# haberdashPI/SignalOperators.jl

Hardware: AMD Instinct MI355X
Metric: frames/sec sink() 44.1kHz 8ch Mix+Filt+Resample; achieved HBM GB/s (higher is better)
Workload: dtype f64

## Files before the change

### include/sigops.h

```cpp
#ifndef SIGOPS_H
#define SIGOPS_H

#include <stdint.h>

#ifdef __cplusplus
extern "C" {
#endif
#if defined(__GNUC__)
#pragma GCC visibility push(default)
#endif

#define SO_ABI_VERSION 1

typedef enum so_status {
    SO_OK = 0,
    SO_ERR_INVALID = -1,
    SO_ERR_LENGTH = -2,
    SO_ERR_UNSUPPORTED = -3,
    SO_ERR_RUNTIME = -4,
    SO_ERR_CHANNELS = -5,
    SO_ERR_NODEVICE = -6
} so_status_t;

typedef enum so_dtype {
// ... 30 lines not shown
    SO_FN_IDENTITY = 2,
    SO_FN_RANDN = 3
} so_fn_t;

typedef enum so_rampfn {
    SO_RAMP_SINRAMP = 0,
    SO_RAMP_IDENTITY = 1,
    SO_RAMP_EXPR = 2
} so_rampfn_t;

typedef enum so_mapfn {
    SO_MAP_ADD = 0,
    SO_MAP_MUL = 1,
    SO_MAP_SUB = 2,
    SO_MAP_DIV = 3,
    SO_MAP_TUPLECAT = 4,
    SO_MAP_GETCHAN = 5,
    SO_MAP_AS1CHANNEL = 6,
    SO_MAP_ASNCHANNELS = 7,
    SO_MAP_TOELTYPE = 8,
    SO_MAP_REVERSECH = 9,
    SO_MAP_EXPR = 10
} so_mapfn_t;

typedef struct so_eop {
    int32_t code;
    int32_t arg;
} so_eop_t;

typedef enum so_eop_code {
    SO_EOP_ARG = 0,
    SO_EOP_CONST = 1,
    SO_EOP_UN = 2,
    SO_EOP_BIN = 3,
    SO_EOP_CMP = 4,
    SO_EOP_SELECT = 5,
    SO_EOP_ROUND32 = 6,
    SO_EOP_INTERP = 7
} so_eop_code_t;

typedef enum so_un {
    SO_UN_NEG = 0, SO_UN_ABS = 1, SO_UN_SQRT = 2, SO_UN_CBRT = 3, SO_UN_SQUARE = 4,
    SO_UN_RECIPROCAL = 5, SO_UN_EXP = 6, SO_UN_EXP2 = 7, SO_UN_EXPM1 = 8, SO_UN_LOG = 9,
    SO_UN_LOG2 = 10, SO_UN_LOG10 = 11, SO_UN_LOG1P = 12, SO_UN_SIN = 13, SO_UN_COS = 14,
    SO_UN_TAN = 15, SO_UN_ARCSIN = 16, SO_UN_ARCCOS = 17, SO_UN_ARCTAN = 18, SO_UN_SINH = 19,
    SO_UN_COSH = 20, SO_UN_TANH = 21, SO_UN_ARCSINH = 22, SO_UN_ARCCOSH = 23,
    SO_UN_ARCTANH = 24, SO_UN_FLOOR = 25, SO_UN_CEIL = 26, SO_UN_TRUNC = 27, SO_UN_RINT = 28,
    SO_UN_SIGN = 29,
    SO_UN_COUNT = 30
} so_un_t;

typedef enum so_bin {
    SO_BIN_ADD = 0, SO_BIN_SUB = 1, SO_BIN_MUL = 2, SO_BIN_DIV = 3, SO_BIN_POW = 4,
    SO_BIN_REMAINDER = 5, SO_BIN_FMOD = 6, SO_BIN_MINIMUM = 7, SO_BIN_MAXIMUM = 8,
    SO_BIN_FMIN = 9, SO_BIN_FMAX = 10, SO_BIN_ARCTAN2 = 11, SO_BIN_HYPOT = 12,
    SO_BIN_COPYSIGN = 13,
    SO_BIN_COUNT = 14
} so_bin_t;

typedef enum so_cmp {
    SO_CMP_LT = 0, SO_CMP_LE = 1, SO_CMP_GT = 2, SO_CMP_GE = 3, SO_CMP_EQ = 4, SO_CMP_NE = 5,
    SO_CMP_COUNT = 6
} so_cmp_t;

typedef enum so_padkind {
    SO_PAD_VALUE = 0,
    SO_PAD_VECTOR = 1,
    SO_PAD_ZERO = 2,
    SO_PAD_ONE = 3,
    SO_PAD_LASTFRAME = 4,
    SO_PAD_CYCLE = 5,
    SO_PAD_MIRROR = 6
} so_padkind_t;

typedef enum so_rskind {
    SO_RS_RATIONAL = 0,
    SO_RS_ARBITRARY = 1,
    SO_RS_FIR = 2
} so_rskind_t;

typedef struct so_node {
    int32_t kind;
    int32_t dtype;
    int32_t nch;
    int32_t n_children;
    const int32_t* children;
    int64_t nframes;
    double fs;
    int32_t i0, i1, i2, i3;
    int64_t l0, l1;
    double d0, d1, d2, d3;
    const void* p0;
    const void* p1;
    int64_t s0, s1;
} so_node_t;

typedef struct so_out_desc {
    int32_t dtype;
    int32_t nch;
    int64_t nframes;
    int64_t frame_stride;
    int64_t chan_stride;
    int32_t is_device;
    int32_t reserved;
} so_out_desc_t;

typedef struct so_stats {
    int32_t n_stages;
    int32_t n_launches;
    int64_t algorithmic_bytes;
    int64_t scratch_bytes;
    int64_t h2d_bytes;
    int64_t d2h_bytes;
    double last_exec_ms;
    double dominant_kernel_ms;
    int64_t dominant_kernel_bytes;
    char dominant_kernel[64];
} so_stats_t;

typedef struct so_plan so_plan_t;

int32_t so_abi_version(void);

const char* so_last_error(void);

int32_t so_device_count(void);

int32_t so_plan_create(const so_node_t* nodes, int32_t n_nodes, int32_t root,
                       const so_out_desc_t* out, int32_t device, so_plan_t** plan);

int64_t so_plan_nframes(const so_plan_t* plan);

int32_t so_plan_execute(so_plan_t* plan, void* out, void* hip_stream);

int32_t so_plan_check(so_plan_t* plan, void* hip_stream);

int32_t so_plan_set_array(so_plan_t* plan, int32_t node_index, const void* data);

int32_t so_plan_stats(const so_plan_t* plan, so_stats_t* stats);

typedef struct so_step_info {
    char name[64];
    int64_t algorithmic_bytes;
    double ms;
    int32_t launches;
    int32_t pad;
} so_step_info_t;
int32_t so_plan_step_info(const so_plan_t* plan, int32_t index, so_step_info_t* info);

typedef enum so_counter {
    SO_COUNTER_GRAPH_REPLAYS = 0,
    SO_COUNTER_GRAPH_CAPTURES = 1,
    SO_COUNTER_DIRECT_EXECUTES = 2,
    SO_COUNTER_FUSED_MFMAS_PER_BLOCK = 3
} so_counter_t;
int64_t so_plan_counter(const so_plan_t* plan, int32_t which);

int32_t so_rtc_compile_check(const char* body, char* log, int32_t log_capacity);

int32_t so_rtc_wait_idle(void);
int32_t so_rtc_shutdown(void);

int32_t so_plan_set_profiling(so_plan_t* plan, int32_t enable);

void so_plan_destroy(so_plan_t* plan);

typedef struct so_comm so_comm_t;
typedef struct so_slab {
    int64_t rows, row_elems;
    int64_t dst_offset;
    int64_t dst_row_stride;
} so_slab_t;
int32_t so_comm_unique_id(void* id128);
int32_t so_comm_create(const void* id128, int32_t world, int32_t rank, int32_t device, so_comm_t** comm);
int32_t so_comm_allgather(so_comm_t* comm, const void* mine, int64_t src_row_stride, void* full,
                          const so_slab_t* slabs, int32_t dtype, void* stream);
int32_t so_comm_reduce_sum(so_comm_t* comm, void* buf, int64_t rows, int64_t row_elems, int64_t row_stride,
                           int32_t dtype, int32_t root, void* stream);
const char* so_comm_last_error(void);
void so_comm_destroy(so_comm_t* comm);

typedef enum so_filt_type {
    SO_FILT_LOWPASS = 0,
    SO_FILT_HIGHPASS = 1,
    SO_FILT_BANDPASS = 2,
    SO_FILT_BANDSTOP = 3
} so_filt_type_t;

typedef enum so_filt_method {
    SO_METHOD_BUTTERWORTH = 0,
    SO_METHOD_CHEBYSHEV1 = 1
} so_filt_method_t;

int32_t so_design_iir(int32_t type, double f1, double f2, double fs, int32_t method,
                      int32_t order, double ripple_db, double* sos, int32_t sos_capacity,
                      int32_t* nsections, double* gain);

int32_t so_design_iir_zpk(int32_t type, double f1, double f2, double fs, int32_t method, int32_t order,
                          double ripple_db, double* z, int32_t* nz, double* p, int32_t* np, int32_t capacity,
                          double* k);
int32_t so_zpk_to_sos(const double* z, int32_t nz, const double* p, int32_t np, double k, double* sos,
                      int32_t sos_capacity, int32_t* nsections, double* gain);

int32_t so_tf_to_sos(const double* b, int32_t nb, const double* a, int32_t na, double* sos, int32_t sos_capacity,
                     int32_t* nsections, double* gain, double* residual);
int32_t so_tf_zero_input(const double* b, int32_t nb, const double* a, int32_t na, const double* si, int32_t nsi,
                         double* out, int64_t capacity, int64_t* nframes);

int32_t so_design_resample_rational(int64_t num, int64_t den, double* h, int32_t capacity,
                                    int32_t* hlen);
int32_t so_design_resample_arbitrary(double rate, int32_t nphi, double* h, int32_t capacity,
                                     int32_t* hlen);

int32_t so_resample_positions(double fs_in, double fs_out, double rate, int32_t nphi, const double* h,
                              int32_t hlen, int64_t n_out, int64_t* j, int32_t* p, double* alpha,
                              int64_t* nfix, int64_t* nbaked);

#if defined(__GNUC__)
#pragma GCC visibility pop
#endif
#ifdef __cplusplus
}
#endif
#endif
```

### signaloperators.jl_amd/_capi.py

```python
import ctypes as C
import os

_HERE = os.path.dirname(os.path.abspath(__file__))
LIB_PATH = os.environ.get("SIGOPS_LIB") or os.path.join(_HERE, "csrc", "libsigops.so")

SO_F32, SO_F64, SO_I64 = 0, 1, 2
SO_LEN_INF, SO_LEN_MISSING, SO_LEN_UNCHECKED = -1, -2, -3
(NODE_ARRAY, NODE_CONST, NODE_FUNC, NODE_UNTIL, NODE_AFTER, NODE_PAD, NODE_APPEND, NODE_RAMP,
 NODE_MAP, NODE_FILT_SOS, NODE_RESAMPLE, NODE_NORMPOWER, NODE_SAMPLEAT, NODE_COMB, NODE_CUMSUM) = range(15)
FN = {"sin": 0, "cos": 1, "identity": 2, "randn": 3}
SO_FN_RANDN = FN["randn"]
RAMPFN = {"sinramp": 0, "identity": 1, "expr": 2}
MAPFN = {"add": 0, "mul": 1, "sub": 2, "div": 3, "tuplecat": 4, "getchan": 5, "as1channel": 6,
         "asnchannels": 7, "toeltype": 8, "reversech": 9, "expr": 10}
EOP = {"arg": 0, "const": 1, "un": 2, "bin": 3, "cmp": 4, "select": 5, "round32": 6, "interp": 7}
INTERP_MAX_KNOTS = 1 << 20
UN = {name: i for i, name in enumerate((
    "neg", "abs", "sqrt", "cbrt", "square", "reciprocal", "exp", "exp2", "expm1", "log", "log2", "log10", "log1p",
    "sin", "cos", "tan", "arcsin", "arccos", "arctan", "sinh", "cosh", "tanh", "arcsinh", "arccosh", "arctanh",
    "floor", "ceil", "trunc", "rint", "sign"))}
BIN = {name: i for i, name in enumerate((
    "add", "sub", "mul", "div", "pow", "remainder", "fmod", "minimum", "maximum", "fmin", "fmax", "arctan2", "hypot",
    "copysign"))}
CMP = {"lt": 0, "le": 1, "gt": 2, "ge": 3, "eq": 4, "ne": 5}
PAD = {"value": 0, "vector": 1, "zero": 2, "one": 3, "lastframe": 4, "cycle": 5, "mirror": 6}
RS_RATIONAL, RS_ARBITRARY, RS_FIR = 0, 1, 2
FILT = {"lowpass": 0, "highpass": 1, "bandpass": 2, "bandstop": 3}
METHOD = {"butterworth": 0, "chebyshev1": 1}


class so_node_t(C.Structure):
    _fields_ = [("kind", C.c_int32), ("dtype", C.c_int32), ("nch", C.c_int32),
                ("n_children", C.c_int32), ("children", C.POINTER(C.c_int32)),
                ("nframes", C.c_int64), ("fs", C.c_double),
                ("i0", C.c_int32), ("i1", C.c_int32), ("i2", C.c_int32), ("i3", C.c_int32),
                ("l0", C.c_int64), ("l1", C.c_int64),
                ("d0", C.c_double), ("d1", C.c_double), ("d2", C.c_double), ("d3", C.c_double),
                ("p0", C.c_void_p), ("p1", C.c_void_p), ("s0", C.c_int64), ("s1", C.c_int64)]


class so_out_desc_t(C.Structure):
    _fields_ = [("dtype", C.c_int32), ("nch", C.c_int32), ("nframes", C.c_int64),
                ("frame_stride", C.c_int64), ("chan_stride", C.c_int64),
                ("is_device", C.c_int32), ("reserved", C.c_int32)]


class so_stats_t(C.Structure):
    _fields_ = [("n_stages", C.c_int32), ("n_launches", C.c_int32),
                ("algorithmic_bytes", C.c_int64), ("scratch_bytes", C.c_int64),
                ("h2d_bytes", C.c_int64), ("d2h_bytes", C.c_int64),
                ("last_exec_ms", C.c_double), ("dominant_kernel_ms", C.c_double),
                ("dominant_kernel_bytes", C.c_int64), ("dominant_kernel", C.c_char * 64)]


class so_slab_t(C.Structure):
    _fields_ = [("rows", C.c_int64), ("row_elems", C.c_int64), ("dst_offset", C.c_int64), ("dst_row_stride", C.c_int64)]


class so_step_info_t(C.Structure):
    _fields_ = [("name", C.c_char * 64), ("algorithmic_bytes", C.c_int64), ("ms", C.c_double),
                ("launches", C.c_int32), ("pad", C.c_int32)]


EXPORTS = ["so_abi_version", "so_last_error", "so_device_count", "so_plan_create",
           "so_plan_nframes", "so_plan_execute", "so_plan_check", "so_plan_set_array", "so_plan_stats",
           "so_plan_set_profiling", "so_plan_destroy", "so_design_iir",
           "so_design_resample_rational", "so_design_resample_arbitrary",
           "so_resample_positions", "so_plan_step_info", "so_design_iir_zpk", "so_zpk_to_sos", "so_tf_to_sos", "so_tf_zero_input", "so_plan_counter",
           "so_rtc_compile_check", "so_rtc_wait_idle", "so_rtc_shutdown", "so_comm_unique_id", "so_comm_create", "so_comm_allgather", "so_comm_reduce_sum", "so_comm_last_error", "so_comm_destroy"]

_lib = None


class EngineMissing(RuntimeError):
    pass


def lib():
    global _lib
    if _lib is not None:
        return _lib
    if not os.path.exists(LIB_PATH):
        raise EngineMissing(
            f"{LIB_PATH} not built: run `python __graft_entry__.py build` "
            "(hipcc --offload-arch=gfx950). The HIP engine has no CPU fallback.")
    try:
        import importlib.util as _ilu

        if _ilu.find_spec("torch") is not None:
            import torch
    except Exception:
        pass
    L = C.CDLL(LIB_PATH)
    L.so_abi_version.restype = C.c_int32
    L.so_last_error.restype = C.c_char_p
    L.so_device_count.restype = C.c_int32
    L.so_plan_create.restype = C.c_int32
    L.so_plan_create.argtypes = [C.POINTER(so_node_t), C.c_int32, C.c_int32,
                                 C.POINTER(so_out_desc_t), C.c_int32, C.POINTER(C.c_void_p)]
    L.so_plan_nframes.restype = C.c_int64
    L.so_plan_nframes.argtypes = [C.c_void_p]
    L.so_plan_execute.restype = C.c_int32
    L.so_plan_execute.argtypes = [C.c_void_p, C.c_void_p, C.c_void_p]
    L.so_plan_check.restype = C.c_int32
    L.so_plan_check.argtypes = [C.c_void_p, C.c_void_p]
    L.so_plan_set_array.restype = C.c_int32
    L.so_plan_set_array.argtypes = [C.c_void_p, C.c_int32, C.c_void_p]
    L.so_plan_stats.restype = C.c_int32
    L.so_plan_stats.argtypes = [C.c_void_p, C.POINTER(so_stats_t)]
    L.so_plan_set_profiling.restype = C.c_int32
    L.so_plan_set_profiling.argtypes = [C.c_void_p, C.c_int32]
    L.so_plan_destroy.restype = None
    L.so_plan_destroy.argtypes = [C.c_void_p]
    L.so_design_iir.restype = C.c_int32
    L.so_design_iir.argtypes = [C.c_int32, C.c_double, C.c_double, C.c_double, C.c_int32,
                                C.c_int32, C.c_double, C.POINTER(C.c_double), C.c_int32,
                                C.POINTER(C.c_int32), C.POINTER(C.c_double)]
    L.so_design_resample_rational.restype = C.c_int32
    L.so_design_resample_rational.argtypes = [C.c_int64, C.c_int64, C.POINTER(C.c_double),
                                              C.c_int32, C.POINTER(C.c_int32)]
    L.so_design_resample_arbitrary.restype = C.c_int32
    L.so_design_resample_arbitrary.argtypes = [C.c_double, C.c_int32, C.POINTER(C.c_double),
                                               C.c_int32, C.POINTER(C.c_int32)]
    L.so_design_iir_zpk.restype = C.c_int32
    L.so_design_iir_zpk.argtypes = [C.c_int32, C.c_double, C.c_double, C.c_double, C.c_int32, C.c_int32, C.c_double,
                                    C.POINTER(C.c_double), C.POINTER(C.c_int32), C.POINTER(C.c_double),
                                    C.POINTER(C.c_int32), C.c_int32, C.POINTER(C.c_double)]
    L.so_zpk_to_sos.restype = C.c_int32
    L.so_zpk_to_sos.argtypes = [C.POINTER(C.c_double), C.c_int32, C.POINTER(C.c_double), C.c_int32, C.c_double,
                                C.POINTER(C.c_double), C.c_int32, C.POINTER(C.c_int32), C.POINTER(C.c_double)]
    L.so_tf_to_sos.restype = C.c_int32
    L.so_tf_to_sos.argtypes = [C.POINTER(C.c_double), C.c_int32, C.POINTER(C.c_double), C.c_int32, C.POINTER(C.c_double),
                               C.c_int32, C.POINTER(C.c_int32), C.POINTER(C.c_double), C.POINTER(C.c_double)]
    L.so_tf_zero_input.restype = C.c_int32
    L.so_tf_zero_input.argtypes = [C.POINTER(C.c_double), C.c_int32, C.POINTER(C.c_double), C.c_int32,
                                   C.POINTER(C.c_double), C.c_int32, C.POINTER(C.c_double), C.c_int64,
                                   C.POINTER(C.c_int64)]
    L.so_rtc_compile_check.restype = C.c_int32
    L.so_rtc_compile_check.argtypes = [C.c_char_p, C.c_char_p, C.c_int32]
    L.so_rtc_wait_idle.restype = C.c_int32
    L.so_rtc_wait_idle.argtypes = []
    L.so_rtc_shutdown.restype = C.c_int32
    L.so_rtc_shutdown.argtypes = []
    import atexit

    atexit.register(L.so_rtc_shutdown)
    L.so_comm_unique_id.restype = C.c_int32
    L.so_comm_unique_id.argtypes = [C.c_void_p]
    L.so_comm_create.restype = C.c_int32
    L.so_comm_create.argtypes = [C.c_void_p, C.c_int32, C.c_int32, C.c_int32, C.POINTER(C.c_void_p)]
    L.so_comm_allgather.restype = C.c_int32
    L.so_comm_allgather.argtypes = [C.c_void_p, C.c_void_p, C.c_int64, C.c_void_p, C.POINTER(so_slab_t), C.c_int32, C.c_void_p]
    L.so_comm_reduce_sum.restype = C.c_int32
    L.so_comm_reduce_sum.argtypes = [C.c_void_p, C.c_void_p, C.c_int64, C.c_int64, C.c_int64, C.c_int32, C.c_int32, C.c_void_p]
    L.so_comm_last_error.restype = C.c_char_p
    L.so_comm_destroy.restype = None
    L.so_comm_destroy.argtypes = [C.c_void_p]
    L.so_plan_counter.restype = C.c_int64
    L.so_plan_counter.argtypes = [C.c_void_p, C.c_int32]
    L.so_plan_step_info.restype = C.c_int32
    L.so_plan_step_info.argtypes = [C.c_void_p, C.c_int32, C.POINTER(so_step_info_t)]
    L.so_resample_positions.restype = C.c_int32
    L.so_resample_positions.argtypes = [C.c_double, C.c_double, C.c_double, C.c_int32, C.POINTER(C.c_double),
                                        C.c_int32, C.c_int64, C.POINTER(C.c_int64), C.POINTER(C.c_int32),
                                        C.POINTER(C.c_double), C.POINTER(C.c_int64), C.POINTER(C.c_int64)]
    if L.so_abi_version() != 1:
        raise EngineMissing("libsigops ABI version mismatch")
    _lib = L
    return L


def last_error():
    return lib().so_last_error().decode("utf-8", "replace")
```

### signaloperators.jl_amd/csrc/capi.cpp

```cpp
#include <hip/hip_runtime_api.h>

#include <cstring>
#include <string>
#include <vector>

#include "../../include/sigops.h"
#include "plan.h"

namespace {
thread_local std::string g_err;
int set_err(int status, const std::string& msg) {
    g_err = msg;
    return status;
}
}

struct so_plan {
    so::Plan* p;
};

extern "C" {

int32_t so_abi_version(void) { return SO_ABI_VERSION; }

// ... 53 lines not shown

int32_t so_plan_set_profiling(so_plan_t* plan, int32_t enable) {
    if (!plan) return set_err(SO_ERR_INVALID, "so_plan_set_profiling: null plan");
    so::plan_set_profiling(plan->p, enable);
    return SO_OK;
}

int32_t so_rtc_compile_check(const char* body, char* log, int32_t log_capacity) {
    if (!body) return set_err(SO_ERR_INVALID, "so_rtc_compile_check: null source");
    std::string err;
    const int st = so::rtc_compile_check(body, err);
    if (log && log_capacity > 0) std::snprintf(log, (size_t)log_capacity, "%s", err.c_str());
    return st == 0 ? SO_OK : set_err(SO_ERR_UNSUPPORTED, err);
}

int32_t so_rtc_wait_idle(void) {
    so::rtc_wait_idle();
    return SO_OK;
}

int32_t so_rtc_shutdown(void) {
    so::rtc_shutdown();
    return SO_OK;
}

int64_t so_plan_counter(const so_plan_t* plan, int32_t which) {
    if (!plan) return -1;
    return so::plan_counter(plan->p, which);
}

int32_t so_plan_step_info(const so_plan_t* plan, int32_t index, so_step_info_t* info) {
    if (!plan) return set_err(SO_ERR_INVALID, "so_plan_step_info: null plan");
    return so::plan_step_info(plan->p, index, info);
}

void so_plan_destroy(so_plan_t* plan) {
    if (!plan) return;
    so::plan_destroy(plan->p);
    delete plan;
}

int32_t so_design_iir(int32_t type, double f1, double f2, double fs, int32_t method,
                      int32_t order, double ripple_db, double* sos, int32_t sos_capacity,
                      int32_t* nsections, double* gain) {
    std::vector<double> s;
    double g = 1.0;
    std::string err;
    int st = so::design_iir(type, f1, f2, fs, method, order, ripple_db, s, g, err);
    if (st != SO_OK) return set_err(st, err);
    if (!sos || !nsections || !gain || (int)s.size() > sos_capacity)
        return set_err(SO_ERR_INVALID, "so_design_iir: output buffer too small");
    std::memcpy(sos, s.data(), s.size() * sizeof(double));
    *nsections = (int32_t)(s.size() / 6);
    *gain = g;
    return SO_OK;
}

int32_t so_design_iir_zpk(int32_t type, double f1, double f2, double fs, int32_t method, int32_t order,
                          double ripple_db, double* z, int32_t* nz, double* p, int32_t* np, int32_t capacity,
                          double* k) {
    std::vector<double> zz, pp;
    double kk = 1.0;
    std::string err;
    int st = so::design_iir_zpk(type, f1, f2, fs, method, order, ripple_db, zz, pp, kk, err);
    if (st != SO_OK) return set_err(st, err);
    if (!z || !p || !nz || !np || !k || (int)zz.size() > 2 * capacity || (int)pp.size() > 2 * capacity)
        return set_err(SO_ERR_INVALID, "so_design_iir_zpk: output buffer too small");
    std::memcpy(z, zz.data(), zz.size() * sizeof(double));
    std::memcpy(p, pp.data(), pp.size() * sizeof(double));
    *nz = (int32_t)(zz.size() / 2);
    *np = (int32_t)(pp.size() / 2);
    *k = kk;
    return SO_OK;
}

int32_t so_zpk_to_sos(const double* z, int32_t nz, const double* p, int32_t np, double k, double* sos,
                      int32_t sos_capacity, int32_t* nsections, double* gain) {
    std::vector<double> s;
    double g = 1.0;
    std::string err;
    if ((nz > 0 && !z) || (np > 0 && !p)) return set_err(SO_ERR_INVALID, "so_zpk_to_sos: null roots");
    int st = so::zpk_to_sos(z, nz, p, np, k, s, g, err);
    if (st != SO_OK) return set_err(st, err);
    if (!sos || !nsections || !gain || (int)s.size() > sos_capacity)
        return set_err(SO_ERR_INVALID, "so_zpk_to_sos: output buffer too small");
    std::memcpy(sos, s.data(), s.size() * sizeof(double));
    *nsections = (int32_t)(s.size() / 6);
    *gain = g;
    return SO_OK;
}

int32_t so_tf_to_sos(const double* b, int32_t nb, const double* a, int32_t na, double* sos, int32_t sos_capacity,
                     int32_t* nsections, double* gain, double* residual) {
    std::vector<double> s;
    double g = 1.0, r = 0.0;
    std::string err;
    int st = so::tf_to_sos(b, nb, a, na, s, g, r, err);
    if (st != SO_OK) return set_err(st, err);
    if (!sos || !nsections || !gain || (int)s.size() > sos_capacity)
        return set_err(SO_ERR_INVALID, "so_tf_to_sos: output buffer too small");
    std::memcpy(sos, s.data(), s.size() * sizeof(double));
    *nsections = (int32_t)(s.size() / 6);
    *gain = g;
    if (residual) *residual = r;
    return SO_OK;
}

int32_t so_tf_zero_input(const double* b, int32_t nb, const double* a, int32_t na, const double* si, int32_t nsi,
                         double* out, int64_t capacity, int64_t* nframes) {
    std::string err;
    int64_t used = 0;
    if (!out || !nframes || capacity < 0) return set_err(SO_ERR_INVALID, "so_tf_zero_input: null output");
    int st = so::tf_zero_input(b, nb, a, na, si, nsi, out, capacity, used, err);
    if (st != SO_OK) return set_err(st, err);
    *nframes = used;
    return SO_OK;
}

static int32_t copy_taps(const std::vector<double>& h, double* out, int32_t capacity, int32_t* hlen) {
    if (!hlen) return set_err(SO_ERR_INVALID, "null hlen");
    *hlen = (int32_t)h.size();
    if (!out) return SO_OK;
    if ((int)h.size() > capacity) return set_err(SO_ERR_INVALID, "tap buffer too small");
    std::memcpy(out, h.data(), h.size() * sizeof(double));
    return SO_OK;
}

int32_t so_design_resample_rational(int64_t num, int64_t den, double* h, int32_t capacity,
                                    int32_t* hlen) {
    std::vector<double> t;
    std::string err;
    int st = so::design_resample_rational(num, den, t, err);
    if (st != SO_OK) return set_err(st, err);
    return copy_taps(t, h, capacity, hlen);
}

int32_t so_design_resample_arbitrary(double rate, int32_t nphi, double* h, int32_t capacity,
                                     int32_t* hlen) {
    std::vector<double> t;
    std::string err;
    int st = so::design_resample_arbitrary(rate, nphi, t, err);
    if (st != SO_OK) return set_err(st, err);
    return copy_taps(t, h, capacity, hlen);
}

int32_t so_resample_positions(double fs_in, double fs_out, double rate, int32_t nphi, const double* h,
                              int32_t hlen, int64_t n_out, int64_t* j, int32_t* p, double* alpha,
                              int64_t* nfix, int64_t* nbaked) {
    if (!h || hlen < 1 || nphi < 1 || !(rate > 0) || n_out < 0 || !j || !p || !alpha)
        return set_err(SO_ERR_INVALID, "so_resample_positions: bad arguments");
    return so::resample_positions(fs_in, fs_out, rate, nphi, h, hlen, n_out, j, p, alpha, nfix, nbaked);
}

}
```

### signaloperators.jl_amd/csrc/executor.cpp

```cpp
#include "plan_impl.h"

namespace so {

static inline int carrier_vec_ok(const DCarrier& c, int64_t V) {
    if (!std::getenv("SIGOPS_STRICT_ALIGN")) return (uintptr_t)c.base % (c.dtype == SO_F64 ? 8 : 4) == 0;
    return ((uintptr_t)c.base % 16 == 0) && (c.cstride % V == 0);
}

static hipError_t h2d_small(void* dst, const void* src, size_t bytes) {
    constexpr size_t kPiece = 16 * 1024;
    if (bytes < 2 * kPiece || bytes > (1u << 20)) return hipMemcpy(dst, src, bytes, hipMemcpyHostToDevice);
    for (size_t off = 0; off < bytes; off += kPiece) {
        const hipError_t e = hipMemcpy((char*)dst + off, (const char*)src + off, std::min(kPiece, bytes - off), hipMemcpyHostToDevice);
        if (e != hipSuccess) return e;
    }
    return hipSuccess;
}

void Plan::finalize() {
    for (size_t si = 0; si < stages.size(); ++si) {
        Stage& S = stages[si];
        if (S.out_buf >= 0 && ((int)si == alias_stage || S.win_off >= 0)) {
            bufs[S.out_buf].external = true;
            bufs[S.out_buf].bytes = 0;
// ... 1101 lines not shown
                P->steps[si].ms = ms;
                total += ms;
                if (ms > best) {
                    best = ms;
                    P->stats.dominant_kernel_ms = ms;
                    P->stats.dominant_kernel_bytes = P->steps[si].bytes;
                    std::snprintf(P->stats.dominant_kernel, sizeof P->stats.dominant_kernel, "%s", P->steps[si].name.c_str());
                }
            }
            P->stats.last_exec_ms = total;
        }
    } catch (const PlanError& e) {
        err = e.msg;
        return e.status;
    }
    return SO_OK;
}

int plan_execute(Plan* P, void* outp, void* stream, std::string& err) {
    DeviceGuard guard(P->device);
    if (kernel_gave_up(P, err)) return SO_ERR_RUNTIME;
    const bool eligible = P->steps.size() >= 4 && P->out.is_device && P->host_leaves.empty() && !P->profiling &&
                          !std::getenv("SIGOPS_NO_GRAPH") && !std::getenv("SIGOPS_RS_TRACE");
    if (!eligible) {
        P->n_direct++;
        return plan_execute_direct(P, outp, stream, err);
    }
    hipStream_t st = (hipStream_t)stream;
    const bool leaves_match = P->out_alias_buf < 0 || P->bufs[P->out_alias_buf].d == outp;
    if (P->graph_exec && P->graph_out == outp && P->graph_epoch == P->array_epoch && leaves_match) {
        if (hipSetDevice(P->device) == hipSuccess && hipGraphLaunch(P->graph_exec, st) == hipSuccess) {
            P->n_replays++;
            return SO_OK;
        }
        (void)hipGetLastError();
        (void)hipGraphExecDestroy(P->graph_exec);
        P->graph_exec = nullptr;
        P->graph_failed = true;
    }
    if (P->graph_failed || P->last_out != outp || P->last_epoch != P->array_epoch) {
        P->last_out = outp;
        P->last_epoch = P->array_epoch;
        P->n_direct++;
        return plan_execute_direct(P, outp, stream, err);
    }
    if (P->graph_exec && P->graph_out == outp && P->graph_epoch == P->array_epoch) {
        P->n_direct++;
        return plan_execute_direct(P, outp, stream, err);
    }
    if (P->graph_exec) {
        (void)hipGraphExecDestroy(P->graph_exec);
        P->graph_exec = nullptr;
    }
    hipGraph_t graph = nullptr;
    if (!P->capture_stream && hipStreamCreateWithFlags(&P->capture_stream, hipStreamNonBlocking) != hipSuccess)
        P->capture_stream = nullptr;
    if (!P->capture_stream || hipSetDevice(P->device) != hipSuccess ||
        hipStreamBeginCapture(P->capture_stream, hipStreamCaptureModeRelaxed) != hipSuccess) {
        (void)hipGetLastError();
        P->graph_failed = true;
        return plan_execute_direct(P, outp, stream, err);
    }
    const int rc = plan_execute_direct(P, outp, (void*)P->capture_stream, err);
    const hipError_t ec = hipStreamEndCapture(P->capture_stream, &graph);
    if (std::getenv("SIGOPS_DEBUG_PLAN"))
        std::fprintf(stderr, "[sigops] graph capture: rc=%d end=%d (%s) graph=%p err=%s\n", rc, (int)ec, hipGetErrorString(ec), (void*)graph, err.c_str());
    if (rc != SO_OK || ec != hipSuccess || !graph ||
        hipGraphInstantiate(&P->graph_exec, graph, nullptr, nullptr, 0) != hipSuccess) {
        (void)hipGetLastError();
        if (graph) (void)hipGraphDestroy(graph);
        P->graph_exec = nullptr;
        P->graph_failed = true;
        return rc != SO_OK ? rc : plan_execute_direct(P, outp, stream, err);
    }
    (void)hipGraphDestroy(graph);
    P->graph_out = outp;
    P->graph_epoch = P->array_epoch;
    P->n_captures++;
    if (hipGraphLaunch(P->graph_exec, st) != hipSuccess) {
        (void)hipGetLastError();
        P->graph_failed = true;
        return plan_execute_direct(P, outp, stream, err);
    }
    return SO_OK;
}

int plan_set_array(Plan* P, int32_t node_index, const void* data, std::string& err) {
    if (node_index < 0 || node_index >= (int)P->nodes.size() || P->nodes[node_index].nd.kind != SO_NODE_ARRAY) {
        err = "so_plan_set_array: not an ARRAY node";
        return SO_ERR_INVALID;
    }
    DeviceGuard guard(P->device);
    P->array_ptr[node_index] = data;
    P->array_epoch++;
    if (P->nodes[node_index].nd.i0) {
        bool changed = false;
        for (size_t i = 0; i < P->leaves.size(); ++i)
            if (P->leaf_array_node[i] == node_index) {
                P->leaves[i].base = data;
                changed = true;
            }
        if (changed && P->d_leaves)
            if (hipMemcpy(P->d_leaves, P->leaves.data(), P->leaves.size() * sizeof(DLeaf), hipMemcpyHostToDevice) != hipSuccess) {
                err = "so_plan_set_array: leaf upload failed";
                return SO_ERR_RUNTIME;
            }
        for (auto& S : P->stages) {
            bool touched = false;
            for (auto& c : S.carriers) {
                if (c.array_node == node_index) {
                    c.base = data;
                    const int64_t V = 16 / (int64_t)dsize(c.dtype);
                    c.vec_ok = carrier_vec_ok(c, V);
                    touched = true;
                }
                if (car_has_arr2(c) && c.array_node2 == node_index) {
                    c.base2 = data;
                    c.vec_ok2 = (uintptr_t)c.base2 % (c.dtype2 == SO_F64 ? 8 : 4) == 0;
                    touched = true;
                }
            }
            if (touched) {
                const RsCtl ctl = P->make_ctl(S);
                if (hipMemcpy(P->bufs[S.car_buf].d, S.carriers.data(), S.carriers.size() * sizeof(DCarrier), hipMemcpyHostToDevice) != hipSuccess ||
                    hipMemcpy(P->bufs[S.ctl_buf].d, &ctl, sizeof(RsCtl), hipMemcpyHostToDevice) != hipSuccess) {
                    err = "so_plan_set_array: carrier upload failed";
                    return SO_ERR_RUNTIME;
                }
            }
        }
    }
    return SO_OK;
}

int64_t plan_nframes(const Plan* P) {
    const Node& R = P->nodes[P->root];
    return isinf_(R.len) ? SO_LEN_INF : R.len.n;
}
void plan_stats(const Plan* P, so_stats_t* st) { *st = P->stats; }
void plan_set_profiling(Plan* P, int mode) {
    P->profiling = mode < 0 || mode > 2 ? 1 : mode;
    P->prof_execs = 0;
}
int64_t plan_counter(const Plan* P, int which) {
    switch (which) {
    case SO_COUNTER_GRAPH_REPLAYS: return P->n_replays;
    case SO_COUNTER_GRAPH_CAPTURES: return P->n_captures;
    case SO_COUNTER_DIRECT_EXECUTES: return P->n_direct;
    case SO_COUNTER_FUSED_MFMAS_PER_BLOCK: {
        for (const Stage& S : P->stages)
            if (S.kind == ST_SOS && S.rsos_src >= 0 && S.need > 0) return S.rs.ks + 14;
        return 0;
    }
    default: return -1;
    }
}
int plan_step_info(const Plan* P, int index, so_step_info_t* info) {
    if (info && index >= 0 && index < (int)P->steps.size()) {
        const Step& s = P->steps[index];
        std::memset(info, 0, sizeof *info);
        std::snprintf(info->name, sizeof info->name, "%s", s.name.c_str());
        info->algorithmic_bytes = s.bytes;
        info->ms = s.ms;
        if (P->profiling == 2 && P->prof_execs > 0) {
            const size_t evset = 2 * P->steps.size();
            const int64_t n = std::min<int64_t>(P->prof_execs, (int64_t)prof_cap(P));
            double sum = 0;
            int64_t got = 0;
            for (int64_t e = 0; e < n; ++e) {
                float ms = 0;
                if (hipEventElapsedTime(&ms, P->events[evset * e + 2 * index], P->events[evset * e + 2 * index + 1]) == hipSuccess) {
                    sum += ms;
                    ++got;
                } else (void)hipGetLastError();
            }
            info->ms = got ? sum / (double)got : 0.0;
        }
        info->launches = s.launches;
    }
    return (int)P->steps.size();
}
int plan_check(Plan* P, void* stream, std::string& err) {
    DeviceGuard guard(P->device);
    try {
        if (P->nlanes > 1 || P->graph_exec) HIPCHECK(hipDeviceSynchronize());
        else HIPCHECK(hipStreamSynchronize((hipStream_t)stream));
    } catch (const PlanError& e) {
        err = e.msg;
        return e.status;
    }
    if (kernel_gave_up(P, err)) return SO_ERR_RUNTIME;
    return SO_OK;
}

void plan_destroy(Plan* P) {
    if (!P) return;
    {
        DeviceGuard guard(P->device);
        P->release();
    }
    delete P;
}


}
```

### signaloperators.jl_amd/csrc/k_rsos.hip

```cpp
#include "kcommon.h"
#include "kstage.h"

#ifndef SO_RSOS_ONLY_KS
#define SO_RSOS_ONLY_KS -1
#endif
#ifndef SO_RSOS_ONLY_F32
#define SO_RSOS_ONLY_F32 0
#endif
#ifndef SO_RSOS_ONLY_NW
#define SO_RSOS_ONLY_NW 0
#endif

namespace so {

typedef double v4d __attribute__((ext_vector_type(4)));
typedef float v4f __attribute__((ext_vector_type(4)));

#define SO_LDS __attribute__((address_space(3)))
__device__ __forceinline__ int flag_ld(uint32_t a) { return *(const volatile SO_LDS int*)(uintptr_t)a; }
__device__ __forceinline__ void flag_st(uint32_t a, int v) { *(volatile SO_LDS int*)(uintptr_t)a = v; }
#define SO_SPIN_PAUSE(spins, sleep, limit)                         \
    do {                                                           \
        if (++(spins) > (limit)) rsos_wait_failed(sh);             \
        if ((sleep) == 1) __builtin_amdgcn_s_sleep(1);             \
// ... 39 lines not shown
    return double2{sb, cb};
}

template <int RU>
__device__ __attribute__((noinline)) void rsos_stage_slow(int64_t n_in, int rpitch, const DCarrier* gcar, int ncar, const DOp* gops,
                                                          const DLeaf* gleaves, int64_t n0, int lanes, int ch0, double* buf) {
    const int lane = threadIdx.x & 63;
    if (lane < lanes) stage_generic_impl<double, RU, true>(n_in, rpitch, gcar, ncar, gops, gleaves, n0 + 2 * lane, lane, 0, ch0, buf);
}
template <int RU>
__device__ __attribute__((noinline)) void rsos_stage_slow32(int64_t n_in, int rpitch, const DCarrier* gcar, int ncar, const DOp* gops,
                                                            const DLeaf* gleaves, int64_t n0, int lanes, int ch0, float* buf) {
    const int lane = threadIdx.x & 63;
    if (lane < lanes) stage_generic_impl<float, RU>(n_in, 2 * rpitch, gcar, ncar, gops, gleaves, n0 + 4 * lane, lane, 0, ch0, buf);
}

template <int RU, int OP>
__device__ __forceinline__ void rsos_rmw(uint32_t la, uint32_t row_bytes, v2d gn) {
    if constexpr (RU > 4) {
        rsos_rmw<4, OP>(la, row_bytes, gn);
        rsos_rmw<RU - 4, OP>(la + 4 * row_bytes, row_bytes, gn);
        return;
    } else {
        v2d raw[RU];
#pragma unroll
        for (int c = 0; c < RU; ++c) raw[c] = lds_ld16(la + (uint32_t)c * row_bytes);
        lds_wait(raw);
#pragma unroll
        for (int c = 0; c < RU; ++c) raw[c] = OP == 0 ? raw[c] * gn : OP == 1 ? raw[c] + gn : OP == 2 ? raw[c] - gn : gn - raw[c];
        lds_pin(raw);
#pragma unroll
        for (int c = 0; c < RU; ++c) lds_st16(la + (uint32_t)c * row_bytes, raw[c]);
    }
}

template <int RU>
__device__ __forceinline__ void rsos_add(uint32_t la, uint32_t row_bytes, v2d gn) {
    const double g0 = gn[0], g1 = gn[1];
#pragma unroll
    for (int c = 0; c < RU; ++c) {
        const uint32_t a = la + (uint32_t)c * row_bytes;
        asm volatile("ds_add_f64 %0, %1\n\tds_add_f64 %0, %2 offset:8" ::"v"(a), "v"(g0), "v"(g1) : "memory");
    }
}

template <int RB, int C, int RU>
__device__ __forceinline__ void rsos_add_imm(uint32_t la, double g0, double g1) {
    if constexpr (C < RU) {
        asm volatile("ds_add_f64 %0, %1 offset:%3\n\tds_add_f64 %0, %2 offset:%4" ::"v"(la), "v"(g0), "v"(g1), "n"(C * RB), "n"(C * RB + 8) : "memory");
        rsos_add_imm<RB, C + 1, RU>(la, g0, g1);
    }
}

template <int RB, int R, int N>
__device__ __forceinline__ void rsos_add_rows(uint32_t la0, uint32_t la8, double g0, double g1) {
    if constexpr (N > 0) {
        asm volatile("ds_add_f64 %0, %1 offset:%3\n\tds_add_f64 %0, %2 offset:%4" ::"v"(R < 8 ? la0 : la8), "v"(g0), "v"(g1), "n"((R & 7) * RB), "n"((R & 7) * RB + 8) : "memory");
        rsos_add_rows<RB, R + 1, N - 1>(la0, la8, g0, g1);
    }
}
template <int RB, int RU, int NL, int J, int MUC>
__device__ __forceinline__ void rsos_add_units(uint32_t la0, uint32_t la8, const double2 (&bs)[MUC], double2 d0, double2 d1, bool sine, double gc, bool neg) {
    if constexpr (J < MUC) {
        double g0 = gc, g1 = gc;
        if (sine) {
            g0 = fma(bs[J].x, d0.y, bs[J].y * d0.x);
            g1 = fma(bs[J].x, d1.y, bs[J].y * d1.x);
        }
        if (neg) {
            g0 = -g0;
            g1 = -g1;
        }
        rsos_add_rows<RB, J * NL * RU, RU>(la0, la8, g0, g1);
        rsos_add_units<RB, RU, NL, J + 1, MUC>(la0, la8, bs, d0, d1, sine, gc, neg);
    }
}

template <int RU, int OP>
__device__ __forceinline__ void rsos_step32(uint32_t la, uint32_t row_bytes, float g0, float g1) {
    if constexpr (RU > 4) {
        rsos_step32<4, OP>(la, row_bytes, g0, g1);
        rsos_step32<RU - 4, OP>(la + 4 * row_bytes, row_bytes, g0, g1);
    } else {
        float2 raw[RU];
#pragma unroll
        for (int c = 0; c < RU; ++c) asm volatile("ds_read_b64 %0, %1" : "=v"(raw[c]) : "v"(la + (uint32_t)c * row_bytes) : "memory");
        if constexpr (RU == 4) asm volatile("s_waitcnt lgkmcnt(0)" : "+v"(raw[0]), "+v"(raw[1]), "+v"(raw[2]), "+v"(raw[3])::"memory");
        else if constexpr (RU == 2) asm volatile("s_waitcnt lgkmcnt(0)" : "+v"(raw[0]), "+v"(raw[1])::"memory");
        else asm volatile("s_waitcnt lgkmcnt(0)" : "+v"(raw[0])::"memory");
#pragma unroll
        for (int c = 0; c < RU; ++c) {
            raw[c].x = OP == 0 ? raw[c].x * g0 : OP == 1 ? raw[c].x + g0 : g0 - raw[c].x;
            raw[c].y = OP == 0 ? raw[c].y * g1 : OP == 1 ? raw[c].y + g1 : g1 - raw[c].y;
        }
#pragma unroll
        for (int c = 0; c < RU; ++c) asm volatile("ds_write_b64 %0, %1" ::"v"(la + (uint32_t)c * row_bytes), "v"(raw[c]) : "memory");
    }
}

template <int RB, int RU, int OP>
__device__ __forceinline__ void rsos_step32_imm(uint32_t la, float g0, float g1) {
    float2 raw[RU];
#define SO_RD(C) if constexpr (C < RU) asm volatile("ds_read_b64 %0, %1 offset:%2" : "=v"(raw[C < RU ? C : 0]) : "v"(la), "n"((C < RU ? C : 0) * RB) : "memory");
    SO_RD(0) SO_RD(1) SO_RD(2) SO_RD(3) SO_RD(4) SO_RD(5) SO_RD(6) SO_RD(7)
#undef SO_RD
    if constexpr (RU == 8) asm volatile("s_waitcnt lgkmcnt(0)" : "+v"(raw[0]), "+v"(raw[1]), "+v"(raw[2]), "+v"(raw[3]), "+v"(raw[4]), "+v"(raw[5]), "+v"(raw[6]), "+v"(raw[7])::"memory");
    else if constexpr (RU == 4) asm volatile("s_waitcnt lgkmcnt(0)" : "+v"(raw[0]), "+v"(raw[1]), "+v"(raw[2]), "+v"(raw[3])::"memory");
    else if constexpr (RU == 2) asm volatile("s_waitcnt lgkmcnt(0)" : "+v"(raw[0]), "+v"(raw[1])::"memory");
    else asm volatile("s_waitcnt lgkmcnt(0)" : "+v"(raw[0])::"memory");
#pragma unroll
    for (int c = 0; c < RU; ++c) {
        raw[c].x = OP == 0 ? raw[c].x * g0 : OP == 1 ? raw[c].x + g0 : g0 - raw[c].x;
        raw[c].y = OP == 0 ? raw[c].y * g1 : OP == 1 ? raw[c].y + g1 : g1 - raw[c].y;
    }
#define SO_WR(C) if constexpr (C < RU) asm volatile("ds_write_b64 %0, %1 offset:%2" ::"v"(la), "v"(raw[C < RU ? C : 0]), "n"((C < RU ? C : 0) * RB) : "memory");
    SO_WR(0) SO_WR(1) SO_WR(2) SO_WR(3) SO_WR(4) SO_WR(5) SO_WR(6) SO_WR(7)
#undef SO_WR
}

template <int RU, int OP>
__device__ __forceinline__ void rsos_widen(uint32_t slot, uint32_t row_bytes, int lane, double g0, double g1) {
    if constexpr (RU > 4) {
        rsos_widen<4, OP>(slot, row_bytes, lane, g0, g1);
        rsos_widen<RU - 4, OP>(slot + 4 * row_bytes, row_bytes, lane, g0, g1);
        return;
    } else {
        float a[RU], b[RU];
        const uint32_t ra = slot + 512u + (uint32_t)lane * 4u;
#pragma unroll
        for (int c = 0; c < RU; ++c) {
            asm volatile("ds_read_b32 %0, %1" : "=v"(a[c]) : "v"(ra + (uint32_t)c * row_bytes) : "memory");
            asm volatile("ds_read_b32 %0, %1 offset:256" : "=v"(b[c]) : "v"(ra + (uint32_t)c * row_bytes) : "memory");
        }
        if constexpr (RU == 4) asm volatile("s_waitcnt lgkmcnt(0)" : "+v"(a[0]), "+v"(a[1]), "+v"(a[2]), "+v"(a[3]), "+v"(b[0]), "+v"(b[1]), "+v"(b[2]), "+v"(b[3])::"memory");
        else if constexpr (RU == 2) asm volatile("s_waitcnt lgkmcnt(0)" : "+v"(a[0]), "+v"(a[1]), "+v"(b[0]), "+v"(b[1])::"memory");
        else asm volatile("s_waitcnt lgkmcnt(0)" : "+v"(a[0]), "+v"(b[0])::"memory");
        double v0[RU], v1[RU];
#pragma unroll
        for (int c = 0; c < RU; ++c) {
            const double x0 = (double)a[c], x1 = (double)b[c];
            v0[c] = OP == 0 ? x0 * g0 : OP == 1 ? x0 + g0 : OP == 2 ? x0 - g0 : OP == 3 ? g0 - x0 : x0;
            v1[c] = OP == 0 ? x1 * g1 : OP == 1 ? x1 + g1 : OP == 2 ? x1 - g1 : OP == 3 ? g1 - x1 : x1;
        }
        const uint32_t wa = slot + (uint32_t)lane * 8u;
#pragma unroll
        for (int c = 0; c < RU; ++c) {
            asm volatile("ds_write_b64 %0, %1" ::"v"(wa + (uint32_t)c * row_bytes), "v"(v0[c]) : "memory");
            asm volatile("ds_write_b64 %0, %1 offset:512" ::"v"(wa + (uint32_t)c * row_bytes), "v"(v1[c]) : "memory");
        }
    }
}

constexpr int kRsosFlagLdp = 0, kRsosFlagYrd = 4, kRsosFlagXseq = 16, kRsosFlagSseq = 48, kRsosFlagXh = 49, kRsosFlagLnd = 52, kRsosFlags = 56;
constexpr int kRsosHres0 = 1, kRsosHres1 = 5, kRsosHres2 = 7, kRsosHelper = 6, kRsosHslots = 3;
constexpr int kRsosMaxGroups = 256;

struct RsosShared {
    RsSos g;
    const DCarrier* gcar;
    const DOp* gops;
    const DLeaf* gleaves;
    void* y;
    const double* tab;
    int flags[kRsosFlags];
    int jend[kRsosMaxGroups];
    RsCtl ctl;
};

__device__ __forceinline__ int uni(int v) { return __builtin_amdgcn_readfirstlane(v); }


#define SO_GLB __attribute__((address_space(1)))

__device__ __forceinline__ void rsos_wait_failed(SO_LDS RsosShared* sh) {
    uint32_t SO_GLB* const e = (uint32_t SO_GLB*)rfl64((int64_t)(uintptr_t)sh->g.err);
    if (e == nullptr) __builtin_trap();
    if ((threadIdx.x & 63) == 0) __hip_atomic_store((uint32_t*)e, 1u, __ATOMIC_RELAXED, __HIP_MEMORY_SCOPE_SYSTEM);
    __threadfence_system();
    asm volatile("s_waitcnt vmcnt(0) lgkmcnt(0)" ::: "memory");
    __builtin_amdgcn_endpgm();
}

#ifndef SO_RSOS_TRACE
#define SO_RSOS_TRACE 0
#endif
__device__ __forceinline__ void rsos_stamp(long long* trace, int wave, int it, int k, int it0 = 400) {
    if constexpr (!SO_RSOS_TRACE) return;
    if (trace != nullptr && blockIdx.x == 0 && (threadIdx.x & 63) == 0 && it >= it0 && it < it0 + kRsosTraceIters)
        ((long long SO_GLB*)trace)[(wave * kRsosTraceIters + (it - it0)) * 8 + k] = clock64();
}

#ifndef SO_RSOS_COUNT
#define SO_RSOS_COUNT 0
#endif
__device__ __forceinline__ void rsos_count_out(long long* trace, int wave, int row, int k, long long v) {
    if constexpr (!SO_RSOS_COUNT) return;
    if (trace != nullptr && blockIdx.x == 0) ((long long SO_GLB*)trace)[((wave * kRsosTraceIters) + row) * 8 + k] = v + 1;
}

struct RsosLds {
    SO_LDS double *taps, *ring, *gtab;
    volatile SO_LDS double *xs, *ss;
    volatile SO_LDS double* xh;
};
__device__ __forceinline__ SO_LDS double* rsos_lds_ptr(const void* p) {
    return (SO_LDS double*)(uintptr_t)__builtin_amdgcn_readfirstlane((uint32_t)(uintptr_t)(const SO_LDS void*)p);
}
#ifndef SO_NSS_EXTRA
#define SO_NSS_EXTRA (ny + 1)
#endif
__host__ __device__ constexpr int rsos_nss(int ny) { return ny + SO_NSS_EXTRA; }
__device__ __forceinline__ RsosLds rsos_carve(double* dyn_, int tapd, int rpitch, int nx, int ns) {
    RsosLds l;
    SO_LDS double* dyn = rsos_lds_ptr(dyn_);
    l.taps = dyn;
    l.ring = l.taps + tapd;
    l.xs = l.ring + (size_t)16 * rpitch;
    l.ss = l.xs + (size_t)nx * 192;
    l.gtab = (SO_LDS double*)l.ss + (size_t)ns * 192;
    l.xh = l.gtab + 16 * 16 * 2;
    return l;
}

struct RsosGroup {
    int cg;
    int64_t pb0;
    int64_t ob0;
    int64_t prM, prL;
    int64_t r0;
    int e0m, prMm;
};
__device__ __forceinline__ RsosGroup rsos_group(const SO_LDS RsosShared* sh, int64_t G, bool single, int64_t base0_8, int64_t cs0, int64_t df0) {
    const SO_LDS RsSos& g = sh->g;
    const int ct = uni(g.ct), rgs = uni(g.rgs);
    const int64_t ncg = uni(g.nch) / ct;
    const int64_t pr = rfl64(g.pr), M = rfl64(g.M), L = rfl64(g.L);
    const int wp = uni(g.wp), ulo = uni(g.ulo);
    RsosGroup q;
    q.cg = (int)(G % ncg);
    const int64_t r0 = (G / ncg) * rgs;
    q.r0 = r0;
    q.pb0 = (r0 * pr - wp) * M;
    q.ob0 = (r0 * pr - wp) * L;
    q.prM = pr * M;
    q.prL = pr * L;
    if (single) {
        const int64_t e = base0_8 + (int64_t)(q.cg * ct) * cs0 + df0 + q.pb0 + ulo;
        q.e0m = (int)(((e % 16) + 16) % 16);
        q.prMm = (int)(q.prM % 16);
    } else
        q.e0m = q.prMm = 0;
    return q;
}

template <int NY, int NK>
__device__ __attribute__((noinline)) void rsos_chain(RsosShared* sh_, double* dyn, int64_t G_) {
    constexpr int NX = 2 * NY + 1;
    const int lane = threadIdx.x & 63;
    SO_LDS RsosShared* const sh = (SO_LDS RsosShared*)rsos_lds_ptr(sh_);
    const SO_LDS RsSos& g = sh->g;
    const int ngroups = uni(g.ngroups);
    const RsosLds l = rsos_carve(dyn, uni(g.cyc) > 0 ? 0 : ngroups * uni(g.ks) * 64, uni(g.rpitch), NX, rsos_nss(NY));
    const int NB = (uni(g.wp) + (int)rfl64(g.pr)) * ngroups;
    const double SO_GLB* mats = (const double SO_GLB*)rfl64((int64_t)(uintptr_t)g.mats);
    long long* trace = (long long*)rfl64((int64_t)(uintptr_t)g.trace);
    const uint32_t fl_base = (uint32_t)(uintptr_t)sh->flags;
    const int debug = uni(g.debug);
    double Ak[3];
#pragma unroll
    for (int v = 0; v < 3; ++v) Ak[v] = mats[(4 + v) * 64 + lane];
    __builtin_amdgcn_s_setprio(3);
    int spins = 0;
    [[maybe_unused]] int cnt_wait = 0, cnt_blocks = 0;
    [[maybe_unused]] const long long cyc0 = SO_RSOS_COUNT ? clock64() : 0;
    while (uni(flag_ld(fl_base + 4 * (kRsosFlagXseq + 0))) < 1 && !(debug & 4)) SO_SPIN_PAUSE(spins, 1, 1 << 22);
    v4d sA = v4d{0.0, 0.0, 0.0, 0.0}, sB = v4d{0.0, 0.0, 0.0, 0.0};
    v4d dA = v4d{0.0, 0.0, 0.0, 0.0}, dB = v4d{0.0, 0.0, 0.0, 0.0};
#pragma unroll
    for (int v = 0; v < NK; ++v) dA[v] = l.xs[v * 64 + lane];
    if (NB > 1) {
        spins = 0;
        while (uni(flag_ld(fl_base + 4 * (kRsosFlagXseq + 1))) < 2 && !(debug & 4)) SO_SPIN_PAUSE(spins, 1, 1 << 22);
#pragma unroll
        for (int v = 0; v < NK; ++v) dB[v] = l.xs[192 + v * 64 + lane];
    }
    const uint32_t xs0 = (uint32_t)(uintptr_t)l.xs + (uint32_t)lane * 8u, ss0 = (uint32_t)(uintptr_t)l.ss + (uint32_t)lane * 8u;
    int fA = NB > 2 ? flag_ld(fl_base + 4 * (kRsosFlagXseq + 2 % NX)) : 0x7fffffff;
    int fB = NB > 3 ? flag_ld(fl_base + 4 * (kRsosFlagXseq + 3 % NX)) : 0x7fffffff;
    int slot = 0;
    int sslot = 0;
    constexpr int NS = rsos_nss(NY);
    auto step = [&](int b, v4d& sin, v4d& sout, v4d& din, int& fpend) __attribute__((always_inline)) {
        int f = uni(fpend);
        const int s2 = slot + 2 >= NX ? slot + 2 - NX : slot + 2, s4 = s2 + 2 >= NX ? s2 + 2 - NX : s2 + 2;
        uint32_t ax = xs0 + (uint32_t)s2 * 1536u, as = ss0 + (uint32_t)sslot * 1536u;
        uint32_t af = fl_base + 4u * (uint32_t)(kRsosFlagXseq + s4), ag = fl_base + 4u * (uint32_t)kRsosFlagSseq;
        int bv = b;
        asm volatile("" : "+v"(ax), "+v"(as), "+v"(af), "+v"(ag), "+v"(bv));
        __builtin_amdgcn_sched_barrier(0);
        v4d acc = __builtin_amdgcn_mfma_f64_16x16x4f64(Ak[0], sin[0], din, 0, 0, 0);
        __builtin_amdgcn_sched_barrier(0);
#ifndef SO_CHAIN_ORDER
#define SO_CHAIN_ORDER 1
#endif
        auto put_state = [&]() __attribute__((always_inline)) {
            if (!(debug & 1024)) {
#pragma unroll
                for (int v = 0; v < NK; ++v) *(volatile SO_LDS double*)(uintptr_t)(as + (uint32_t)v * 512u) = sin[v];
                *(volatile SO_LDS int*)(uintptr_t)ag = bv;
            }
        };
        const bool more = b + 2 < NB && !(debug & 512);
        auto wait_dx = [&]() __attribute__((always_inline)) {
            if (more && f < b + 3 && !(debug & 4)) {
                spins = 0;
                if constexpr (SO_RSOS_COUNT) cnt_blocks += lane == (b + 2) % NY ? 1 : 0;
                do {
                    SO_SPIN_PAUSE(spins, 1, 1 << 22);
                    if constexpr (SO_RSOS_COUNT) cnt_wait += lane == (b + 2) % NY ? 1 : 0;
                    f = uni(flag_ld(fl_base + 4 * (kRsosFlagXseq + s2)));
                } while (f < b + 3);
            }
        };
        auto get_dx = [&]() __attribute__((always_inline)) {
            if (more) {
#pragma unroll
                for (int v = 0; v < NK; ++v) din[v] = *(volatile SO_LDS double*)(uintptr_t)(ax + (uint32_t)v * 512u);
            }
        };
        auto get_flag = [&]() __attribute__((always_inline)) {
            if (more && b + 4 < NB) fpend = *(volatile SO_LDS int*)(uintptr_t)af;
        };
        if constexpr (NK == 1) {
            put_state();
            wait_dx();
            get_dx();
            get_flag();
        } else if constexpr (NK == 2) {
            put_state();
            wait_dx();
            get_dx();
            get_flag();
            __builtin_amdgcn_sched_barrier(0);
            acc = __builtin_amdgcn_mfma_f64_16x16x4f64(Ak[1], sin[1], acc, 0, 0, 0);
        } else if constexpr (SO_CHAIN_ORDER == 0) {
            wait_dx();
            get_dx();
            get_flag();
            put_state();
            __builtin_amdgcn_sched_barrier(0);
            acc = __builtin_amdgcn_mfma_f64_16x16x4f64(Ak[1], sin[1], acc, 0, 0, 0);
            acc = __builtin_amdgcn_mfma_f64_16x16x4f64(Ak[2], sin[2], acc, 0, 0, 0);
        } else {
            put_state();
            __builtin_amdgcn_sched_barrier(0);
            acc = __builtin_amdgcn_mfma_f64_16x16x4f64(Ak[1], sin[1], acc, 0, 0, 0);
            __builtin_amdgcn_sched_barrier(0);
            wait_dx();
            get_dx();
            get_flag();
            __builtin_amdgcn_sched_barrier(0);
            acc = __builtin_amdgcn_mfma_f64_16x16x4f64(Ak[2], sin[2], acc, 0, 0, 0);
        }
        __builtin_amdgcn_sched_barrier(0);
        sout = acc;
        slot = slot + 1 == NX ? 0 : slot + 1;
        sslot = sslot + 1 == NS ? 0 : sslot + 1;
    };
    for (int b = 0; b < NB; b += 2) {
        rsos_stamp(trace, 0, b >> 1, 0, 200);
        step(b, sA, sB, dA, fA);
        if (b + 1 < NB) step(b + 1, sB, sA, dB, fB);
        rsos_stamp(trace, 0, b >> 1, 3, 200);
    }
    __builtin_amdgcn_s_setprio(0);
    if constexpr (SO_RSOS_COUNT) {
        if (lane < 8) rsos_count_out(trace, 0, 0, lane, cnt_wait);
        else if (lane < 16) rsos_count_out(trace, 0, 1, lane - 8, cnt_wait);
        if (lane < 8) rsos_count_out(trace, 0, 2, lane, cnt_blocks);
        else if (lane < 16) rsos_count_out(trace, 0, 3, lane - 8, cnt_blocks);
        if (lane == 0) rsos_count_out(trace, 0, 4, 0, clock64() - cyc0);
    }
    int32_t* bad = (int32_t*)rfl64((int64_t)(uintptr_t)g.bad);
    if (bad != nullptr) {
        const v4d sE = (NB & 1) ? sB : sA;
        const bool nf = !(isfinite(sE[0]) && (NK < 2 || isfinite(sE[1])) && (NK < 3 || isfinite(sE[2])));
        const uint64_t m = __ballot(nf);
        const uint32_t rows = (uint32_t)((m | (m >> 16) | (m >> 32) | (m >> 48)) & 0xffffu);
        if (rows != 0 && lane < 16 && ((rows >> lane) & 1u)) {
            const int ct = uni(g.ct), rgs = uni(g.rgs);
            const int64_t G = rfl64(G_);
            const int64_t ncg = uni(g.nch) / ct;
            const int64_t r = (G / ncg) * rgs + lane / ct;
            if (r < uni(g.nranges)) atomicMin(bad + ((int)(G % ncg) * ct + lane % ct), (int32_t)r);
        }
    }
}

__device__ __forceinline__ bool rsos_two_ok(const SO_LDS DCarrier& C0, int chunk) {
    const uint64_t b0 = (uint64_t)rfl64((int64_t)(uintptr_t)C0.base), b2 = (uint64_t)rfl64((int64_t)(uintptr_t)C0.base2);
    const int64_t df0 = rfl64(C0.df), df2 = rfl64(C0.df2), cs0 = rfl64(C0.cstride), cs2 = rfl64(C0.cstride2);
    return uni((int)(C0.base2 != nullptr && C0.vec_ok2 && C0.dtype2 == SO_F64)) && chunk == 128 && !((((b2 >> 3) + (uint64_t)df2) ^ ((b0 >> 3) + (uint64_t)df0)) & 1) &&
           !((cs2 ^ cs0) & 1);
}

__device__ __forceinline__ int vmcnt_now() {
    const uint32_t v = __builtin_amdgcn_s_getreg(7 | (0 << 6) | (31 << 11));
    return (int)((v & 0xfu) | ((v >> 18) & 0x30u));
}

template <int NY, int NL, int RU, bool SRC32, int RB = 0, int MODE = 0, bool A2 = false>
__device__ __attribute__((noinline)) void rsos_loader(RsosShared* sh_, double* dyn, int64_t G_, int q_) {
    static_assert(!A2 || ((RU == 8 || RU == 4 || RU == 2) && !SRC32 && MODE == 2 && NL == 2), "the second array's waves: groups of two, four or eight channels, sixteen waves");
    constexpr int NX = 2 * NY + 1;
    const int lane = threadIdx.x & 63;
    const int wave = uni(threadIdx.x >> 6);
    SO_LDS RsosShared* const sh = (SO_LDS RsosShared*)rsos_lds_ptr(sh_);
    const int64_t G = rfl64(G_);
    const int q = uni(q_);
    const SO_LDS RsSos& g = sh->g;
    const int ngroups = uni(g.ngroups), rpitch = uni(g.rpitch), RING = uni(g.ring), CH = uni(g.chunk);
    const RsosLds l = rsos_carve(dyn, uni(g.cyc) > 0 ? 0 : ngroups * uni(g.ks) * 64, rpitch, NX, rsos_nss(NY));
    const int ct = uni(g.ct);
    const int M = (int)rfl64(g.M);
    const int NP = uni(g.wp) + (int)rfl64(g.pr);
    const int ulo = uni(g.ulo);
    const int64_t n_in = rfl64(g.n_in);
    long long* trace = (long long*)rfl64((int64_t)(uintptr_t)g.trace);
    const uint32_t fl_base = (uint32_t)(uintptr_t)sh->flags;
    constexpr int nunits = 16 / RU;
    const int lanes = CH >> 1;
    const uint64_t dmask = lanes >= 64 ? ~0ull : ((1ull << lanes) - 1ull);
    const int total_rho = (NP - 1) * M + uni(sh->jend[ngroups - 1]) - ulo + 1 + 16;
    const int NK = (total_rho + CH - 1) / CH;
    const uint32_t ring_b = (uint32_t)(uintptr_t)l.ring;
    const uint32_t row_bytes = (uint32_t)rpitch * 8u;
    const uint32_t lane16 = (uint32_t)lane * 16u;
    __builtin_amdgcn_s_setprio(2);
    const SO_LDS DCarrier& C0 = sh->ctl.car[0];
    const int64_t a0 = rfl64(C0.a), b0 = rfl64(C0.b), cs0 = rfl64(C0.cstride), df0 = rfl64(C0.df);
    const char* const base0 = (const char*)rfl64((int64_t)(uintptr_t)C0.base);
    const int fuse = uni(g.fuse), fuse_sine = uni(g.fuse_sine), debug = uni(g.debug);
    const bool ring32 = SRC32 && uni(g.ring32) != 0;
    const bool sring = ring32 && uni(g.sring) != 0;
    const uint32_t half_bytes = (uint32_t)uni(g.rpitch) * 4u;
    constexpr bool src32 = SRC32;
    constexpr int esh = src32 ? 2 : 3;
    const bool single = uni((int)(C0.base != nullptr && C0.vec_ok && C0.dtype == (src32 ? SO_F32 : SO_F64))) && !(df0 & 1) && fuse >= -1 &&
                        (!src32 || CH == 128) && (!uni(g.arr2) || rsos_two_ok(C0, CH));
    const int64_t lo_ok = a0 > 0 ? a0 : 0, hi_ok = b0 < n_in ? b0 : n_in;
    const RsosGroup grp = rsos_group(sh, G, single, (int64_t)((uintptr_t)base0 >> esh), cs0, df0);
    const int kind0 = uni(C0.slot_kind[0]);
    const DLeaf leaf0 = leaf_uniform(sh_->ctl.leaves[min(kCtlLeaves - 1, max(0, uni(C0.slot_leaf[0])))]);
    double2 d0 = double2{0.0, 1.0}, d1 = double2{0.0, 1.0};
    double2 d16 = double2{0.0, 1.0};
    double gconst = 0.0;
    if (fuse >= 0) {
        if (fuse_sine) {
            d0 = rsos_sine_at(src32 && !ring32 ? lane : 2 * lane, leaf0.v0, 0.0, leaf0.v2, leaf0.flag);
            d1 = rsos_sine_at(src32 && !ring32 ? 64 + lane : 2 * lane + 1, leaf0.v0, 0.0, leaf0.v2, leaf0.flag);
            d16 = rsos_sine_at(16 * CH, leaf0.v0, 0.0, leaf0.v2, leaf0.flag);
        } else
            gconst = slot_eval(kind0, leaf0, 0);
    }
    double2 rbase[4] = {double2{0.0, 1.0}, double2{0.0, 1.0}, double2{0.0, 1.0}, double2{0.0, 1.0}};
    const int shift = CH == 128 ? 7 : 6;
    int64_t Au_l = 0, rowb_l = 0;
    int klo_l = 1, khi_l = 0, ch0_l = 0;
    int kzl_l = 0, kzh_l = 0x3fffffff;
    uint32_t lds_l = 0;
    {
        const int u = q + lane * NL;
        if (u < nunits) {
            const int ri = (u * RU) / ct, c0u = (u * RU) % ct;
            ch0_l = grp.cg * ct + c0u;
            Au_l = grp.pb0 + ri * grp.prM + ulo - ((grp.e0m + ri * grp.prMm) & 15);
            rowb_l = (int64_t)(uintptr_t)base0 + (((int64_t)ch0_l * cs0 + df0 + Au_l) << esh);
            lds_l = ring_b + (uint32_t)(u * RU) * row_bytes;
            {
                const int64_t zl = (-Au_l) >> shift, zh = (n_in - Au_l + CH - 1) >> shift;
                kzl_l = (int)(zl < 0 ? 0 : (zl > 0x3fffffff ? 0x3fffffff : zl));
                kzh_l = (int)(zh < 0 ? 0 : (zh > 0x3fffffff ? 0x3fffffff : zh));
            }
            if (single) {
                const int64_t lo = (lo_ok - Au_l + CH - 1) >> shift, hi = (hi_ok - Au_l) >> shift;
                klo_l = (int)(lo < 0 ? 0 : (lo > 0x3fffffff ? 0x3fffffff : lo));
                khi_l = (int)(hi < 0 ? 0 : (hi > 0x3fffffff ? 0x3fffffff : hi));
            }
        }
    }
    auto lane64 = [&](int64_t v, int j) __attribute__((always_inline)) {
        const uint32_t lo = __builtin_amdgcn_readlane((uint32_t)v, j), hi = __builtin_amdgcn_readlane((uint32_t)((uint64_t)v >> 32), j);
        return (int64_t)(((uint64_t)hi << 32) | lo);
    };
    const int MU = (nunits - q + NL - 1) / NL;
    const int64_t rowb_s0 = lane64(rowb_l, 0), rowb_s1 = lane64(rowb_l, 1), Au_s0 = lane64(Au_l, 0), Au_s1 = lane64(Au_l, 1);
    const int klo_s0 = __builtin_amdgcn_readlane(klo_l, 0), khi_s0 = __builtin_amdgcn_readlane(khi_l, 0);
    const int klo_s1 = __builtin_amdgcn_readlane(klo_l, 1), khi_s1 = __builtin_amdgcn_readlane(khi_l, 1);
    const int ch0_s0 = __builtin_amdgcn_readlane(ch0_l, 0), ch0_s1 = __builtin_amdgcn_readlane(ch0_l, 1);
    const uint32_t lds_s0 = (uint32_t)__builtin_amdgcn_readlane((int)lds_l, 0), lds_s1 = (uint32_t)__builtin_amdgcn_readlane((int)lds_l, 1);
    auto u_klo = [&](int j) __attribute__((always_inline)) { return j == 0 ? klo_s0 : j == 1 ? klo_s1 : __builtin_amdgcn_readlane(klo_l, j); };
    auto u_khi = [&](int j) __attribute__((always_inline)) { return j == 0 ? khi_s0 : j == 1 ? khi_s1 : __builtin_amdgcn_readlane(khi_l, j); };
    auto u_rowb = [&](int j) __attribute__((always_inline)) { return j == 0 ? rowb_s0 : j == 1 ? rowb_s1 : lane64(rowb_l, j); };
    auto u_Au = [&](int j) __attribute__((always_inline)) { return j == 0 ? Au_s0 : j == 1 ? Au_s1 : lane64(Au_l, j); };
    auto u_ch0 = [&](int j) __attribute__((always_inline)) { return j == 0 ? ch0_s0 : j == 1 ? ch0_s1 : __builtin_amdgcn_readlane(ch0_l, j); };
    auto u_lds = [&](int j) __attribute__((always_inline)) { return j == 0 ? lds_s0 : j == 1 ? lds_s1 : (uint32_t)__builtin_amdgcn_readlane((int)lds_l, j); };
    auto issue = [&](int k, int rho0) __attribute__((always_inline)) -> int {
        int n = 0;
        if constexpr (RU < 8) {
            const bool mine = lane < MU;
            const bool fast_l = mine && k >= klo_l && k < khi_l && !(debug & 8192);
            const bool zero_l = mine && !(k >= klo_l && k < khi_l) && (k < kzl_l || k >= kzh_l);
            const bool slow_l = mine && !(k >= klo_l && k < khi_l) && !zero_l && !(debug & 4096);
            const uint64_t fast_m = __ballot(fast_l), zero_m = __ballot(zero_l), slow_m = __ballot(slow_l);
            const int64_t row_l = rowb_l + ((int64_t)k << (shift + esh));
            for (uint64_t m = fast_m; m; m &= m - 1) {
                const int j = __builtin_ctzll(m);
                const char* row = (const char*)(uintptr_t)lane64(row_l, j);
                const uint32_t ld = (uint32_t)__builtin_amdgcn_readlane((int)lds_l, j);
                if constexpr (src32) dma_rows<RU>(0xffffffffull, lane16, row, cs0 * 4, ld + (ring32 ? (uint32_t)rho0 * 4u : (uint32_t)rho0 * 8u + 512u), row_bytes);
                else dma_rows<RU>(dmask, lane16, row, cs0 * 8, ld + (uint32_t)rho0 * 8u, row_bytes);
                n += RU;
            }
            for (uint64_t m = zero_m; m; m &= m - 1) {
                const int j = __builtin_ctzll(m);
                if (lane < (ring32 ? lanes >> 1 : lanes)) {
                    const uint32_t la = (uint32_t)__builtin_amdgcn_readlane((int)lds_l, j) + (uint32_t)rho0 * (ring32 ? 4u : 8u) + lane16;
                    const v2d z = v2d{0.0, 0.0};
#pragma unroll
                    for (int c = 0; c < RU; ++c) lds_st16(la + (uint32_t)c * row_bytes, z);
                }
            }
            for (uint64_t m = slow_m; m; m &= m - 1) {
                const int j = __builtin_ctzll(m);
                const int u = q + j * NL;
                if (ring32) {
                    if constexpr (src32)
                        rsos_stage_slow32<RU>(n_in, rpitch, (const DCarrier*)rfl64((int64_t)(uintptr_t)sh->gcar), uni(sh->ctl.ncar),
                                              (const DOp*)rfl64((int64_t)(uintptr_t)sh->gops), (const DLeaf*)rfl64((int64_t)(uintptr_t)sh->gleaves),
                                              lane64(Au_l, j) + ((int64_t)k << shift), lanes >> 1, __builtin_amdgcn_readlane(ch0_l, j),
                                              (float*)(l.ring + (size_t)(u * RU) * rpitch) + rho0);
                } else
                    rsos_stage_slow<RU>(n_in, rpitch, (const DCarrier*)rfl64((int64_t)(uintptr_t)sh->gcar), uni(sh->ctl.ncar),
                                        (const DOp*)rfl64((int64_t)(uintptr_t)sh->gops), (const DLeaf*)rfl64((int64_t)(uintptr_t)sh->gleaves),
                                        lane64(Au_l, j) + ((int64_t)k << shift), lanes, __builtin_amdgcn_readlane(ch0_l, j),
                                        (double*)(l.ring + (size_t)(u * RU) * rpitch + rho0));
            }
            return n;
        }
        for (int j = 0; j < MU; ++j) {
            const bool fast = k >= u_klo(j) && k < u_khi(j);
            if (fast && (debug & 8192)) continue;
            if (fast) {
                const char* row = (const char*)(uintptr_t)(u_rowb(j) + ((int64_t)k << (shift + esh)));
                if constexpr (src32) dma_rows<RU>(0xffffffffull, lane16, row, cs0 * 4, u_lds(j) + (ring32 ? (uint32_t)rho0 * 4u : (uint32_t)rho0 * 8u + 512u), row_bytes);
                else dma_rows<RU>(dmask, lane16, row, cs0 * 8, u_lds(j) + (uint32_t)rho0 * 8u, row_bytes);
                n += RU;
            } else if (k < __builtin_amdgcn_readlane(kzl_l, j) || k >= __builtin_amdgcn_readlane(kzh_l, j)) {
                if (lane < (ring32 ? lanes >> 1 : lanes)) {
                    const uint32_t la = u_lds(j) + (uint32_t)rho0 * (ring32 ? 4u : 8u) + lane16;
                    const v2d z = v2d{0.0, 0.0};
#pragma unroll
                    for (int c = 0; c < RU; ++c) lds_st16(la + (uint32_t)c * row_bytes, z);
                }
            } else if (!(debug & 4096) && ring32) {
                if constexpr (src32) {
                    const int u = q + j * NL;
                    rsos_stage_slow32<RU>(n_in, rpitch, (const DCarrier*)rfl64((int64_t)(uintptr_t)sh->gcar), uni(sh->ctl.ncar),
                                          (const DOp*)rfl64((int64_t)(uintptr_t)sh->gops), (const DLeaf*)rfl64((int64_t)(uintptr_t)sh->gleaves),
                                          u_Au(j) + ((int64_t)k << shift), lanes >> 1, u_ch0(j),
                                          (float*)(l.ring + (size_t)(u * RU) * rpitch) + rho0);
                }
            } else if (!(debug & 4096)) {
                const int u = q + j * NL;
                rsos_stage_slow<RU>(n_in, rpitch, (const DCarrier*)rfl64((int64_t)(uintptr_t)sh->gcar), uni(sh->ctl.ncar),
                                    (const DOp*)rfl64((int64_t)(uintptr_t)sh->gops), (const DLeaf*)rfl64((int64_t)(uintptr_t)sh->gleaves),
                                    u_Au(j) + ((int64_t)k << shift), lanes, u_ch0(j),
                                    (double*)(l.ring + (size_t)(u * RU) * rpitch + rho0));
// ... 166 lines not shown
        }
        flag_st(fl_base + 4 * (kRsosFlagLdp + q), (k + 1) * CH);
        rsos_stamp(trace, wave, k, 4, 40);
    };
    if constexpr (MODE == 2 && A2) {
        constexpr int MUA = (16 / RU) / NL;
        const char* const base2 = (const char*)rfl64((int64_t)(uintptr_t)C0.base2);
        const int64_t cs2 = rfl64(C0.cstride2), df2 = rfl64(C0.df2);
        v2d b0[8], b1[8], b2[8];
        auto ld = [&](int k, v2d (&b)[8]) __attribute__((always_inline)) -> int {
            int n = 0;
            if (k >= NK) return 0;
#pragma unroll
            for (int j = 0; j < MUA; ++j) {
                if (!(k >= u_klo(j) && k < u_khi(j))) continue;
                const char* row = base2 + ((((int64_t)u_ch0(j) * cs2 + df2 + u_Au(j)) << 3) + ((int64_t)k << 10));
#pragma unroll
                for (int c = 0; c < RU; ++c) {
                    uint64_t rc = (uint64_t)(uintptr_t)(row + (int64_t)c * cs2 * 8);
                    asm volatile("" : "+s"(rc));
                    asm volatile("global_load_dwordx4 %0, %1, %2" SO_LD_NT : "=v"(b[j * RU + c]) : "v"(lane16), "s"(rc) : "memory");
                }
                n += RU;
            }
            return n;
        };
        auto ap = [&](int k, int rho0, v2d (&b)[8], int nself, int younger) __attribute__((always_inline)) {
            int sp = 0;
            while (uni(flag_ld(fl_base + 4 * (kRsosFlagLnd + q))) < k + 1 && !(debug & 32)) SO_SPIN_PAUSE(sp, 2, 1 << 22);
            if (nself && !(debug & 2)) {
                wait_vmcnt_le60(younger);
#pragma unroll
                for (int j = 0; j < MUA; ++j) {
                    if (!(k >= u_klo(j) && k < u_khi(j))) continue;
                    const uint32_t la = u_lds(j) + (uint32_t)rho0 * 8u + lane16;
                    if (fuse == 1) {
#pragma unroll
                        for (int c = 0; c < RU; ++c)
                            asm volatile("ds_add_f64 %0, %1\n\tds_add_f64 %0, %2 offset:8" ::"v"(la + (uint32_t)c * row_bytes), "v"(b[j * RU + c][0]), "v"(b[j * RU + c][1]) : "memory");
                    } else if (fuse == 2) {
#pragma unroll
                        for (int c = 0; c < RU; ++c)
                            asm volatile("ds_add_f64 %0, %1\n\tds_add_f64 %0, %2 offset:8" ::"v"(la + (uint32_t)c * row_bytes), "v"(-b[j * RU + c][0]), "v"(-b[j * RU + c][1]) : "memory");
                    } else {
#pragma unroll
                        for (int c = 0; c < RU; ++c) {
                            const uint32_t a = la + (uint32_t)c * row_bytes;
                            v2d vv[1] = {lds_ld16(a)};
                            lds_wait(vv);
                            vv[0] = fuse == 0 ? vv[0] * b[j * RU + c] : b[j * RU + c] - vv[0];
                            lds_pin(vv);
                            lds_st16(a, vv[0]);
                        }
                    }
                }
            }
            flag_st(fl_base + 4 * (kRsosFlagLdp + q), (k + 1) * CH);
        };
        int n0 = ld(0, b0), n1 = ld(1, b1), n2 = ld(2, b2);
        int rho = 0;
        for (int k = 0; k < NK; k += 3) {
            ap(k, rho, b0, n0, n1 + n2);
            n0 = ld(k + 3, b0);
            rho = rho + CH == RING ? 0 : rho + CH;
            if (k + 1 < NK) {
                ap(k + 1, rho, b1, n1, n2 + n0);
                n1 = ld(k + 4, b1);
                rho = rho + CH == RING ? 0 : rho + CH;
            }
            if (k + 2 < NK) {
                ap(k + 2, rho, b2, n2, n0 + n1);
                n2 = ld(k + 5, b2);
                rho = rho + CH == RING ? 0 : rho + CH;
            }
        }
        asm volatile("s_waitcnt vmcnt(0)" ::: "memory");
        __builtin_amdgcn_s_setprio(0);
        return;
    }
    if constexpr (MODE == 2) {
        int rho = 0, spins2 = 0;
        for (int k = 0; k < NK; ++k) {
            spins2 = 0;
            while (uni(flag_ld(fl_base + 4 * (kRsosFlagLnd + q))) < k + 1 && !(debug & 32)) SO_SPIN_PAUSE(spins2, 2, 1 << 22);
            retire(k, rho, 0);
            rho = rho + CH == RING ? 0 : rho + CH;
        }
        __builtin_amdgcn_s_setprio(0);
        return;
    }
    int issued = 0, retired = 0;
    int rho_i = 0, rho_r = 0;
    int c0n = 0, c1n = 0, c2n = 0;
    const int depth = uni(g.depth);
    int minrd = 0;
    int spins = 0;
    [[maybe_unused]] int cnt_idle = 0;
    [[maybe_unused]] const long long cyc0 = SO_RSOS_COUNT ? clock64() : 0;
    for (;;) {
        if (retired < issued && !(debug & 16384)) {
            const int inflight = issued - retired;
            const int allowed = (inflight > 1 ? c0n : 0) + (inflight > 2 ? c1n : 0) + (inflight > 3 ? c2n : 0);
            if (vmcnt_now() <= allowed) {
                retire(retired, rho_r, allowed);
                rho_r = rho_r + CH == RING ? 0 : rho_r + CH;
                ++retired;
                spins = 0;
                continue;
            }
        }
        bool can = issued < NK && issued - retired < depth;
        if (can && (issued + 1) * CH > RING) {
            const int needrd = (issued + 1) * CH - RING;
            if (minrd < needrd) {
                const int v = lane < NY ? flag_ld(fl_base + 4 * (kRsosFlagYrd + lane)) : 0x7fffffff;
                minrd = wave_min(v, NY);
            }
            can = minrd >= needrd || (debug & 32);
        }
        if (can) {
            spins = 0;
            rsos_stamp(trace, wave, issued, 0, 40);
            const int n = issue(issued, rho_i);
            rsos_stamp(trace, wave, issued, 1, 40);
            rho_i = rho_i + CH == RING ? 0 : rho_i + CH;
            c2n = c1n;
            c1n = c0n;
            c0n = n;
            ++issued;
            continue;
        }
        if (retired < issued) {
            const int inflight = issued - retired;
            const int allowed = (inflight > 1 ? c0n : 0) + (inflight > 2 ? c1n : 0) + (inflight > 3 ? c2n : 0);
            retire(retired, rho_r, allowed);
            rho_r = rho_r + CH == RING ? 0 : rho_r + CH;
            ++retired;
            spins = 0;
            continue;
        }
        if (issued >= NK) break;
        SO_SPIN_PAUSE(spins, 2, 1 << 22);
        if constexpr (SO_RSOS_COUNT) ++cnt_idle;
    }
    __builtin_amdgcn_s_setprio(0);
    if constexpr (SO_RSOS_COUNT) {
        if (lane == 0) {
            rsos_count_out(trace, wave, 0, 0, cnt_idle);
            rsos_count_out(trace, wave, 0, 4, clock64() - cyc0);
        }
    }
}

template <int NY>
__device__ __attribute__((noinline)) void rsos_helper(RsosShared* sh_, double* dyn) {
    constexpr int NX = 2 * NY + 1;
    const int lane = threadIdx.x & 63;
    SO_LDS RsosShared* const sh = (SO_LDS RsosShared*)rsos_lds_ptr(sh_);
    const SO_LDS RsSos& g = sh->g;
    const RsosLds l = rsos_carve(dyn, 0, uni(g.rpitch), NX, rsos_nss(NY));
    const int NB = (uni(g.wp) + (int)rfl64(g.pr)) * uni(g.ngroups);
    const double SO_GLB* mats = (const double SO_GLB*)rfl64((int64_t)(uintptr_t)g.mats);
    const uint32_t fl_base = (uint32_t)(uintptr_t)sh->flags;
    const int debug = uni(g.debug);
    const bool f32m = uni(g.f32m) != 0 && uni(g.out_f32) != 0;
    double Dk[4];
#pragma unroll
    for (int v = 0; v < 4; ++v) Dk[v] = f32m ? mats[(lane >> 4) * 64 + v * 16 + (lane & 15)] : mats[v * 64 + lane];
    __builtin_amdgcn_s_setprio(1);
    constexpr int res[3] = {kRsosHres0, kRsosHres1, kRsosHres2};
    int hslot[3] = {kRsosHres0 % NX, kRsosHres1 % NX, kRsosHres2 % NX}, hring = 0;
    for (int b0 = 0; b0 < NB; b0 += NY) {
#pragma unroll
        for (int j = 0; j < 3; ++j) {
            const int bh = b0 + res[j];
            if (bh < NB) {
                int spins = 0;
                while (uni(flag_ld(fl_base + 4 * (kRsosFlagXh + j))) < bh + 1 && !(debug & 16)) SO_SPIN_PAUSE(spins, 2, 1 << 22);
                double xr[4];
#pragma unroll
                for (int v = 0; v < 3; ++v) xr[v] = l.xs[hslot[j] * 192 + v * 64 + lane];
                xr[3] = l.xh[(j * kRsosHslots + hring) * 64 + lane];
                v4d dh = v4d{0.0, 0.0, 0.0, 0.0};
#pragma unroll
                for (int v = 0; v < 4; ++v) dh = __builtin_amdgcn_mfma_f64_16x16x4f64(Dk[v], xr[v], dh, 0, 0, 0);
#pragma unroll
                for (int v = 0; v < 3; ++v) l.xs[hslot[j] * 192 + v * 64 + lane] = dh[v];
                flag_st(fl_base + 4 * (kRsosFlagXseq + hslot[j]), bh + 1);
            }
            hslot[j] += NY;
            if (hslot[j] >= NX) hslot[j] -= NX;
        }
        hring = hring + 1 == kRsosHslots ? 0 : hring + 1;
    }
    __builtin_amdgcn_s_setprio(0);
}

template <int KS, int NY, int NL, typename TO, int CYC, bool F32M = false, bool HW = false>
__device__ __attribute__((noinline)) void rsos_ywave(RsosShared* sh_, double* dyn, int64_t G_, int yi_) {
    static_assert(!F32M || (sizeof(TO) == 4 && CYC > 0), "the Float32 MFMA form: Float32 results, taps in registers");
    constexpr int NX = 2 * NY + 1;
    const int lane = threadIdx.x & 63;
    const int wave = uni(threadIdx.x >> 6);
    SO_LDS RsosShared* const sh = (SO_LDS RsosShared*)rsos_lds_ptr(sh_);
    const int64_t G = rfl64(G_);
    const int yi = uni(yi_);
    const SO_LDS RsSos& g = sh->g;
    const int ngroups = uni(g.ngroups), rpitch = uni(g.rpitch), RING = uni(g.ring);
    const RsosLds l = rsos_carve(dyn, CYC > 0 ? 0 : ngroups * KS * 64, rpitch, NX, rsos_nss(NY));
    const int ct = uni(g.ct), wp = uni(g.wp), debug = uni(g.debug);
    const int M = (int)rfl64(g.M);
    const int NB = (wp + (int)rfl64(g.pr)) * ngroups;
    constexpr int kw = 4 * KS;
    const int ulo_kw = uni(g.ulo) + (kw - 1);
    const int64_t n_out = rfl64(g.n_out), out_pitch = rfl64(g.out_pitch);
    const double SO_GLB* mats = (const double SO_GLB*)rfl64((int64_t)(uintptr_t)g.mats);
    long long* trace = (long long*)rfl64((int64_t)(uintptr_t)g.trace);
    TO SO_GLB* const y = (TO SO_GLB*)rfl64((int64_t)(uintptr_t)sh->y);
    const uint32_t fl_base = (uint32_t)(uintptr_t)sh->flags;
    const SO_LDS DCarrier& C0 = sh->ctl.car[0];
    const int64_t cs0 = rfl64(C0.cstride), df0 = rfl64(C0.df);
    const bool src32 = uni(g.src32) != 0;
    const bool x32 = sizeof(TO) == 4 && uni(g.x32) != 0;
    [[maybe_unused]] const bool ring32 = sizeof(TO) == 4 && uni(g.ring32) != 0;
    [[maybe_unused]] const bool sring = F32M && uni(g.sring) != 0;
    [[maybe_unused]] const int srow = ((lane & 15) / (ct < 8 ? ct : 8)) * (ct < 8 ? ct : 8);
    const bool single = uni((int)(C0.base != nullptr && C0.vec_ok && C0.dtype == (src32 ? SO_F32 : SO_F64))) && !(df0 & 1) && uni(g.fuse) >= -1 &&
                        (!src32 || uni(g.chunk) == 128) && (!uni(g.arr2) || rsos_two_ok(C0, uni(g.chunk)));
    const RsosGroup grp = rsos_group(sh, G, single, (int64_t)(rfl64((int64_t)(uintptr_t)C0.base) >> (src32 ? 2 : 3)), cs0, df0);
    const int gq = lane >> 4, n16 = lane & 15;
    double Dk[4], Tk[4], Ck[3];
    const int nkc = (uni(g.debug) & 131072) ? 3 : (2 * uni(g.nsec) + 3) / 4;
#pragma unroll
    for (int v = 0; v < 4; ++v) Dk[v] = F32M ? mats[(lane >> 4) * 64 + v * 16 + (lane & 15)] : mats[v * 64 + lane];
#pragma unroll
    for (int v = 0; v < 4; ++v) Tk[v] = F32M ? mats[(7 + (lane >> 4)) * 64 + v * 16 + (lane & 15)] : mats[(7 + v) * 64 + lane];
#pragma unroll
    for (int v = 0; v < 3; ++v) Ck[v] = mats[(11 + v) * 64 + lane];
    int cl;
    int nb0;
    {
        const int ri = n16 / ct;
        cl = ((grp.e0m + ri * grp.prMm) & 15) + gq;
        const int64_t ob = grp.ob0 + ri * grp.prL;
        nb0 = ob < 0 ? (int)((-ob) / 16) : 0;
    }
    const SO_LDS char* const ringc = (const SO_LDS char*)l.ring + (uint32_t)n16 * (uint32_t)rpitch * 8u;
    uint32_t yo0;
    int64_t ystep[4];
    const int64_t ybase_e = (int64_t)(grp.cg * ct) * out_pitch + grp.ob0;
#ifndef SO_Y_EARLY
#define SO_Y_EARLY 0
#endif
#ifndef SO_Y_SADDR
#define SO_Y_SADDR 1
#endif
#ifndef SO_ST_NT
#define SO_ST_NT ""
#endif
    const bool yfits = SO_Y_SADDR && uni((int)((((int64_t)(ct - 1) * out_pitch + (int64_t)(16 / ct) * grp.prL + 16) * (int64_t)sizeof(TO)) < ((int64_t)1 << 32)));
    int nbs_all;
    {
        int m = 0x7fffffff;
        int64_t off0 = 0;
#pragma unroll
        for (int v = 0; v < 4; ++v) {
            const int row = gq + 4 * v;
            const int ri = row / ct, cv = row % ct;
            const int64_t ob = grp.ob0 + ri * grp.prL;
            const int64_t off = ((int64_t)cv * out_pitch + (int64_t)ri * grp.prL + n16) * (int64_t)sizeof(TO);
            if (v == 0) off0 = off;
            ystep[v] = rfl64(off - off0);
            const int64_t tl = n_out - ob - n16;
            const int64_t nb = tl <= 0 ? 0 : (tl + 15) / 16;
            m = min(m, (int)(nb > 0x3fffffff ? 0x3fffffff : nb));
        }
        yo0 = (uint32_t)off0;
#pragma unroll
        for (int off = 32; off > 0; off >>= 1) m = min(m, __shfl_xor(m, off, 64));
        nbs_all = uni(m);
    }
    const int64_t slo = rfl64(g.store_lo);
    int nbl_max = 0;
    if (slo > grp.ob0) {
        const int64_t nb = (slo - grp.ob0 + 15) / 16;
        nbl_max = (int)(nb > 0x3fffffff ? 0x3fffffff : nb);
    }
    int nb0_any;
    {
        int m = nb0;
#pragma unroll
        for (int off = 32; off > 0; off >>= 1) m = max(m, __shfl_xor(m, off, 64));
        nb0_any = uni(m);
    }
    constexpr bool HELPABLE = HW && NY == 10 && CYC == 1;
    const bool help_on = HELPABLE && uni(g.help) != 0;
    const int hj = !help_on ? -1 : yi == kRsosHres0 ? 0 : yi == kRsosHres1 ? 1 : yi == kRsosHres2 ? 2 : -1;
    int hr = 0;
    int pi = 0, gi = yi;
    while (gi >= ngroups) {
        gi -= ngroups;
        ++pi;
    }
    int slot = yi % NX;
    int avail = 0;
    int wbm = -1;
    if (yi >= NB) flag_st(fl_base + 4 * (kRsosFlagYrd + yi), 0x7fffffff);
    uint32_t f_sseq = fl_base + 4 * kRsosFlagSseq, f_yrd = fl_base + 4 * (kRsosFlagYrd + yi);
    asm volatile("" : "+v"(f_sseq), "+v"(f_yrd));
    constexpr int NS = rsos_nss(NY);
    int sslot = yi % NS;
    int pb_ = -1, ppi_ = 0, pslot_ = 0;
    uint64_t ycur = (uint64_t)rfl64((int64_t)(uintptr_t)(y + (ybase_e + (int64_t)16 * yi))), ypend = 0;
    [[maybe_unused]] int cnt_in = 0, cnt_in_b = 0, cnt_st = 0, cnt_st_b = 0;
    [[maybe_unused]] const long long cyc0 = SO_RSOS_COUNT ? clock64() : 0;
    v4d payA = v4d{0.0, 0.0, 0.0, 0.0}, payB = v4d{0.0, 0.0, 0.0, 0.0};
    auto back_wait = [&](int sq, double (&sv)[3]) __attribute__((always_inline)) {
        int spins = 0;
        sq = uni(sq);
        if (sq < pb_ && !(debug & 8)) {
            if constexpr (SO_RSOS_COUNT) ++cnt_st_b;
            do {
                SO_SPIN_PAUSE(spins, 1, (debug & 32768) ? 4096 : (1 << 22));
                if constexpr (SO_RSOS_COUNT) ++cnt_st;
                sq = uni(flag_ld(f_sseq));
            } while (sq < pb_);
#pragma unroll
            for (int v = 0; v < 3; ++v) sv[v] = l.ss[pslot_ * 192 + v * 64 + lane];
        }
    };
    auto back_mfma = [&](const double (&sv)[3], v4d ay) __attribute__((always_inline)) {
        ay = __builtin_amdgcn_mfma_f64_16x16x4f64(sv[0], Ck[0], ay, 0, 0, 0);
        if (nkc > 1) ay = __builtin_amdgcn_mfma_f64_16x16x4f64(sv[1], Ck[1], ay, 0, 0, 0);
        if (nkc > 2) ay = __builtin_amdgcn_mfma_f64_16x16x4f64(sv[2], Ck[2], ay, 0, 0, 0);
        return ay;
    };
    auto back_store = [&](v4d ay, bool fresh) __attribute__((always_inline)) {
        if (debug & 1) return;
        const int64_t t0 = (int64_t)16 * pb_;
        const uint64_t yb = (uint64_t)rfl64((int64_t)ypend);
        if (fresh && yfits && sizeof(TO) == 8) asm volatile("s_nop 15\n\ts_nop 1" : "+v"(ay[0]), "+v"(ay[1]), "+v"(ay[2]), "+v"(ay[3])::"memory");
        auto out_index = [&](int v) __attribute__((always_inline)) { return grp.ob0 + (int64_t)((gq + 4 * v) / ct) * grp.prL + t0 + n16; };
        auto put = [&](int v, TO val) __attribute__((always_inline)) {
            if (yfits) {
                const uint64_t ybv = yb + (uint64_t)ystep[v];
                if constexpr (sizeof(TO) == 8) asm volatile("global_store_dwordx2 %0, %1, %2" SO_ST_NT ::"v"(yo0), "v"(val), "s"(ybv) : "memory");
                else asm volatile("global_store_dword %0, %1, %2" ::"v"(yo0), "v"(val), "s"(ybv) : "memory");
            } else {
                int row = gq + 4 * v;
                asm volatile("" : "+v"(row));
                y[(int64_t)(grp.cg * ct + row % ct) * out_pitch + grp.ob0 + (int64_t)(row / ct) * grp.prL + n16 + t0] = val;
            }
        };
        if (pb_ >= nbl_max && pb_ < nbs_all) {
#pragma unroll
            for (int v = 0; v < 4; ++v) put(v, (TO)ay[v]);
        } else {
#pragma unroll
            for (int v = 0; v < 4; ++v) {
                const int64_t m = out_index(v);
                if (m >= slo && m < n_out) put(v, (TO)ay[v]);
            }
        }
// ... 118 lines not shown
        bool early = false;
        v4d ay_early = pin;
        if (SO_Y_EARLY && pb_ >= 0 && ppi_ >= wp && (uni(sq) >= pb_ || (debug & 8))) {
            ay_early = back_mfma(sv, pin);
            early = true;
        }
        int pi2 = pi, gi2 = gi + NY;
        while (gi2 >= ngroups) {
            gi2 -= ngroups;
            ++pi2;
        }
        const int wb2 = b + NY < NB ? pi2 * M + jn - ulo_kw : 0x7fffffff;
        flag_st(f_yrd, wb2);
        if (b + NY < NB) {
            wbm += wb2 - wb;
            while (wbm >= RING) wbm -= RING;
        }
        if (b < nb0_any) {
            asm volatile("" ::: "memory");
            if (b < nb0) ax = v4d{0.0, 0.0, 0.0, 0.0};
            asm volatile("" : "+v"(ax));
        }
        rsos_stamp(trace, wave, b / NY, 2, 40);
        v4d dx = v4d{0.0, 0.0, 0.0, 0.0};
        if (!HELPABLE || hj < 0) {
#pragma unroll
            for (int v = 0; v < 4; ++v) dx = __builtin_amdgcn_mfma_f64_16x16x4f64(Dk[v], ax[v], dx, 0, 0, 0);
        }
        pout = __builtin_amdgcn_mfma_f64_16x16x4f64(ax[0], Tk[0], v4d{0.0, 0.0, 0.0, 0.0}, 0, 0, 0);
#pragma unroll
        for (int v = 1; v < 4; ++v) pout = __builtin_amdgcn_mfma_f64_16x16x4f64(ax[v], Tk[v], pout, 0, 0, 0);
        if (!HELPABLE || hj < 0) {
#pragma unroll
            for (int v = 0; v < 3; ++v) l.xs[slot * 192 + v * 64 + lane] = dx[v];
            flag_st(fl_base + 4 * (kRsosFlagXseq + slot), b + 1);
        } else {
#pragma unroll
            for (int v = 0; v < 3; ++v) l.xs[slot * 192 + v * 64 + lane] = ax[v];
            l.xh[(hj * kRsosHslots + hr) * 64 + lane] = ax[3];
            flag_st(fl_base + 4 * (kRsosFlagXh + hj), b + 1);
            hr = hr + 1 == kRsosHslots ? 0 : hr + 1;
        }
        if (early) back_store(ay_early, false);
        else if (pb_ >= 0) back(sq, sv, pin);
        rsos_stamp(trace, wave, b / NY, 3, 40);
        pb_ = b;
        ppi_ = pi;
        pslot_ = sslot;
        ypend = ycur;
        ycur += (uint64_t)(16 * NY) * sizeof(TO);
        sslot += NY % NS;
        if (sslot >= NS) sslot -= NS;
        pi = pi2;
        gi = gi2;
        slot += NY;
        if (slot >= NX) slot -= NX;
    };
    int cur = 0;
    auto last_back = [&]() __attribute__((always_inline)) {
        if (pb_ < 0) return;
        double sv[3];
        const int sq = flag_ld(f_sseq);
#pragma unroll
        for (int v = 0; v < 3; ++v) sv[v] = l.ss[pslot_ * 192 + v * 64 + lane];
        if (cur) back(sq, sv, payB);
        else back(sq, sv, payA);
    };
    if constexpr (CYC > 0) {
        const double SO_GLB* tab = (const double SO_GLB*)rfl64((int64_t)(uintptr_t)sh->tab);
        TapT treg[CYC][KS];
        int jec[CYC];
#pragma unroll
        for (int c = 0; c < CYC; ++c) {
            const int gc = (yi + c * NY) % ngroups;
            jec[c] = uni(sh->jend[gc]);
#pragma unroll
            for (int s = 0; s < KS; ++s) treg[c][s] = (TapT)tab[((size_t)gc * KS + s) * 64 + lane];
        }
        for (int b = yi; b < NB;) {
#pragma unroll
            for (int k = 0; k < 2 * CYC; ++k) {
                if (b < NB) {
                    if ((k & 1) == 0) block(b, treg[k % CYC], payA, payB, jec[k % CYC], jec[(k + 1) % CYC]);
                    else block(b, treg[k % CYC], payB, payA, jec[k % CYC], jec[(k + 1) % CYC]);
                    cur = (k & 1) ^ 1;
                }
                b += NY;
            }
        }
        last_back();
        if constexpr (SO_RSOS_COUNT) {
            if (lane == 0) {
                rsos_count_out(trace, wave, 0, 0, cnt_in);
                rsos_count_out(trace, wave, 0, 1, cnt_in_b);
                rsos_count_out(trace, wave, 0, 2, cnt_st);
                rsos_count_out(trace, wave, 0, 3, cnt_st_b);
                rsos_count_out(trace, wave, 0, 4, clock64() - cyc0);
            }
        }
    } else if constexpr (!F32M) {
        for (int b = yi; b < NB; b += NY) {
            double at[KS];
            const SO_LDS double* tp = l.taps + gi * KS * 64 + lane;
#pragma unroll
            for (int s = 0; s < KS; ++s) at[s] = tp[s * 64];
            int gn = gi + NY;
            while (gn >= ngroups) gn -= ngroups;
            const int je = uni(sh->jend[gi]), jn = uni(sh->jend[gn]);
            if (cur == 0) block(b, at, payA, payB, je, jn);
            else block(b, at, payB, payA, je, jn);
            cur ^= 1;
        }
        last_back();
    }
}


constexpr int rsos_nthreads(int nw) { return (nw == 17 ? 16 : nw) * 64; }
template <int KS, int NW, typename TO, int CYC>
__device__ __forceinline__ void rsos_body(const double* __restrict__ tab, const int* __restrict__ jend_g, const RsSos& g, TO* __restrict__ y,
                                          const RsGlobalTables& gsrc, int64_t G0, int64_t Gstep) {
    constexpr bool HW = NW == 17;
    constexpr int NT = rsos_nthreads(NW);
    constexpr int NY = NW >= 16 ? 10 : NW - 2, NL = NW == 16 ? 2 : 1, NX = 2 * NY + 1;
    extern __shared__ double lds_raw[];
    __shared__ RsosShared sh;
    const int wave = uni(threadIdx.x >> 6);
    {
        if (threadIdx.x == 0) {
            sh.g = g;
            sh.gcar = gsrc.car;
            sh.gops = gsrc.ops;
            sh.gleaves = gsrc.leaves;
            sh.y = (void*)y;
            sh.tab = tab;
        }
    }
    if constexpr (CYC == 0)
        for (int i = threadIdx.x; i < g.ngroups * KS * 64; i += NT) lds_raw[i] = tab[i];
    for (int i = threadIdx.x; i < g.ngroups; i += NT) sh.jend[i] = jend_g[i];
    {
        const int* src = reinterpret_cast<const int*>(gsrc.ctl);
        int* dst = reinterpret_cast<int*>(&sh.ctl);
        for (int i = threadIdx.x; i < (int)(sizeof(RsCtl) / 4); i += NT) dst[i] = src[i];
    }
    const int64_t ncg = g.nch / g.ct;
    const int64_t ngrp = ncg * ((g.nranges + g.rgs - 1) / g.rgs);
    double* const ss = lds_raw + (CYC > 0 ? 0 : (size_t)g.ngroups * KS * 64) + (size_t)16 * g.rpitch + (size_t)NX * 192;
    const int ru = g.ct < 8 ? g.ct : 8;
    for (int64_t G = G0; G < ngrp; G += Gstep) {
        __syncthreads();
        if (threadIdx.x < kRsosFlags) sh.flags[threadIdx.x] = 0;
        if (threadIdx.x < 192) ss[threadIdx.x] = 0.0;
        __syncthreads();
        if (wave == 0) {
            if (!(g.debug & 64)) {
                const int nk = (g.debug & 131072) ? 3 : (2 * g.nsec + 3) / 4;
                if (nk <= 1) rsos_chain<NY, 1>(&sh, lds_raw, G);
                else if (nk == 2) rsos_chain<NY, 2>(&sh, lds_raw, G);
                else rsos_chain<NY, 3>(&sh, lds_raw, G);
            }
        } else if (NW == 16 && (wave == 13 || wave == 14)) {
            if (!g.gsplit || (g.debug & 256) || g.src32) continue;
            const int q = wave - 13;
            if (g.arr2) {
                if constexpr (NL == 2) {
                    if (ru == 8) rsos_loader<NY, NL, 8, false, 0, 2, true>(&sh, lds_raw, G, q);
                    else if (ru == 4) rsos_loader<NY, NL, 4, false, 0, 2, true>(&sh, lds_raw, G, q);
                    else if (ru == 2) rsos_loader<NY, NL, 2, false, 0, 2, true>(&sh, lds_raw, G, q);
                }
            } else if (ru == 2) {
                if (g.rpitch == 770) rsos_loader<NY, NL, 2, false, 770 * 8, 2>(&sh, lds_raw, G, q);
                else if (g.rpitch == 642) rsos_loader<NY, NL, 2, false, 642 * 8, 2>(&sh, lds_raw, G, q);
                else rsos_loader<NY, NL, 2, false, 0, 2>(&sh, lds_raw, G, q);
            } else if (ru == 4) {
                if (g.rpitch == 770) rsos_loader<NY, NL, 4, false, 770 * 8, 2>(&sh, lds_raw, G, q);
                else if (g.rpitch == 642) rsos_loader<NY, NL, 4, false, 642 * 8, 2>(&sh, lds_raw, G, q);
                else rsos_loader<NY, NL, 4, false, 0, 2>(&sh, lds_raw, G, q);
            }
        } else if (wave == 4 || (NW == 16 && wave == 8)) {
            const int q = wave == 4 ? 0 : 1;
            if (g.debug & 256) continue;
            if (NW == 16 && g.gsplit && !g.src32 && ru == 8 && g.arr2) {
                rsos_loader<NY, NL, 8, false, 0, 1>(&sh, lds_raw, G, q);
                continue;
            }
            if (NW == 16 && g.gsplit && !g.src32 && (ru == 2 || ru == 4)) {
                if (ru == 2) {
                    if (g.rpitch == 770) rsos_loader<NY, NL, 2, false, 770 * 8, 1>(&sh, lds_raw, G, q);
                    else if (g.rpitch == 642) rsos_loader<NY, NL, 2, false, 642 * 8, 1>(&sh, lds_raw, G, q);
                    else rsos_loader<NY, NL, 2, false, 0, 1>(&sh, lds_raw, G, q);
                } else {
                    if (g.rpitch == 770) rsos_loader<NY, NL, 4, false, 770 * 8, 1>(&sh, lds_raw, G, q);
                    else if (g.rpitch == 642) rsos_loader<NY, NL, 4, false, 642 * 8, 1>(&sh, lds_raw, G, q);
                    else rsos_loader<NY, NL, 4, false, 0, 1>(&sh, lds_raw, G, q);
                }
                continue;
            }
            switch (ru) {
            case 8:
                if (g.src32 && g.rpitch == 770) rsos_loader<NY, NL, 8, true, 770 * 8>(&sh, lds_raw, G, q);
                else if (g.src32 && g.rpitch == 642) rsos_loader<NY, NL, 8, true, 642 * 8>(&sh, lds_raw, G, q);
                else if (g.src32) rsos_loader<NY, NL, 8, true>(&sh, lds_raw, G, q);
                else if (g.rpitch == 770) rsos_loader<NY, NL, 8, false, 770 * 8>(&sh, lds_raw, G, q);
                else if (g.rpitch == 642) rsos_loader<NY, NL, 8, false, 642 * 8>(&sh, lds_raw, G, q);
                else rsos_loader<NY, NL, 8, false>(&sh, lds_raw, G, q);
                break;
            case 4:
                if (g.src32) rsos_loader<NY, NL, 4, true>(&sh, lds_raw, G, q);
                else if (g.rpitch == 770) rsos_loader<NY, NL, 4, false, 770 * 8>(&sh, lds_raw, G, q);
                else if (g.rpitch == 642) rsos_loader<NY, NL, 4, false, 642 * 8>(&sh, lds_raw, G, q);
                else rsos_loader<NY, NL, 4, false>(&sh, lds_raw, G, q);
                break;
            case 2:
                if (g.src32) rsos_loader<NY, NL, 2, true>(&sh, lds_raw, G, q);
                else if (g.rpitch == 770) rsos_loader<NY, NL, 2, false, 770 * 8>(&sh, lds_raw, G, q);
                else if (g.rpitch == 642) rsos_loader<NY, NL, 2, false, 642 * 8>(&sh, lds_raw, G, q);
                else rsos_loader<NY, NL, 2, false>(&sh, lds_raw, G, q);
                break;
            default:
                if (g.src32) rsos_loader<NY, NL, 1, true>(&sh, lds_raw, G, q);
                else rsos_loader<NY, NL, 1, false>(&sh, lds_raw, G, q);
                break;
            }
        } else if (HW && wave == 12) {
            if (g.help && !(g.debug & 128)) rsos_helper<NY>(&sh, lds_raw);
        } else if (!(g.debug & 128))
            {
            if (NW >= 16 && wave > 12) continue;
            const int yi = NW == 16 ? (wave < 4 ? wave - 1 : wave < 8 ? wave - 2 : wave < 12 ? wave - 3 : 9) : wave - (wave > 4 ? 2 : 1);
            if constexpr (sizeof(TO) == 4 && CYC > 0) {
                if (g.f32m) {
                    rsos_ywave<KS, NY, NL, TO, CYC, true, HW>(&sh, lds_raw, G, yi);
                    continue;
                }
            }
            rsos_ywave<KS, NY, NL, TO, CYC, false, HW>(&sh, lds_raw, G, yi);
        }
    }
}

template <int KS, int NW, typename TO, int CYC>
__global__ __launch_bounds__(rsos_nthreads(NW)) void k_rsos(const double* __restrict__ tab, const int* __restrict__ jend_g, RsSos g,
                                                  TO* __restrict__ y, RsGlobalTables gsrc) {
    rsos_body<KS, NW, TO, CYC>(tab, jend_g, g, y, gsrc, (int64_t)blockIdx.x, (int64_t)gridDim.x);
}

template <int KS, int NW, typename TO, int CYC>
__global__ __launch_bounds__(rsos_nthreads(NW)) void k_rsos_batch(const RsosItem* __restrict__ items, int gpm) {
    const int it = (int)(blockIdx.x / (unsigned)gpm);
    const RsosItem I = items[it];
    rsos_body<KS, NW, TO, CYC>(I.tab, I.jend, I.g, (TO*)I.y, I.gsrc, (int64_t)(blockIdx.x % (unsigned)gpm), (int64_t)gpm);
}

constexpr size_t kRsosStaticLds = sizeof(RsosShared) + 64;

#if SO_RSOS_ONLY_KS != 0
template <int KS, int NW, typename TO, int CYC>
static void launch_rsos_k(const double* tab, const int* jend, const RsSos& g, void* y, const RsGlobalTables& gsrc, int grid, hipStream_t st) {
    const size_t lds = rsos_lds_bytes(g.ngroups, KS, g.rpitch, NW, CYC);
    static bool seen[64];
    if (first_use_on_device(seen))
        (void)hipFuncSetAttribute((const void*)k_rsos<KS, NW, TO, CYC>, hipFuncAttributeMaxDynamicSharedMemorySize, (int)rsos_lds_budget());
    hipLaunchKernelGGL((k_rsos<KS, NW, TO, CYC>), dim3((unsigned)grid), dim3(rsos_nthreads(NW)), lds, st, tab, jend, g, (TO*)y, gsrc);
}

template <int KS, int NW, typename TO>
static void launch_rsos_batch_k(const RsosItem* items, int nitems, int gpm, const RsSos& g0, hipStream_t st) {
    const size_t lds = rsos_lds_bytes(g0.ngroups, KS, g0.rpitch, NW, 1);
    static bool seen[64];
    if (first_use_on_device(seen))
        (void)hipFuncSetAttribute((const void*)k_rsos_batch<KS, NW, TO, 1>, hipFuncAttributeMaxDynamicSharedMemorySize, (int)rsos_lds_budget());
    hipLaunchKernelGGL((k_rsos_batch<KS, NW, TO, 1>), dim3((unsigned)(nitems * gpm)), dim3(rsos_nthreads(NW)), lds, st, items, gpm);
}

template <int KS, typename TO>
static int launch_rsos_t(const double* tab, const int* jend, const RsSos& g, void* y, const RsGlobalTables& gsrc, int grid, hipStream_t st) {
    if constexpr (SO_RSOS_ONLY_NW == 0 || SO_RSOS_ONLY_NW == 12) if (g.nwaves == 12) {
        switch (g.cyc) {
        case 0: launch_rsos_k<KS, 12, TO, 0>(tab, jend, g, y, gsrc, grid, st); return 0;
        case 1: launch_rsos_k<KS, 12, TO, 1>(tab, jend, g, y, gsrc, grid, st); return 0;
        case 2:
            if constexpr (KS <= 16) {
                launch_rsos_k<KS, 12, TO, 2>(tab, jend, g, y, gsrc, grid, st);
                return 0;
            }
            return -1;
        default: return -1;
        }
    }
    if constexpr (SO_RSOS_ONLY_NW == 0 || SO_RSOS_ONLY_NW == 16) if (g.nwaves == 16) {
        if (g.cyc != 1) return -1;
        launch_rsos_k<KS, 16, TO, 1>(tab, jend, g, y, gsrc, grid, st);
        return 0;
    }
    if constexpr (SO_RSOS_ONLY_NW == 0 || SO_RSOS_ONLY_NW == 17) if (g.nwaves == 17) {
        if (g.cyc != 1) return -1;
        launch_rsos_k<KS, 17, TO, 1>(tab, jend, g, y, gsrc, grid, st);
        return 0;
    }
    if constexpr (SO_RSOS_ONLY_NW == 0 || SO_RSOS_ONLY_NW == 8) if (g.nwaves == 8) {
        switch (g.cyc) {
        case 0: launch_rsos_k<KS, 8, TO, 0>(tab, jend, g, y, gsrc, grid, st); return 0;
        case 1: launch_rsos_k<KS, 8, TO, 1>(tab, jend, g, y, gsrc, grid, st); return 0;
        case 2: launch_rsos_k<KS, 8, TO, 2>(tab, jend, g, y, gsrc, grid, st); return 0;
        case 3:
            if constexpr (KS <= 20) {
                launch_rsos_k<KS, 8, TO, 3>(tab, jend, g, y, gsrc, grid, st);
                return 0;
            }
            return -1;
        case 5:
            if constexpr (KS <= 16) {
                launch_rsos_k<KS, 8, TO, 5>(tab, jend, g, y, gsrc, grid, st);
                return 0;
            }
            return -1;
        default: return -1;
        }
    }
    return -1;
}
#endif

#define SO_RSOS_ARGS const double *tab, const int *jend, const RsSos &g, void *y, const RsGlobalTables &gsrc, int grid, hipStream_t st
#if SO_RSOS_ONLY_KS > 0
#define SO_RSOS_CAT2(a, b) a##b
#define SO_RSOS_CAT(a, b) SO_RSOS_CAT2(a, b)
#if SO_RSOS_ONLY_F32
#define SO_RSOS_TAG f
#define SO_RSOS_TO float
#else
#define SO_RSOS_TAG d
#define SO_RSOS_TO double
#endif
int SO_RSOS_CAT(SO_RSOS_CAT(SO_RSOS_CAT(launch_rsos_ks, SO_RSOS_ONLY_KS), SO_RSOS_TAG), SO_RSOS_ONLY_NW)(SO_RSOS_ARGS) {
    return launch_rsos_t<SO_RSOS_ONLY_KS, SO_RSOS_TO>(tab, jend, g, y, gsrc, grid, st);
}
#if SO_RSOS_ONLY_KS == 4 && (SO_RSOS_ONLY_NW == 12 || SO_RSOS_ONLY_NW == 16)
int SO_RSOS_CAT(SO_RSOS_CAT(launch_rsos_batch4, SO_RSOS_TAG), SO_RSOS_ONLY_NW)(const RsosItem* items, int nitems, int gpm, const RsSos& g0, hipStream_t st) {
    launch_rsos_batch_k<4, SO_RSOS_ONLY_NW, SO_RSOS_TO>(items, nitems, gpm, g0, st);
    return 0;
}
#endif
#else
size_t rsos_lds_bytes(int ngroups, int ks, int rpitch, int nwaves, int cyc) {
    const int ny = nwaves >= 16 ? 10 : nwaves - 2, nx = 2 * ny + 1;
    return ((cyc > 0 ? 0 : (size_t)ngroups * ks * 64) + (size_t)16 * rpitch + (size_t)nx * 192 + (size_t)rsos_nss(ny) * 192 + 16 * 16 * 2 +
            (nwaves == 17 ? 3 * kRsosHslots * 64 : 0)) * 8;
}
size_t rsos_lds_budget() { return 160 * 1024 - kRsosStaticLds; }

#if SO_RSOS_ONLY_KS == 0
#define SO_RS(KS_) \
    int launch_rsos_ks##KS_##d12(SO_RSOS_ARGS); int launch_rsos_ks##KS_##d16(SO_RSOS_ARGS); int launch_rsos_ks##KS_##d8(SO_RSOS_ARGS); \
    int launch_rsos_ks##KS_##f12(SO_RSOS_ARGS); int launch_rsos_ks##KS_##f16(SO_RSOS_ARGS); int launch_rsos_ks##KS_##f8(SO_RSOS_ARGS); \
    int launch_rsos_ks##KS_##d17(SO_RSOS_ARGS); int launch_rsos_ks##KS_##f17(SO_RSOS_ARGS);
SO_RS(4) SO_RS(12) SO_RS(13) SO_RS(14) SO_RS(16) SO_RS(20)
#undef SO_RS
#endif
#if SO_RSOS_ONLY_KS == 0
int launch_rsos_batch4d12(const RsosItem*, int, int, const RsSos&, hipStream_t);
int launch_rsos_batch4f12(const RsosItem*, int, int, const RsSos&, hipStream_t);
int launch_rsos_batch4d16(const RsosItem*, int, int, const RsSos&, hipStream_t);
int launch_rsos_batch4f16(const RsosItem*, int, int, const RsSos&, hipStream_t);
#endif
int launch_rsos_batch(const RsosItem* items, int nitems, int gpm, const RsSos& g0, hipStream_t st) {
    if (nitems <= 0 || gpm <= 0) return 0;
    if (g0.ks != 4 || g0.cyc != 1 || (g0.nwaves != 12 && g0.nwaves != 16)) return -1;
#if SO_RSOS_ONLY_KS == 0
    if (g0.nwaves == 12) return g0.out_f32 ? launch_rsos_batch4f12(items, nitems, gpm, g0, st) : launch_rsos_batch4d12(items, nitems, gpm, g0, st);
    return g0.out_f32 ? launch_rsos_batch4f16(items, nitems, gpm, g0, st) : launch_rsos_batch4d16(items, nitems, gpm, g0, st);
#else
    if (g0.nwaves == 12) {
        if (g0.out_f32) launch_rsos_batch_k<4, 12, float>(items, nitems, gpm, g0, st);
        else launch_rsos_batch_k<4, 12, double>(items, nitems, gpm, g0, st);
    } else {
        if (g0.out_f32) launch_rsos_batch_k<4, 16, float>(items, nitems, gpm, g0, st);
        else launch_rsos_batch_k<4, 16, double>(items, nitems, gpm, g0, st);
    }
    return 0;
#endif
}
// ... 25 lines not shown
```

### signaloperators.jl_amd/csrc/plan.h

```cpp
#pragma once
#include <cstdint>
#include <string>
#include <vector>

#include "../../include/sigops.h"

namespace so {

int design_iir(int type, double f1, double f2, double fs, int method, int order, double ripple,
               std::vector<double>& sos, double& gain, std::string& err);
int design_iir_zpk(int type, double f1, double f2, double fs, int method, int order, double ripple,
                   std::vector<double>& z, std::vector<double>& p, double& k, std::string& err);
int zpk_to_sos(const double* z, int nz, const double* p, int np, double k, std::vector<double>& sos, double& gain,
               std::string& err);
int tf_to_sos(const double* b, int nb, const double* a, int na, std::vector<double>& sos, double& gain, double& resid,
              std::string& err);
int tf_zero_input(const double* b, int nb, const double* a, int na, const double* si0, int nsi, double* out, int64_t cap,
                  int64_t& used, std::string& err);
int design_resample_rational(int64_t num, int64_t den, std::vector<double>& h, std::string& err);
int design_resample_arbitrary(double rate, int nphi, std::vector<double>& h, std::string& err);

int resample_positions(double fs_in, double fs_out, double rate, int nphi, const double* h, int hlen,
                       int64_t n_out, int64_t* j, int32_t* p, double* alpha, int64_t* nfix, int64_t* nbaked);

int rtc_compile_check(const std::string& body, std::string& err);
void rtc_wait_idle();
void rtc_shutdown();

struct Plan;
Plan* plan_create(const so_node_t* nodes, int32_t n_nodes, int32_t root, const so_out_desc_t* out,
                  int32_t device, int& status, std::string& err);
int plan_execute(Plan* p, void* out, void* stream, std::string& err);
int plan_check(Plan* p, void* stream, std::string& err);
int plan_set_array(Plan* p, int32_t node_index, const void* data, std::string& err);
int64_t plan_nframes(const Plan* p);
void plan_stats(const Plan* p, so_stats_t* st);
void plan_set_profiling(Plan* p, int mode);
int64_t plan_counter(const Plan* p, int which);
int plan_step_info(const Plan* p, int index, so_step_info_t* info);
void plan_destroy(Plan* p);

}
```

### signaloperators.jl_amd/csrc/sigops_internal.h

```cpp
#pragma once
#include <cstdint>

namespace so {

enum OpCode : int32_t {
    OP_CONST = 0,
    OP_LOAD = 1,
    OP_SCALAR = 2,
    OP_FUNC = 3,
    OP_RAMP = 4,
    OP_ADD = 5,
    OP_SUB = 6,
    OP_MUL = 7,
    OP_DIV = 8,
    OP_NEG = 9,
    OP_ROUND32 = 10,
    OP_STOREF = 11,
    OP_LOADF = 12
};

enum LeafMode : int32_t { LM_PLAIN = 0, LM_CYCLE = 1, LM_MIRROR = 2 };

struct DOp {
    int32_t code;
// ... 132 lines not shown
    int32_t nch;
    int32_t ntiles;
    int32_t nlev;
    int32_t kt;
    int32_t vec_in, vec_out;
    int32_t bt;
    int32_t debug;
};

struct RsGeom {
    int64_t n_in, n_out;
    int64_t m0;
    int64_t j0;
    int64_t L, M;
    double delta, c0;
    int64_t c0i;
    int32_t arbitrary;
    int32_t exact;
    int32_t nphi, taps, nch;
    int32_t in_dtype, out_dtype;
    int64_t in_pitch, out_pitch;
};

struct RsTiled {
    RsGeom g;
    int32_t ct;
    int32_t tile_out;
    int32_t tile_in;
    int32_t pitch;
    int64_t ntiles;
    int32_t pair;
    int32_t pad_;
};

struct RsArb {
    RsGeom g;
    int32_t ct;
    int32_t nc;
    int32_t ringf;
    int32_t zrows;
    int32_t nranges;
    int32_t dma_ok, vec_out, depth, debug;
    int32_t no, pad_;
    int64_t bpr;
    int64_t nbatches;
    uint32_t* err;
};

struct RsFix {
    int64_t m;
    int64_t j;
    int32_t p;
    int32_t pad;
    double alpha;
};
struct RsFixArgs {
    const RsFix* fix;
    int64_t nfix;
    const double* pfb;
    const double* dpfb;
    int64_t n_in;
    int32_t taps, nch;
    int32_t stage_dtype;
    int32_t out_dtype;
    const DCarrier* car;
    const DOp* ops;
    const DLeaf* leaves;
    int32_t ncar, in_dtype;
    const void* x;
    int64_t in_pitch;
    void* y;
    int64_t out_pitch;
};

struct RsPeriodic {
    int64_t n_in, n_out;
    int64_t L, M;
    int64_t nperiods;
    int32_t pt, ct;
    int32_t rows;
    int32_t f32m;
    int32_t ngroups;
    int32_t kw;
    int32_t tile_len;
    int32_t lds_pitch;
    int32_t jlo;
    int32_t nch;
    int32_t vec_ok;
    int32_t nwaves;
    int32_t ptshift;
    int32_t ncompute;
    int32_t grid;
    int32_t pad;
    int32_t nslots;
    int32_t fslots;
    int32_t fpitch;
    int32_t nload;
    int32_t ftwo;
    int32_t out_f32;
    int32_t ga;
    int32_t arr2;
    int32_t nstate, ksw;
    const double* wtab;
    double* vper;
    int64_t in_pitch, out_pitch;
    long long* trace;
    uint32_t* nf;
};
constexpr int kRsTraceIters = 48, kRsTraceStamps = 8;
constexpr uint32_t kRsNfCap = 2047;

struct RsPerFixup {
    RsPeriodic g;
    const double* tab;
    const int* jend;
    const int* jrel;
    int32_t taps, out_f32;
    RsGlobalTables gsrc;
    void* y;
};
constexpr int kRsTwoBases = 128;
constexpr int kRsTwoDoubles = 128 + 2 * 2 * kRsTwoBases;

struct RsSos {
    int64_t n_in, n_out;
    int64_t L, M;
    int64_t pr;
    int32_t wp;
    int32_t nranges;
    int32_t ngroups;
    int32_t ks;
    int32_t ulo;
    int32_t ct, rgs;
    int32_t nch;
    int32_t nwaves;
    int32_t ring;
    int32_t rpitch;
    int32_t chunk;
    int32_t depth;
    int32_t nsec;
    int32_t fuse;
    int32_t fuse_sine;
    int32_t out_f32;
    int32_t src32;
    int32_t ring32;
    int32_t x32;
    int32_t f32m;
    int32_t sring;
    int32_t gsplit;
    int32_t help;
    int32_t debug;
    int32_t cyc;
    int32_t arr2;
    int32_t pad_;
    int64_t out_pitch;
    int64_t store_lo;
    const double* mats;
    int32_t* bad;
    long long* trace;
    uint32_t* err;
};
constexpr int kRsosTraceIters = 96;

struct RsosItem {
    RsSos g;
    const double* tab;
    const int* jend;
    void* y;
    RsGlobalTables gsrc;
};

struct RsFixup {
    RsSos g;
    const double* tab;
    const int* jend;
    const int* jrel;
    int32_t taps;
    int32_t pad;
    SosCoefs cf;
    RsGlobalTables gsrc;
    void* y;
};

struct RsRows {
    int64_t n_in, n_out;
    int64_t L, M;
    int64_t nperiods;
    int32_t taps;
    int32_t ct, pb;
    int32_t jlo;
    int32_t tile_len;
    int32_t pitch;
    int32_t nch;
    int32_t debug;
    int32_t kw, ngroups, pbshift;
    int32_t threads;
    int64_t in_pitch, out_pitch;
};

}
```

### signaloperators.jl_amd/csrc/stages.cpp

```cpp
#include "plan_impl.h"

namespace so {

static int env_int(const char* name, int dflt) {
    const char* ev = std::getenv(name);
    return ev ? std::atoi(ev) : dflt;
}

Mat matmul(const Mat& a, const Mat& b, int D) {
    Mat c((size_t)D * D, 0.0);
    for (int i = 0; i < D; ++i)
        for (int k = 0; k < D; ++k) {
            double v = a[(size_t)i * D + k];
            if (v == 0.0) continue;
            for (int j = 0; j < D; ++j) c[(size_t)i * D + j] += v * b[(size_t)k * D + j];
        }
    return c;
}
double maxabs(const Mat& a) {
    double m = 0;
    for (double v : a) {
        if (!std::isfinite(v)) return INFINITY;
        m = std::max(m, std::fabs(v));
    }
// ... 1286 lines not shown
    const size_t leaves_before = leaves.size();
    for (size_t i = 0; i < cs.size(); ++i) {
        DCarrier& c = cs[i];
        std::vector<DOp>& fcode = fcodes[i];
        int dmax = 2;
        c.nslots = (int)monos_all[i].size();
        for (size_t k = 0; k < monos_all[i].size(); ++k) {
            int ei = monos_all[i][k], r32 = 0;
            for (;;) {
                const Expr& ex = exprs[ei];
                if (ex.op == E_RETYPE) ei = ex.a;
                else if (ex.op == E_ROUND32) { r32 = 0x100; ei = ex.a; }
                else if (ex.op == E_ADD && is_const(ex.a, 0.0)) ei = ex.b;
                else if ((ex.op == E_ADD || ex.op == E_SUB) && is_const(ex.b, 0.0)) ei = ex.a;
                else break;
            }
            const int eop = exprs[ei].op;
            const int kind = eop == E_CONST ? OP_CONST : eop == E_SCALAR ? OP_SCALAR : eop == E_FUNC ? OP_FUNC : eop == E_RAMP ? OP_RAMP : -1;
            if (kind < 0) {
                leaves.resize(leaves_before);
                leaf_array_node.resize(leaves_before);
                { if (std::getenv("SIGOPS_DEBUG_PLAN")) std::fprintf(stderr, "[sigops] carrier fusion rejected (#%d)\n", 5); return false; }
            }
            c.slot_leaf[k] = add_leaf(exprs[ei]);
            c.slot_kind[k] = kind | r32;
            leafset.insert(c.slot_leaf[k]);
            std::map<int, int> none;
            gen(monos_all[i][k], fcode, none, fcode, false);
            fcode.push_back(DOp{OP_STOREF, (int)k});
            dmax = std::max(dmax, depth(monos_all[i][k]));
        }
        c.depth = dmax;
        nops_total += fcode.size();
        for (auto& o : fcode)
            if (o.code <= OP_RAMP) leafset.insert(o.arg);
        if (dmax > 2 || nops_total > (size_t)kCtlOps || leafset.size() > (size_t)kCtlLeaves) {
            leaves.resize(leaves_before);
            leaf_array_node.resize(leaves_before);
            { if (std::getenv("SIGOPS_DEBUG_PLAN")) std::fprintf(stderr, "[sigops] carrier fusion rejected (#%d)\n", 6); return false; }
        }
    }
    for (size_t i = 0; i < cs.size(); ++i) {
        cs[i].frame_pc = (int)ops.size();
        cs[i].frame_len = (int)fcodes[i].size();
        ops.insert(ops.end(), fcodes[i].begin(), fcodes[i].end());
    }
    if (ga) {
        auto same_leaf = [&](int a, int b) {
            const DLeaf &x = leaves[a], &y = leaves[b];
            return x.base == y.base && x.fstride == y.fstride && x.cstride == y.cstride && x.df == y.df && x.dc == y.dc &&
                   x.modn == y.modn && x.v0 == y.v0 && x.v1 == y.v1 && x.v2 == y.v2 && x.sf == y.sf && x.sc == y.sc &&
                   x.dtype == y.dtype && x.mode == y.mode && x.flag == y.flag && x.buf == y.buf;
        };
        for (size_t i = 1; i < cs.size(); ++i)
            if (cs[i].slot_kind[0] != cs[0].slot_kind[0] || !same_leaf(cs[i].slot_leaf[0], cs[0].slot_leaf[0])) ga = false;
        if (!ga) {
            leaves.resize(leaves_before);
            leaf_array_node.resize(leaves_before);
            ops.resize(ops.size() - nops_total);
            if (std::getenv("SIGOPS_DEBUG_PLAN")) std::fprintf(stderr, "[sigops] carrier fusion rejected (#%d)\n", 7);
            return false;
        }
        for (size_t i = 0; i < cs.size(); ++i) {
            cs[i].pad_ = (i == 0 ? 1 : 2) + (ga_add ? 2 : 0);
            cs[i].nsteps = 0;
            cs[i].dtype = SO_F32;
        }
    }
    out = cs;
    return true;
}

RsCtl Plan::make_ctl(const Stage& S) const {
    RsCtl ctl{};
    std::map<int, int> leafmap;
    for (const DCarrier& c0 : S.carriers) {
        if (ctl.ncar >= kCtlCar) throw PlanError{SO_ERR_RUNTIME, "internal: carrier control block overflow"};
        DCarrier c = c0;
        c.frame_pc = ctl.nops;
        for (int k = 0; k < c0.frame_len; ++k) {
            DOp o = ops[c0.frame_pc + k];
            if (o.code <= OP_RAMP) {
                auto it = leafmap.find(o.arg);
                if (it == leafmap.end()) {
                    if (ctl.nleaves >= kCtlLeaves) throw PlanError{SO_ERR_RUNTIME, "internal: leaf control block overflow"};
                    ctl.leaves[ctl.nleaves] = leaves[o.arg];
                    if (o.code == OP_SCALAR) ctl.leaves[ctl.nleaves].flag = 0;
                    it = leafmap.emplace(o.arg, ctl.nleaves++).first;
                }
                o.arg = it->second;
            }
            if (ctl.nops >= kCtlOps) throw PlanError{SO_ERR_RUNTIME, "internal: op control block overflow"};
            ctl.ops[ctl.nops++] = o;
        }
        for (int k = 0; k < c0.nslots; ++k) {
            auto it = leafmap.find(c0.slot_leaf[k]);
            if (it == leafmap.end()) {
                if (ctl.nleaves >= kCtlLeaves) throw PlanError{SO_ERR_RUNTIME, "internal: leaf control block overflow"};
                ctl.leaves[ctl.nleaves] = leaves[c0.slot_leaf[k]];
                if ((c0.slot_kind[k] & 0xff) == OP_SCALAR) ctl.leaves[ctl.nleaves].flag = 0;
                it = leafmap.emplace(c0.slot_leaf[k], ctl.nleaves++).first;
            }
            c.slot_leaf[k] = it->second;
        }
        ctl.car[ctl.ncar++] = c;
    }
    return ctl;
}


void Plan::batch_sos_stages() {
    if (std::getenv("SIGOPS_SOS_NOBATCH")) return;
    std::map<std::pair<int, int>, std::vector<int>> kinds;
    std::vector<int> order;
    for (size_t i = 0; i < stages.size(); ++i)
        if (stages[i].need > 0) order.push_back((int)i);
    std::sort(order.begin(), order.end(), [&](int a, int b) { return stages[a].node < stages[b].node; });
    for (int sid : order) {
        const Stage& S = stages[sid];
        if (S.kind != ST_SOS || S.onepass || S.sg.exact || S.xscan || S.under_norm || S.pre_stage >= 0 || S.groups.size() != 1 ||
            S.in_array_node < 0 || S.pw_step >= 0 || S.sg.nchunks < 1 || S.rsos_src >= 0)
            continue;
        kinds[{S.groups[0].nsec, nodes[S.node].dtype}].push_back(sid);
    }
    for (auto& kv : kinds) {
        if (kv.second.size() < 2) continue;
        SosBatch B;
        B.members = kv.second;
        B.nsec = kv.first.first;
        B.dtype = kv.first.second;
        int64_t chans = 0;
        for (int sid : B.members) chans += stages[sid].sg.nch;
        if (!std::getenv("SIGOPS_SOS_BATCH_KEEPCHUNKS"))
            for (int sid : B.members) {
                Stage& S = stages[sid];
                sos_chunking(sid, S.sg.n, S.sg.nch, nodes[S.node].dtype, S.groups, false, std::max<int64_t>(1, kSosSequences / chans));
            }
        B.desc_buf = raw_buf((B.members.size() + 1) * sizeof(SosDesc));
        {
            int off = 0;
            for (int sid : B.members) {
                B.bad_off.push_back(off);
                off += stages[sid].sg.nch;
            }
            B.bad_buf = raw_buf((size_t)std::max(off, 1) * 4);
        }
        for (int sid : B.members) stages[sid].batch = (int)batches.size();
        if (std::getenv("SIGOPS_DEBUG_PLAN"))
            std::fprintf(stderr, "[sigops] %zu IIR stages of %d sections share their launches\n", B.members.size(), B.nsec);
        batches.push_back(std::move(B));
    }
}

static void rsos_block_matrices(const SosCoefs& cf, std::vector<double>& mats) {
    const int ns = cf.nsec, D = 2 * ns, B = 16;
    std::vector<double> Tm(B * B, 0.0), Cm(B * 12, 0.0), Dm(12 * B, 0.0), Am(12 * 12, 0.0);
    for (int col = 0; col < B + D; ++col) {
        std::vector<double> st(D, 0.0);
        if (col >= B) st[col - B] = 1.0;
        for (int t = 0; t < B; ++t) {
            double v = col == t ? 1.0 : 0.0;
            for (int f = 0; f < ns; ++f) {
                const double xi = v;
                v = st[2 * f] + cf.b0[f] * xi;
                st[2 * f] = st[2 * f + 1] + cf.b1[f] * xi - cf.a1[f] * v;
                st[2 * f + 1] = cf.b2[f] * xi - cf.a2[f] * v;
            }
            v *= cf.gain;
            if (col < B) Tm[t * B + col] = v;
            else Cm[t * 12 + (col - B)] = v;
        }
        for (int d = 0; d < D; ++d) {
            if (col < B) Dm[d * B + col] = st[d];
            else Am[d * 12 + (col - B)] = st[d];
        }
    }
    mats.assign((size_t)14 * 64, 0.0);
    for (int lane = 0; lane < 64; ++lane) {
        const int i = lane & 15, kq = lane >> 4;
        for (int v = 0; v < 4; ++v) {
            const int k = 4 * v + kq;
            mats[(size_t)(0 + v) * 64 + lane] = i < 12 ? Dm[i * B + k] : 0.0;
            mats[(size_t)(7 + v) * 64 + lane] = Tm[i * B + k];
            if (v < 3) {
                mats[(size_t)(4 + v) * 64 + lane] = i < 12 ? Am[i * 12 + k] : 0.0;
                mats[(size_t)(11 + v) * 64 + lane] = Cm[i * 12 + k];
            }
        }
    }
}

void Plan::fuse_resample_sos() {
    if (std::getenv("SIGOPS_NO_RSOS")) return;
    auto env_int = [](const char* name, int dflt) {
        const char* ev = std::getenv(name);
        return ev ? std::atoi(ev) : dflt;
    };
    for (size_t i2 = 0; i2 < stages.size(); ++i2) {
        Stage& S2 = stages[i2];
        if (S2.kind != ST_SOS || S2.onepass || S2.need <= 0 || S2.groups.size() != 1 || S2.groups[0].nsec > 6 ||
            S2.in_buf < 0 || S2.in_array_node >= 0 || S2.in_offset != S2.base || S2.pw_step >= 0 || S2.sg.exact || (S2.xscan && !S2.under_norm) ||
            (S2.under_norm && (S2.norm_df != 0 || S2.base != 0 || std::getenv("SIGOPS_NORM_EXACT_FILT"))) || S2.src_op || S2.batch >= 0 || S2.pre_stage >= 0 ||
            (nodes[S2.node].dtype != SO_F64 && nodes[S2.node].dtype != SO_F32) || S2.in_frames != S2.need - S2.base)
            continue;
        const bool pure32 = nodes[S2.node].dtype == SO_F32;
        if (pure32 && std::getenv("SIGOPS_RSOS_NO32")) continue;
        if (S2.base > 0 && std::getenv("SIGOPS_RSOS_NOWINDOWS")) continue;
        int i3 = -1;
        for (size_t j = 0; j < stages.size(); ++j)
            if (stages[j].kind == ST_RESAMPLE && stages[j].out_buf == S2.in_buf) i3 = (int)j;
        if (i3 < 0 || i3 == alias_stage || stages[i3].win_off >= 0) continue;
        Stage& S3 = stages[i3];
        const RsPeriodic& rp = S3.rp;
        if (S3.base > S2.base) continue;
        if (rp.nstate || nodes[S3.node].dtype != nodes[S2.node].dtype || !S3.fix_host.empty() || S3.need < S2.need || (int)S3.carriers.size() > kCtlCar)
            continue;
        struct AltGuard {
            Stage& S;
            std::vector<DCarrier> car;
            int pw;
            bool armed;
            ~AltGuard() {
                if (armed) {
                    S.carriers = car;
                    S.pw_step = pw;
                }
            }
        } alt{S3, S3.carriers, S3.pw_step, false};
        if (!rp.arr2 && !S3.alt_carriers.empty() && S3.pw_step >= 0 && S3.in_buf >= 0 && !std::getenv("SIGOPS_RSOS_NO_ARR2")) {
            S3.carriers = S3.alt_carriers;
            S3.pw_step = -1;
            alt.armed = true;
        }
        bool two_arrays = false;
        if (rp.arr2 || alt.armed) {
            const bool ok = !pure32 && nodes[S2.node].dtype == SO_F64 && S3.carriers.size() == 1 && S3.carriers[0].nsteps == 1 &&
                            (S3.carriers[0].arg[0] & kCarArr2) && !(S3.carriers[0].arg[0] & 0x200) && S3.carriers[0].dtype == SO_F64 &&
                            S3.carriers[0].dtype2 == SO_F64 && nodes[S2.node].nch % 2 == 0 &&
                            (S3.carriers[0].op[0] == OP_ADD || S3.carriers[0].op[0] == OP_SUB || S3.carriers[0].op[0] == OP_MUL) &&
                            !std::getenv("SIGOPS_RSOS_NO_ARR2");
            if (!ok) continue;
            two_arrays = true;
        }
        if (pure32) {
            bool plain = nodes[nodes[S3.node].kids[0]].dtype == SO_F32 && rp.ga == 0;
            for (auto& c : S3.carriers)
                if (c.nsteps != 0 || c.pad_ != 0 || c.dtype != SO_F32) plain = false;
            if (!plain) continue;
        }
        const bool plain_src = S3.carriers.empty() && (S3.in_buf >= 0 || S3.in_array_node >= 0);
        if (S3.carriers.empty() && !plain_src) continue;
        int64_t Lp = rp.L, Mp = rp.M;
        int ngp = rp.ngroups, kwp = rp.kw, jlop = rp.jlo;
        bool own_tab = false;
        std::vector<double> own_taps;
        std::vector<int> own_jend;
        std::vector<int64_t> own_jr;
        const bool blocks_ok = S3.periodic && Lp > 0 && Lp % 16 == 0 && (int64_t)ngp * 16 == Lp && ngp <= 256;
        if (!S3.rg.arbitrary && (!blocks_ok || ngp > 10) && !std::getenv("SIGOPS_RSOS_NOOWNTAB")) {
            const RsGeom& rg = S3.rg;
            const so_node_t& nd3 = nodes[S3.node].nd;
            const double* h = (const double*)nd3.p0;
            const int hlen = nd3.i2;
            const int64_t tmin = 16 / std::__gcd<int64_t>(rg.L, 16);
            bool found = false;
            for (int64_t m : {1, 2, 3, 5}) {
                const int64_t Ls = rg.L * tmin * m, Ms = rg.M * tmin * m;
                const int ng = (int)(Ls / 16);
                if (Ls > 4096 || (ng != 1 && ng != 2 && ng != 3 && ng != 5 && ng != 6 && ng != 10)) continue;
                std::vector<int64_t> jr((size_t)Ls);
                std::vector<int> prr((size_t)Ls);
                for (int64_t r = 0; r < Ls; ++r) {
                    const int64_t qi = rg.c0i + r * rg.M;
                    jr[(size_t)r] = qi / rg.nphi;
                    prr[(size_t)r] = (int)(qi % rg.nphi);
                }
                std::vector<int> jend((size_t)ng);
                int64_t maxspan = 0;
                for (int gi = 0; gi < ng; ++gi) {
                    jend[(size_t)gi] = (int)jr[(size_t)gi * 16 + 15];
                    maxspan = std::max(maxspan, jr[(size_t)gi * 16 + 15] - jr[(size_t)gi * 16]);
                }
                const int ksneed = (int)((rg.taps + maxspan + 3) / 4);
                int ksc = 0;
                for (int k : {12, 14, 16, 20})
                    if (!ksc && k >= ksneed) ksc = k;
                if (std::getenv("SIGOPS_DEBUG_PLAN"))
                    std::fprintf(stderr, "[sigops] k_rsos own taps: L %lld M %lld x %lld -> %d blocks, taps %d span %lld: %d k-steps (%d)\n",
                                 (long long)rg.L, (long long)rg.M, (long long)(tmin * m), ng, rg.taps, (long long)maxspan, ksneed, ksc);
                if (!ksc) break;
                const int kw = 4 * ksc;
                int jlo = jend[0] - (kw - 1);
                jlo -= ((jlo % 4) + 4) % 4;
                std::vector<double> tab((size_t)ng * kw * 16, 0.0);
                for (int gi = 0; gi < ng; ++gi)
                    for (int rr = 0; rr < 16; ++rr)
                        for (int kk = 0; kk < kw; ++kk) {
                            const int64_t r = (int64_t)gi * 16 + rr;
                            const int64_t age = jr[(size_t)r] - ((int64_t)jend[(size_t)gi] - (kw - 1) + kk);
                            if (age < 0 || age >= rg.taps) continue;
                            const int64_t hi = prr[(size_t)r] + (int64_t)rg.nphi * age;
                            tab[((size_t)gi * kw + kk) * 16 + rr] = hi < hlen ? h[hi] : 0.0;
                        }
                Lp = Ls;
                Mp = Ms;
                ngp = ng;
                kwp = kw;
                jlop = jlo;
                own_taps.swap(tab);
                own_jend.swap(jend);
                own_jr = jr;
                own_tab = found = true;
                break;
            }
            (void)found;
        }
        if (!own_tab && (!blocks_ok || !S3.periodic)) continue;
        if (S3.base % Lp != 0 || Mp >= (1 << 20)) continue;
        if (!own_tab && !std::getenv("SIGOPS_RSOS_NOTRIM") && !S3.tab_host.empty() && (size_t)ngp * kwp * 16 == S3.tab_host.size()) {
            int lead = kwp;
            for (int gi = 0; gi < ngp && lead > 0; ++gi)
                for (int kk = 0; kk < lead; ++kk) {
                    bool z = true;
                    for (int rr = 0; rr < 16 && z; ++rr) z = S3.tab_host[((size_t)gi * kwp + kk) * 16 + rr] == 0.0;
                    if (!z) {
                        lead = kk;
                        break;
                    }
                }
            int ksc = 0;
            for (int k : {12, 13, 14, 16, 20})
                if (!ksc && 4 * k >= kwp - lead) ksc = k;
            if (ksc && 4 * ksc < kwp) {
                const int drop = kwp - 4 * ksc, kw = 4 * ksc;
                own_taps.assign((size_t)ngp * kw * 16, 0.0);
                for (int gi = 0; gi < ngp; ++gi)
                    for (int kk = 0; kk < kw; ++kk)
                        for (int rr = 0; rr < 16; ++rr)
                            own_taps[((size_t)gi * kw + kk) * 16 + rr] = S3.tab_host[((size_t)gi * kwp + kk + drop) * 16 + rr];
                own_jend = S3.jend_host;
                kwp = kw;
                own_tab = true;
                if (std::getenv("SIGOPS_DEBUG_PLAN"))
                    std::fprintf(stderr, "[sigops] k_rsos: %d leading zero slots in every group's window: %d k-steps instead of %d\n", lead, ksc,
                                 (kw + drop) / 4);
            }
        }
        const int ks = kwp / 4;
        if (!(ks == 12 || ks == 13 || ks == 14 || ks == 16 || ks == 20)) continue;
        bool ok = true;
        const bool was_ga = rp.ga != 0;
        for (auto& c : S3.carriers)
            if ((c.pad_ != 0) != was_ga) ok = false;
        if (was_ga && std::getenv("SIGOPS_RSOS_NO32")) ok = false;
        for (auto& L : leaves)
            if (L.buf == S2.in_buf) ok = false;
        for (size_t j = 0; j < stages.size(); ++j) {
            if (j != i2 && stages[j].in_buf == S2.in_buf) ok = false;
            if (j != i2)
                for (auto& c : stages[j].carriers)
                    if (c.buf == S2.in_buf) ok = false;
        }
        if (!ok) continue;
        const SosCoefs& cf = S2.groups[0];
        const int D = 2 * cf.nsec;
        const int nch = nodes[S2.node].nch;
        const int64_t need = S2.need - S3.base, L = Lp;
        const int64_t store_lo = S2.base - S3.base;
        const int64_t nperiods = (need + L - 1) / L;
        int64_t wp = 1;
        {
            const double tol = std::ldexp(1.0, -std::abs(env_int("SIGOPS_RSOS_WTOL", S2.under_norm ? 70 : 56)));
            const Mat P = matpow(sos_state_matrix(cf), L, D);
            Mat cur = P;
            while (!(maxabs(cur) < tol) && wp < 1000000 && std::isfinite(maxabs(cur))) {
                cur = matmul(cur, P, D);
                ++wp;
            }
            if (!(maxabs(cur) < tol)) continue;
        }
        int ct = 1;
        for (int c : {16, 8, 4, 2})
            if (nch % c == 0) {
                ct = c;
                break;
            }
        const int rgs = 16 / ct;
        const int64_t ncg = nch / ct;
        const int cus = env_int("SIGOPS_RSOS_GRID", 256);
        int64_t rgroups = std::max<int64_t>(1, cus / ncg);
        int64_t nranges = rgroups * rgs;
        const int64_t min_pr = std::max<int64_t>(1, wp);
        if (nperiods / nranges < min_pr) nranges = std::max<int64_t>(rgs, nperiods / min_pr / rgs * rgs);
        if (const char* ev = std::getenv("SIGOPS_RSOS_RANGES")) nranges = std::max<int64_t>(1, std::atoll(ev));
        int64_t pr = (nperiods + nranges - 1) / nranges;
        if (ct < 8 && !std::getenv("SIGOPS_RSOS_NOALIGNPR")) {
            const int64_t mlt = 16 / std::__gcd<int64_t>(Mp % 16 == 0 ? 16 : Mp % 16, 16);
            if (pr % mlt != 0 && pr >= 8 * mlt) pr = (pr + mlt - 1) / mlt * mlt;
        }
        nranges = (nperiods + pr - 1) / pr;
        const int64_t ngrp = ncg * ((nranges + rgs - 1) / rgs);
        if ((pr + wp) * ngp >= (1 << 30) || (pr + wp) * Mp >= ((int64_t)1 << 30)) continue;
        if (const char* ev = std::getenv("SIGOPS_RSOS_MINGROUPS")) {
            if (ngrp < std::atoll(ev)) continue;
        } else {
            const double unit_cost = ct >= 8 ? 1.0 : ct == 4 ? 1.1 : ct == 2 ? 1.15 : 3.2;
            const double t_fused = (double)((ngrp + cus - 1) / cus) * (double)((pr + wp) * ngp) * 0.30 * unit_cost * (ks + 14) / 28.0 + 15.0;
            const double t_two = 8.0e-6 * (double)need * nch + 95.0;
            if (std::getenv("SIGOPS_DEBUG_PLAN"))
                std::fprintf(stderr, "[sigops] k_rsos estimate: fused %.0f us (%lld groups, %lld + %lld periods), two kernels %.0f us\n", t_fused,
                             (long long)ngrp, (long long)pr, (long long)wp, t_two);
            if (t_fused > t_two) continue;
        }
        RsSos g{};
        g.n_in = S3.rg.n_in;
        g.n_out = need;
        g.store_lo = store_lo;
        g.L = L;
        g.M = Mp;
        g.pr = pr;
        g.wp = (int32_t)wp;
        g.nranges = (int32_t)nranges;
        g.ngroups = ngp;
        g.ks = ks;
        g.ulo = jlop;
        g.ct = ct;
        g.rgs = rgs;
        g.nch = nch;
        g.chunk = env_int("SIGOPS_RSOS_CHUNK", 128) == 64 ? 64 : 128;
        g.depth = std::max(1, std::min(4, env_int("SIGOPS_RSOS_DEPTH", 4)));
        g.nsec = cf.nsec;
        g.debug = env_int("SIGOPS_RSOS_DEBUG", 0);
        {
            auto cyc_of = [&](int nw) { return g.ngroups / std::__gcd(nw >= 16 ? 10 : nw - 2, g.ngroups); };
            auto fits = [&](int nw) {
                const int c = cyc_of(nw);
                return nw == 12 ? ((c == 1 || c == 2) && c * ks <= 32) : ((c == 1 || c == 2 || c == 3 || c == 5) && c * ks <= 80);
            };
            int nw = fits(12) ? 12 : fits(8) ? 8 : 12;
            const bool stepped = was_ga || (!plain_src && !S3.carriers.empty() && S3.carriers[0].nsteps > 0);
            if ((ct == 2 || (ct == 4 && !was_ga && nodes[S2.node].dtype == SO_F64 && !std::getenv("SIGOPS_RSOS_NOGSPLIT"))) && stepped && nw == 12 &&
                cyc_of(16) == 1 && ks <= 16)
                nw = 16;
            if (const char* ev = std::getenv("SIGOPS_RSOS_NWAVES")) nw = std::atoi(ev) == 8 ? 8 : (std::atoi(ev) == 16 || std::atoi(ev) == 17) && cyc_of(16) == 1 && ks <= 16 ? std::atoi(ev) : 12;
            if (two_arrays) {
                if (!(cyc_of(16) == 1 && ks <= 16)) continue;
                nw = 16;
            }
            g.nwaves = nw;
            g.cyc = (nw >= 16 || fits(nw)) && !std::getenv("SIGOPS_RSOS_LDSTAPS") ? cyc_of(nw) : 0;
            const bool inst = nw == 12 ? (g.cyc == 0 || g.cyc == 1 || (g.cyc == 2 && ks <= 16))
                            : nw >= 16 ? g.cyc == 1
                                       : (g.cyc == 0 || g.cyc == 1 || g.cyc == 2 || (g.cyc == 3 && ks <= 20) || (g.cyc == 5 && ks <= 16));
            if (!inst) continue;
        }
        {
            const int ny = g.nwaves >= 16 ? 10 : g.nwaves - 2;
            const int64_t span = (int64_t)(2 * ny - 1) * ((16 * Mp + L - 1) / L + 1) + kwp + 16 + 2 * g.chunk;
            int ring = 4096;
            while (ring >= 128 && rsos_lds_bytes(g.ngroups, ks, ring + 2, g.nwaves, g.cyc) > rsos_lds_budget()) ring -= 128;
            if (const char* ev = std::getenv("SIGOPS_RSOS_RING")) ring = std::min(ring, std::max(128, std::atoi(ev) / 128 * 128));
            if (std::getenv("SIGOPS_DEBUG_PLAN"))
                std::fprintf(stderr, "[sigops] k_rsos: ring %d frames (needs %lld), LDS %zu of %zu\n", ring, (long long)span,
                             rsos_lds_bytes(g.ngroups, ks, ring + 2, g.nwaves, g.cyc), rsos_lds_budget());
            if (ring < 128 || ring < span) continue;
            g.ring = ring;
            g.rpitch = ring + 2;
        }
        if (plain_src) {
            DCarrier c{};
            c.a = 0;
            c.b = S3.in_frames;
            c.dtype = nodes[nodes[S3.node].kids[0]].dtype == SO_F32 ? SO_F32 : SO_F64;
            c.array_node = S3.in_array_node;
            c.buf = S3.in_array_node >= 0 ? -1 : S3.in_buf;
            c.df = S3.in_offset;
            c.cstride = S3.in_array_node >= 0 ? (nch == 1 ? 0 : S3.in_pitch) : -1;
            S3.carriers.push_back(c);
            S3.car_buf = raw_buf(sizeof(DCarrier));
            S3.ctl_buf = raw_buf(sizeof(RsCtl));
        }
        if (was_ga) {
            for (size_t i = 0; i < S3.carriers.size(); ++i) {
                DCarrier& c = S3.carriers[i];
                c.pad_ = 0;
                c.nsteps = 1;
                if (i > 0) c.dtype = SO_F64;
            }
            S3.rp.ga = 0;
            g.src32 = 1;
        } else
            g.src32 = S3.carriers[0].dtype == SO_F32 && S3.carriers[0].nsteps == 0 ? 1 : 0;
        g.x32 = pure32 ? 1 : 0;
        {
            const DCarrier& c0 = S3.carriers[0];
            g.fuse = -1;
            if (two_arrays) {
                g.fuse = c0.op[0] == OP_MUL ? 0 : c0.op[0] == OP_ADD ? 1 : ((c0.arg[0] & 0x100) ? 3 : 2);
                g.fuse_sine = 0;
                g.arr2 = 1;
            } else if (c0.nsteps == 1 && (c0.arg[0] & 0x2ff) == 0 && c0.nslots >= 1 &&
                (c0.op[0] == OP_MUL || c0.op[0] == OP_ADD || c0.op[0] == OP_SUB)) {
                g.fuse = c0.op[0] == OP_MUL ? 0 : c0.op[0] == OP_ADD ? 1 : ((c0.arg[0] & 0x100) ? 3 : 2);
                const DLeaf& L0 = leaves[c0.slot_leaf[0]];
                const int kind = c0.slot_kind[0];
                if (kind == OP_FUNC && L0.mode == SO_FN_SIN && L0.sf == 1) g.fuse_sine = 1;
                else if (kind == OP_CONST || kind == OP_SCALAR) g.fuse_sine = 0;
                else g.fuse = -2;
            } else if (c0.nsteps > 0)
                g.fuse = -2;
        }
        g.gsplit = g.nwaves == 16 && !g.src32 && g.fuse >= 0 && (g.arr2 || ((ct == 2 || ct == 4) && !std::getenv("SIGOPS_RSOS_NOGSPLIT"))) ? 1 : 0;
        g.ring32 = g.src32 && g.fuse == -1 && pure32 && !std::getenv("SIGOPS_RSOS_NO_RING32") ? 1 : 0;
        g.help = g.nwaves == 17 ? 1 : 0;
        g.f32m = g.src32 && g.fuse >= -1 && g.cyc > 0 && !std::getenv("SIGOPS_RSOS_NO_F32MFMA") && !std::getenv("SIGOPS_RSOS_NO_RING32") ? 1 : 0;
        S2.rs = g;
        S2.rsos_src = i3;
        S2.carriers.clear();
        {
            const std::vector<int64_t>& jr = own_jr.empty() ? S3.per_j : own_jr;
            const std::vector<int>& je = own_tab ? own_jend : S3.jend_host;
            S2.rsos_jrel_host.clear();
            if ((int64_t)jr.size() >= Lp && (int64_t)je.size() >= ngp) {
                S2.rsos_jrel_host.resize((size_t)Lp);
                for (int64_t r = 0; r < Lp; ++r) S2.rsos_jrel_host[(size_t)r] = (int)(jr[(size_t)r] - je[(size_t)(r / 16)]);
                S2.rsos_jrel_buf = raw_buf(S2.rsos_jrel_host.size() * 4);
                S2.rsos_taps = S3.rg.taps;
            }
        }
        if (own_tab) {
            S2.rsos_tab_host.swap(own_taps);
            S2.rsos_jend_host.swap(own_jend);
            S2.rsos_tab_buf = raw_buf(S2.rsos_tab_host.size() * 8);
            S2.rsos_jend_buf = raw_buf(S2.rsos_jend_host.size() * 4);
        }
        S2.rsos_grid = (int)std::min<int64_t>(ngrp, cus);
        rsos_block_matrices(cf, S2.rsos_mats_host);
        S2.rsos_mats_buf = raw_buf(S2.rsos_mats_host.size() * 8);
        if (S2.bad_buf < 0) S2.bad_buf = raw_buf((size_t)nch * 4);
        S3.fused_away = true;
        if (alt.armed) {
            alt.armed = false;
            bufs[S3.in_buf].bytes = 0;
        }
        if (std::getenv("SIGOPS_DEBUG_PLAN"))
            std::fprintf(stderr,
                         "[sigops] resampler + IIR fused (k_rsos): %lld ranges of %lld periods (+%lld warm-up), %lld groups of %d ch x %d ranges, "
                         "ks=%d ring=%d chunk=%d waves=%d cyc=%d fuse=%d/%d\n",
                         (long long)nranges, (long long)pr, (long long)wp, (long long)ngrp, ct, rgs, ks, g.ring, g.chunk, g.nwaves, g.cyc,
                         g.fuse, g.fuse_sine);
    }
}

void Plan::fuse_plain_sos() {
    if (std::getenv("SIGOPS_NO_RSOS") || std::getenv("SIGOPS_NO_PLAIN_RSOS")) return;
    auto env_int = [](const char* name, int dflt) {
        const char* ev = std::getenv(name);
        return ev ? std::atoi(ev) : dflt;
    };
    const int cus = env_int("SIGOPS_RSOS_GRID", 256);
    auto fit = [&](size_t i2, int gpm, RsSos& g, double& cost) -> bool {
        Stage& S2 = stages[i2];
        const int dt = nodes[S2.node].dtype;
        if (dt != SO_F64 && dt != SO_F32) return false;
        const DCarrier& c0 = S2.carriers[0];
        const bool pure32 = dt == SO_F32;
        if (pure32 && (c0.nsteps != 0 || c0.dtype != SO_F32)) return false;
        if (!pure32 && c0.dtype != SO_F64) return false;
        const SosCoefs& cf = S2.groups[0];
        const int D = 2 * cf.nsec;
        const int nch = nodes[S2.node].nch;
        const int64_t need = S2.need, L = 160;
        const int ngp = 10, ks = 4, kw = 16;
        const int64_t nperiods = (need + L - 1) / L;
        int64_t wp = 1;
        {
            const double tol = std::ldexp(1.0, -std::abs(env_int("SIGOPS_PLAIN_WTOL", 70)));
            const Mat P = matpow(sos_state_matrix(cf), L, D);
            Mat cur = P;
            while (!(maxabs(cur) < tol) && wp < 1000000 && std::isfinite(maxabs(cur))) {
                cur = matmul(cur, P, D);
                ++wp;
            }
            if (!(maxabs(cur) < tol)) return false;
        }
        int ct = 1;
        for (int c : {16, 8, 4, 2})
            if (nch % c == 0) {
                ct = c;
                break;
            }
        const int rgs = 16 / ct;
        const int64_t ncg = nch / ct;
        if (gpm > 0 && ncg > gpm) return false;
        int64_t rgroups = gpm > 0 ? gpm / ncg : std::max<int64_t>(1, cus / ncg);
        int64_t nranges = rgroups * rgs;
        const int64_t min_pr = std::max<int64_t>(1, 4 * wp);
        if (nperiods / nranges < min_pr) nranges = std::max<int64_t>(rgs, nperiods / min_pr / rgs * rgs);
        if (const char* ev = std::getenv("SIGOPS_RSOS_RANGES"))
            if (gpm == 0) nranges = std::max<int64_t>(1, std::atoll(ev));
        const int64_t pr = (nperiods + nranges - 1) / nranges;
        nranges = (nperiods + pr - 1) / pr;
        const int64_t ngrp = ncg * ((nranges + rgs - 1) / rgs);
        if ((pr + wp) * ngp >= (1 << 30) || (pr + wp) * L >= ((int64_t)1 << 30)) return false;
        const bool stepped_few = (ct == 2 || ct == 4) && !pure32 && c0.nsteps == 1 && !std::getenv("SIGOPS_RSOS_NOGSPLIT");
        const int plain_nw = env_int("SIGOPS_PLAIN_NWAVES", stepped_few ? 16 : 12) == 16 ? 16 : 12;
        const double unit_cost = stepped_few && plain_nw == 16 ? (ct == 4 ? 1.16 : 1.22) : ct >= 8 ? 1.0 : ct == 4 ? 1.19 : ct == 2 ? 1.4 : 3.4;
        cost = (double)((pr + wp) * ngp) * 0.197 * unit_cost;
        if (gpm > 0) {
            cost *= (double)((ngrp + gpm - 1) / gpm);
        } else if (const char* ev = std::getenv("SIGOPS_RSOS_MINGROUPS")) {
            if (ngrp < std::atoll(ev)) return false;
        } else {
            const double t_fused = (double)((ngrp + cus - 1) / cus) * cost + 15.0;
            const double nsamp = (double)need * nch;
            const double t_three = (nsamp < 1e8 ? 4.4e-6 * nsamp + 25.0 : 3.4e-6 * nsamp + 110.0) * (pure32 ? 0.9 : 1.0) * (c0.nsteps > 0 ? 1.1 : 1.0) *
                                   (S2.under_norm ? 1.6 : 1.0);
            if (std::getenv("SIGOPS_DEBUG_PLAN"))
                std::fprintf(stderr, "[sigops] single-pass IIR estimate: %.0f us (%lld groups, %lld + %lld periods), three passes %.0f us\n", t_fused,
                             (long long)ngrp, (long long)pr, (long long)wp, t_three);
            if (t_fused > t_three) return false;
        }
        g = RsSos{};
        g.n_in = S2.in_frames;
        g.n_out = need;
        g.store_lo = 0;
        g.L = L;
        g.M = L;
        g.pr = pr;
        g.wp = (int32_t)wp;
        g.nranges = (int32_t)nranges;
        g.ngroups = ngp;
        g.ks = ks;
        g.ulo = 0;
        g.ct = ct;
        g.rgs = rgs;
        g.nch = nch;
        g.chunk = 128;
        g.depth = std::max(1, std::min(4, env_int("SIGOPS_RSOS_DEPTH", 4)));
        g.nsec = cf.nsec;
        g.debug = env_int("SIGOPS_RSOS_DEBUG", 0);
        g.nwaves = plain_nw;
        g.cyc = 1;
        {
            const int ny = 10;
            const int64_t span = (int64_t)(2 * ny - 1) * 17 + kw + 16 + 2 * g.chunk;
            int ring = 4096;
            while (ring >= 128 && rsos_lds_bytes(g.ngroups, ks, ring + 2, g.nwaves, g.cyc) > rsos_lds_budget()) ring -= 128;
            if (const char* ev = std::getenv("SIGOPS_RSOS_RING")) ring = std::min(ring, std::max(128, std::atoi(ev) / 128 * 128));
            if (ring < 128 || ring < span) return false;
            g.ring = ring;
            g.rpitch = ring + 2;
        }
        g.help = 0;
        g.src32 = pure32 ? 1 : 0;
        g.x32 = pure32 ? 1 : 0;
        g.ring32 = pure32 && !std::getenv("SIGOPS_RSOS_NO_RING32") ? 1 : 0;
        g.gsplit = 0;
        g.fuse = -1;
        if (c0.nsteps == 1 && (c0.arg[0] & 0x2ff) == 0 && c0.nslots >= 1 && (c0.op[0] == OP_MUL || c0.op[0] == OP_ADD || c0.op[0] == OP_SUB)) {
            g.fuse = c0.op[0] == OP_MUL ? 0 : c0.op[0] == OP_ADD ? 1 : ((c0.arg[0] & 0x100) ? 3 : 2);
            const DLeaf& L0 = leaves[c0.slot_leaf[0]];
            const int kind = c0.slot_kind[0];
            if (kind == OP_FUNC && L0.mode == SO_FN_SIN && L0.sf == 1) g.fuse_sine = 1;
            else if (kind == OP_CONST || kind == OP_SCALAR) g.fuse_sine = 0;
            else g.fuse = -2;
        } else if (c0.nsteps > 0)
            g.fuse = -2;
        g.gsplit = g.nwaves == 16 && !g.src32 && g.fuse >= 0 && (ct == 2 || ct == 4) && !std::getenv("SIGOPS_RSOS_NOGSPLIT") ? 1 : 0;
        return true;
    };
    auto commit = [&](size_t i2, const RsSos& g) {
        Stage& S2 = stages[i2];
        const int ngp = g.ngroups, kw = 16;
        const int64_t L = g.L;
        S2.rsos_tab_host.assign((size_t)ngp * kw * 16, 0.0);
        S2.rsos_jend_host.assign((size_t)ngp, 0);
        for (int gi = 0; gi < ngp; ++gi) {
            S2.rsos_jend_host[(size_t)gi] = 16 * gi + 15;
            for (int kk = 0; kk < kw; ++kk) S2.rsos_tab_host[((size_t)gi * kw + kk) * 16 + kk] = 1.0;
        }
        S2.rsos_tab_buf = raw_buf(S2.rsos_tab_host.size() * 8);
        S2.rsos_jend_buf = raw_buf(S2.rsos_jend_host.size() * 4);
        S2.rsos_jrel_host.resize((size_t)L);
        for (int64_t r = 0; r < L; ++r) S2.rsos_jrel_host[(size_t)r] = (int)(r % 16) - 15;
        S2.rsos_jrel_buf = raw_buf(S2.rsos_jrel_host.size() * 4);
        S2.rsos_taps = 1;
        S2.rs = g;
        S2.rsos_src = (int)i2;
        const int64_t ngrp = (int64_t)(g.nch / g.ct) * ((g.nranges + g.rgs - 1) / g.rgs);
// ... 209 lines not shown
```

### signaloperators.jl_amd/engine.py

```python
import ctypes as C

import numpy as np

from . import _capi as K
from . import signals as S
from .lowering import lower, _DT

Array = np.ndarray


def process_sink_params(x):
    x = S._assignal(x)
    n = S.nframes(x)
    if n is None:
        S.error("Unknown number of frames in signal.")
    if S.isknowninf(n):
        S.error("Cannot store infinite signal.")
    return x


def _timeslice(x):
    if isinstance(x, S.ArraySig):
        return x.data
    d = _timeslice(x.signal)
    n = d.shape[0]
    L = x.resolvelen()
    if x.kind == "until":
        return d[: min(max(L, 0), n)]
    return d[min(max(L, 0), n):]


def _is_datacut(x):
    if isinstance(x, S.ArraySig):
        return True
    return isinstance(x, S.CutApply) and x.evaltrait == "data" and _is_datacut(x.signal)


def _root(x):
    if isinstance(x, S.ArraySig):
        if x.container is not None:
            return 2, x
        if S._is_torch(x.data):
            return 0, x
        return (1 if x.fs is None else 0), x
    best = None
    for c in getattr(x, "children", ()):
        r = _root(c)
        if best is None or r[0] > best[0]:
            best = r
    return best or (0, None)


def _refineroot(x):
    pr, leaf = _root(x)
    if pr == 2:
        return leaf.container
    if pr == 1:
        return Array
    return tuple


class Plan:

    def __init__(self, x, result_shape, result_dtype, strides, is_device, device=0, rng=None):
        self.lowered = lower(x, nframes_out=result_shape[0], rng=rng)
        self.desc = K.so_out_desc_t(dtype=_DT[np.dtype(result_dtype)], nch=result_shape[1],
                                    nframes=result_shape[0], frame_stride=strides[0],
                                    chan_stride=strides[1], is_device=1 if is_device else 0)
        self.handle = C.c_void_p()
        L = K.lib()
        st = L.so_plan_create(self.lowered.nodes, self.lowered.n, self.lowered.root,
                              C.byref(self.desc), device, C.byref(self.handle))
        if st != 0:
            raise S.ErrorException(K.last_error())

    def execute(self, out_ptr, stream=None):
        st = K.lib().so_plan_execute(self.handle, C.c_void_p(out_ptr), C.c_void_p(stream or 0))
        if st != 0:
            raise S.ErrorException(K.last_error())
        self._unchecked = (stream or 0) if self.desc.is_device else None

    def check(self, stream=None):
        self._unchecked = None
        st = K.lib().so_plan_check(self.handle, C.c_void_p(stream or 0))
        if st != 0:
            raise S.ErrorException(K.last_error())

    def set_array(self, k, data):
        idx, sig = self.lowered.array_nodes[k]
        if hasattr(data, "data_ptr"):
            ptr = data.data_ptr()
        else:
            ptr = data.ctypes.data
        self._keep_arrays = getattr(self, "_keep_arrays", {})
        self._keep_arrays[k] = data
        st = K.lib().so_plan_set_array(self.handle, idx, C.c_void_p(ptr))
        if st != 0:
            raise S.ErrorException(K.last_error())

    def set_profiling(self, on=True):
        K.lib().so_plan_set_profiling(self.handle, int(on))

    def stats(self):
        s = K.so_stats_t()
        K.lib().so_plan_stats(self.handle, C.byref(s))
        return {f[0]: (getattr(s, f[0]).decode() if f[0] == "dominant_kernel" else getattr(s, f[0]))
                for f in K.so_stats_t._fields_}

    def counters(self):
        L = K.lib()
        return {"graph_replays": L.so_plan_counter(self.handle, 0), "graph_captures": L.so_plan_counter(self.handle, 1),
                "direct_executes": L.so_plan_counter(self.handle, 2), "fused_mfmas_per_block": L.so_plan_counter(self.handle, 3)}

    def steps(self):
        out = []
        info = K.so_step_info_t()
        n = K.lib().so_plan_step_info(self.handle, 0, C.byref(info))
        for i in range(n):
            K.lib().so_plan_step_info(self.handle, i, C.byref(info))
            out.append({"name": info.name.decode(), "algorithmic_bytes": info.algorithmic_bytes,
                        "ms": info.ms, "launches": info.launches})
        return out

    def close(self):
        if self.handle:
            err = None
            if getattr(self, "_unchecked", None) is not None:
                if K.lib().so_plan_check(self.handle, C.c_void_p(self._unchecked)) != 0:
                    err = K.last_error()
                self._unchecked = None
            K.lib().so_plan_destroy(self.handle)
            self.handle = C.c_void_p()
            if err is not None:
                raise S.ErrorException(err)

    def __del__(self):
        try:
            self.close()
        except Exception:
            pass


def _result_fields(result):
    if S._is_torch(result):
        shape = tuple(result.shape)
        st = result.stride()
        if len(shape) == 1:
            shape, st = (shape[0], 1), (st[0], 0)
        dt = {"torch.float32": S.F32, "torch.float64": S.F64}[str(result.dtype)]
        return shape, dt, st, result.is_cuda, result.data_ptr()
    shape = result.shape
    item = result.itemsize
    if result.ndim == 1:
        return (shape[0], 1), result.dtype, (result.strides[0] // item or 1, 0), False, result.ctypes.data
    return shape, result.dtype, (result.strides[0] // item or 1, result.strides[1] // item), False, \
        result.ctypes.data


def sink_into(result, x, *, device=0, rng=None, stream=None):
    x = S._assignal(x)
    shape, dt, strides, is_dev, ptr = _result_fields(result)
    n = S.nframes(x)
    if n is not None and not S.isknowninf(n) and n < shape[0]:
        S.error(f"Signal is too short to fill buffer of length {shape[0]}.")
    x = S.ToChannels(x, shape[1])
    plan = Plan(x, shape, dt, strides, is_dev, device=device, rng=rng)
    try:
        plan.execute(ptr, stream)
        if is_dev:
            plan.check(stream)
    finally:
        plan.close()
    return result


def sink(x, to=None, *, device=0, rng=None):
    if to is None and (isinstance(x, type) or x is tuple or (isinstance(x, str) and x == "torch")):
        to_ = x
        return S.Curried(lambda y: sink(y, to_, device=device, rng=rng))
    x = process_sink_params(x)
    if to is None:
        to = _refineroot(x)
    if _is_datacut(x) and to is Array:
        return _timeslice(x)
    n = S.nframes(x)
    dt = x.dtype
    if dt == S.I64:
        S.error("the HIP engine sinks Float32/Float64 signals only (SURVEY.md §8(b)); "
                "integer signals take the stock CPU sink")
    if to == "torch":
        import torch

        tdt = torch.float32 if dt == S.F32 else torch.float64
        res = torch.empty((x.nch, n), dtype=tdt, device=f"cuda:{device}").t()
        sink_into(res, x, device=device, rng=rng)
        return res, x.fs
    res = np.empty((n, x.nch), dtype=dt, order="F")
    sink_into(res, x, device=device, rng=rng)
    if isinstance(to, type) and hasattr(to, "initsink"):
        if x.fs is None:
            S.error("Unknown frame rate: array-type sinks carry a frame rate")
        return to.initsink(res, x.fs)
    return res if to is Array else (res, x.fs)


def stream(x, blocksize, to=None, *, device=0):
    from . import lowering as LW
    from .units import frames

    x = S._assignal(x)
    blocksize = int(blocksize)
    if blocksize <= 0:
        S.error("stream: blocksize must be positive")
    n = S.nframes(x)
    if n is None:
        S.error("Unknown number of frames in signal.")
    finite = not S.isknowninf(n)
    if to is None:
        to = _refineroot(x)
    cache = {"device": f"cuda:{device}"}
    pos = 0
    while not finite or pos < n:
        m = blocksize if not finite else min(blocksize, n - pos)
        blk = S.Until(S.After(x, pos * frames) if pos else x, m * frames)
        prev, LW._device_cache = LW._device_cache, cache
        try:
            res = sink(blk, to, device=device)
        finally:
            LW._device_cache = prev
        yield res
        pos += m


class BlockStream:

    def __init__(self, pipeline, fs, nch=1, dtype=np.float64, history=1 << 16, device=0):
        import torch

        from .units import inHz

        self.pipeline = pipeline
        self.fs = inHz(fs)
        self.nch = int(nch)
        self.dtype = np.dtype(dtype)
        self.tdt = torch.float32 if self.dtype == np.float32 else torch.float64
        self.history = int(history)
        self.device = device
        self.dev = f"cuda:{device}"
        self.cap = 0
        self.buf = None
        self.start = 0
        self.received = 0
        self.emitted = 0
        self.closed = False

    def _append(self, block):
        import torch

        if hasattr(block, "data_ptr"):
            b = block.to(self.dev, self.tdt)
        else:
            b = torch.from_numpy(np.ascontiguousarray(np.asarray(block, dtype=self.dtype))).to(self.dev)
        if b.dim() == 1:
            b = b[:, None]
        if b.shape[1] != self.nch:
# ... 168 lines not shown
```

Baseline: 29.23 billion.

## Replace resampler+IIR warm-up periods with a precomputed linear projection via MFMA

Instead of running the warm-up periods through the recursive resample+SOS chain for each range, the planner precomputes on the host one matrix that maps the raw input window directly to the filter state. Each y-wave then computes a partial product of that matrix with input samples using f64 MFMA. The chain wave sums these partials into the initial state, and when the source is a sine it adds a closed-form sine correction. This removes the serial warm-up blocks from every range group, at the cost of a larger coefficient table, extra global loads, and added planning and flag-synchronisation complexity.

```diff
diff --git a/include/sigops.h b/include/sigops.h
--- a/include/sigops.h
+++ b/include/sigops.h
@@ -206,7 +206,13 @@
     SO_COUNTER_GRAPH_REPLAYS = 0,
     SO_COUNTER_GRAPH_CAPTURES = 1,
     SO_COUNTER_DIRECT_EXECUTES = 2,
-    SO_COUNTER_FUSED_MFMAS_PER_BLOCK = 3
+    SO_COUNTER_FUSED_MFMAS_PER_BLOCK = 3,
+    SO_COUNTER_WPROJ = 4,
+    SO_COUNTER_RSOS_RANGE_PERIODS = 5,
+    SO_COUNTER_RSOS_WARMUP_PERIODS = 6,
+    SO_COUNTER_RSOS_PERIOD_INPUTS = 7,
+    SO_COUNTER_WPROJ_FRAMES = 8,
+    SO_COUNTER_WPROJ_FIRST = 9
 } so_counter_t;
 int64_t so_plan_counter(const so_plan_t* plan, int32_t which);
 
@@ -270,6 +276,10 @@
                               int32_t hlen, int64_t n_out, int64_t* j, int32_t* p, double* alpha,
                               int64_t* nfix, int64_t* nbaked);
 
+int32_t so_rsos_wproj_matrix(const double* sos, int32_t nsec, double gain, const double* tab, const int32_t* jend,
+                             int32_t ngroups, int32_t kw, int64_t m, int32_t wp, double* v, int32_t capacity,
+                             int32_t* j0, int32_t* k);
+
 #if defined(__GNUC__)
 #pragma GCC visibility pop
 #endif
diff --git a/signaloperators.jl_amd/_capi.py b/signaloperators.jl_amd/_capi.py
--- a/signaloperators.jl_amd/_capi.py
+++ b/signaloperators.jl_amd/_capi.py
@@ -66,7 +66,7 @@
            "so_plan_nframes", "so_plan_execute", "so_plan_check", "so_plan_set_array", "so_plan_stats",
            "so_plan_set_profiling", "so_plan_destroy", "so_design_iir",
            "so_design_resample_rational", "so_design_resample_arbitrary",
-           "so_resample_positions", "so_plan_step_info", "so_design_iir_zpk", "so_zpk_to_sos", "so_tf_to_sos", "so_tf_zero_input", "so_plan_counter",
+           "so_resample_positions", "so_plan_step_info", "so_design_iir_zpk", "so_zpk_to_sos", "so_tf_to_sos", "so_tf_zero_input", "so_plan_counter", "so_rsos_wproj_matrix",
            "so_rtc_compile_check", "so_rtc_wait_idle", "so_rtc_shutdown", "so_comm_unique_id", "so_comm_create", "so_comm_allgather", "so_comm_reduce_sum", "so_comm_last_error", "so_comm_destroy"]
 
 _lib = None
@@ -158,6 +158,10 @@
     L.so_comm_destroy.argtypes = [C.c_void_p]
     L.so_plan_counter.restype = C.c_int64
     L.so_plan_counter.argtypes = [C.c_void_p, C.c_int32]
+    L.so_rsos_wproj_matrix.restype = C.c_int32
+    L.so_rsos_wproj_matrix.argtypes = [C.POINTER(C.c_double), C.c_int32, C.c_double, C.POINTER(C.c_double), C.POINTER(C.c_int32),
+                                       C.c_int32, C.c_int32, C.c_int64, C.c_int32, C.POINTER(C.c_double), C.c_int32,
+                                       C.POINTER(C.c_int32), C.POINTER(C.c_int32)]
     L.so_plan_step_info.restype = C.c_int32
     L.so_plan_step_info.argtypes = [C.c_void_p, C.c_int32, C.POINTER(so_step_info_t)]
     L.so_resample_positions.restype = C.c_int32
diff --git a/signaloperators.jl_amd/csrc/capi.cpp b/signaloperators.jl_amd/csrc/capi.cpp
--- a/signaloperators.jl_amd/csrc/capi.cpp
+++ b/signaloperators.jl_amd/csrc/capi.cpp
@@ -229,4 +229,24 @@
     return so::resample_positions(fs_in, fs_out, rate, nphi, h, hlen, n_out, j, p, alpha, nfix, nbaked);
 }
 
-}
+int32_t so_rsos_wproj_matrix(const double* sos, int32_t nsec, double gain, const double* tab, const int32_t* jend,
+                             int32_t ngroups, int32_t kw, int64_t m, int32_t wp, double* v, int32_t capacity,
+                             int32_t* j0, int32_t* k) {
+    if (!sos || !tab || !jend || !v || !j0 || !k || nsec < 1 || nsec > 6 || ngroups < 1 || kw < 1 || m < 1 || wp < 1)
+        return set_err(SO_ERR_INVALID, "so_rsos_wproj_matrix: bad arguments");
+    if (ngroups > 256 || kw > 4096 || capacity < 0 || m > (1 << 20) || wp > (1 << 20) || (int64_t)wp * m + kw > (1 << 22))
+        return set_err(SO_ERR_INVALID, "so_rsos_wproj_matrix: period, window or warm-up too long");
+    for (int g = 0; g < ngroups; ++g)
+        if (jend[g] < -(1 << 22) || jend[g] > (1 << 22)) return set_err(SO_ERR_INVALID, "so_rsos_wproj_matrix: window end out of range");
+    std::vector<double> V;
+    int jj = 0, K = 0;
+    so::rsos_wproj_matrix_sos(sos, nsec, gain, tab, jend, ngroups, kw, m, wp, V, jj, K);
+    *j0 = jj;
+    *k = K;
+    if (K > capacity) return set_err(SO_ERR_INVALID, "so_rsos_wproj_matrix: capacity too small");
+    for (int d = 0; d < 12; ++d)
+        for (int o = 0; o < K; ++o) v[(size_t)d * capacity + o] = V[(size_t)d * K + o];
+    return SO_OK;
+}
+
+}
diff --git a/signaloperators.jl_amd/csrc/executor.cpp b/signaloperators.jl_amd/csrc/executor.cpp
--- a/signaloperators.jl_amd/csrc/executor.cpp
+++ b/signaloperators.jl_amd/csrc/executor.cpp
@@ -1277,6 +1277,21 @@
             if (S.kind == ST_SOS && S.rsos_src >= 0 && S.need > 0) return S.rs.ks + 14;
         return 0;
     }
+    case SO_COUNTER_WPROJ: {
+        for (const Stage& S : P->stages)
+            if (S.kind == ST_SOS && S.rsos_src >= 0 && S.need > 0) return S.rs.wproj;
+        return 0;
+    }
+    case SO_COUNTER_RSOS_RANGE_PERIODS:
+    case SO_COUNTER_RSOS_WARMUP_PERIODS:
+    case SO_COUNTER_RSOS_PERIOD_INPUTS:
+    case SO_COUNTER_WPROJ_FRAMES:
+    case SO_COUNTER_WPROJ_FIRST:
+        for (const Stage& S : P->stages)
+            if (S.kind == ST_SOS && S.rsos_src >= 0 && S.need > 0)
+                return which == SO_COUNTER_RSOS_RANGE_PERIODS ? S.rs.pr : which == SO_COUNTER_RSOS_WARMUP_PERIODS ? S.rs.wp
+                     : which == SO_COUNTER_RSOS_PERIOD_INPUTS ? S.rs.M : which == SO_COUNTER_WPROJ_FRAMES ? S.rs.wk : S.rs.wj0;
+        return 0;
     default: return -1;
     }
 }
diff --git a/signaloperators.jl_amd/csrc/k_rsos.hip b/signaloperators.jl_amd/csrc/k_rsos.hip
--- a/signaloperators.jl_amd/csrc/k_rsos.hip
+++ b/signaloperators.jl_amd/csrc/k_rsos.hip
@@ -215,6 +215,7 @@
 }
 
 constexpr int kRsosFlagLdp = 0, kRsosFlagYrd = 4, kRsosFlagXseq = 16, kRsosFlagSseq = 48, kRsosFlagXh = 49, kRsosFlagLnd = 52, kRsosFlags = 56;
+constexpr int kRsosFlagWp = 37;
 constexpr int kRsosHres0 = 1, kRsosHres1 = 5, kRsosHres2 = 7, kRsosHelper = 6, kRsosHslots = 3;
 constexpr int kRsosMaxGroups = 256;
 
@@ -228,6 +229,7 @@
     int flags[kRsosFlags];
     int jend[kRsosMaxGroups];
     RsCtl ctl;
+    int wpe, proj;
 };
 
 __device__ __forceinline__ int uni(int v) { return __builtin_amdgcn_readfirstlane(v); }
@@ -298,7 +300,7 @@
     const int ct = uni(g.ct), rgs = uni(g.rgs);
     const int64_t ncg = uni(g.nch) / ct;
     const int64_t pr = rfl64(g.pr), M = rfl64(g.M), L = rfl64(g.L);
-    const int wp = uni(g.wp), ulo = uni(g.ulo);
+    const int wp = uni(sh->wpe), ulo = uni(g.ulo);
     RsosGroup q;
     q.cg = (int)(G % ncg);
     const int64_t r0 = (G / ncg) * rgs;
@@ -324,7 +326,7 @@
     const SO_LDS RsSos& g = sh->g;
     const int ngroups = uni(g.ngroups);
     const RsosLds l = rsos_carve(dyn, uni(g.cyc) > 0 ? 0 : ngroups * uni(g.ks) * 64, uni(g.rpitch), NX, rsos_nss(NY));
-    const int NB = (uni(g.wp) + (int)rfl64(g.pr)) * ngroups;
+    const int NB = (uni(sh->wpe) + (int)rfl64(g.pr)) * ngroups;
     const double SO_GLB* mats = (const double SO_GLB*)rfl64((int64_t)(uintptr_t)g.mats);
     long long* trace = (long long*)rfl64((int64_t)(uintptr_t)g.trace);
     const uint32_t fl_base = (uint32_t)(uintptr_t)sh->flags;
@@ -338,6 +340,8 @@
     [[maybe_unused]] const long long cyc0 = SO_RSOS_COUNT ? clock64() : 0;
     while (uni(flag_ld(fl_base + 4 * (kRsosFlagXseq + 0))) < 1 && !(debug & 4)) SO_SPIN_PAUSE(spins, 1, 1 << 22);
     v4d sA = v4d{0.0, 0.0, 0.0, 0.0}, sB = v4d{0.0, 0.0, 0.0, 0.0};
+#pragma unroll
+    for (int v = 0; v < NK; ++v) sA[v] = l.ss[v * 64 + lane];
     v4d dA = v4d{0.0, 0.0, 0.0, 0.0}, dB = v4d{0.0, 0.0, 0.0, 0.0};
 #pragma unroll
     for (int v = 0; v < NK; ++v) dA[v] = l.xs[v * 64 + lane];
@@ -486,7 +490,7 @@
     const RsosLds l = rsos_carve(dyn, uni(g.cyc) > 0 ? 0 : ngroups * uni(g.ks) * 64, rpitch, NX, rsos_nss(NY));
     const int ct = uni(g.ct);
     const int M = (int)rfl64(g.M);
-    const int NP = uni(g.wp) + (int)rfl64(g.pr);
+    const int NP = uni(sh->wpe) + (int)rfl64(g.pr);
     const int ulo = uni(g.ulo);
     const int64_t n_in = rfl64(g.n_in);
     long long* trace = (long long*)rfl64((int64_t)(uintptr_t)g.trace);
@@ -959,6 +963,137 @@
     }
 }
 
+typedef double v2d_a8 __attribute__((ext_vector_type(2), aligned(8)));
+
+__device__ __forceinline__ bool rsos_wproj_group(const RsosShared& sh, int64_t G) {
+    const RsSos& g = sh.g;
+    const DCarrier& C0 = sh.ctl.car[0];
+    if (!g.wproj || g.src32 || g.arr2 || g.fuse < -1 || g.ct < 8) return false;
+    if (!(C0.base != nullptr && C0.vec_ok && C0.dtype == SO_F64) || (C0.df & 1)) return false;
+    const int64_t ncg = g.nch / g.ct;
+    const int64_t r0 = (G / ncg) * g.rgs, r1 = r0 + g.rgs - 1;
+    if (r1 >= g.nranges || r0 * g.pr < g.wp) return false;
+    if (g.store_lo > r0 * g.pr * g.L) return false;
+    const int64_t lo_ok = C0.a > 0 ? C0.a : 0, hi_ok = C0.b < g.n_in ? C0.b : g.n_in;
+    const int64_t f0 = (r0 * g.pr - g.wp) * g.M + g.wj0, f1 = (r1 * g.pr - g.wp) * g.M + g.wj0 + g.wk;
+    return f0 >= lo_ok && f1 <= hi_ok;
+}
+
+template <int NY>
+__device__ __attribute__((noinline)) void rsos_wproj_y(RsosShared* sh_, double* dyn, int64_t G_, int yi_) {
+    constexpr int NX = 2 * NY + 1;
+    const int lane = threadIdx.x & 63;
+    SO_LDS RsosShared* const sh = (SO_LDS RsosShared*)rsos_lds_ptr(sh_);
+    const int64_t G = rfl64(G_);
+    const int yi = uni(yi_);
+    const SO_LDS RsSos& g = sh->g;
+    const RsosLds l = rsos_carve(dyn, uni(g.cyc) > 0 ? 0 : uni(g.ngroups) * uni(g.ks) * 64, uni(g.rpitch), NX, rsos_nss(NY));
+    const uint32_t fl_base = (uint32_t)(uintptr_t)sh->flags;
+    const int ct = uni(g.ct), K = uni(g.wk);
+    const int npairs = (K + 7) >> 3;
+    const int c0 = (int)((int64_t)yi * npairs / NY), c1 = (int)((int64_t)(yi + 1) * npairs / NY);
+    const double SO_GLB* const V = (const double SO_GLB*)rfl64((int64_t)(uintptr_t)g.mats) + 14 * 64 + lane;
+    const SO_LDS DCarrier& C0 = sh->ctl.car[0];
+    const int64_t ncg = uni(g.nch) / ct;
+    const int gq = lane >> 4, n16 = lane & 15;
+    const int64_t r = (G / ncg) * uni(g.rgs) + n16 / ct;
+    const int64_t f0 = (r * rfl64(g.pr) - uni(g.wp)) * rfl64(g.M) + uni(g.wj0);
+    const double SO_GLB* const row = (const double SO_GLB*)rfl64((int64_t)(uintptr_t)C0.base) +
+                                     ((int64_t)((int)(G % ncg) * ct + n16 % ct) * rfl64(C0.cstride) + rfl64(C0.df) + f0 + 2 * gq);
+    v4d acc = v4d{0.0, 0.0, 0.0, 0.0};
+    auto mm = [&](const double (&a)[16], const v2d (&b)[8]) __attribute__((always_inline)) {
+#pragma unroll
+        for (int i = 0; i < 8; ++i) {
+            acc = __builtin_amdgcn_mfma_f64_16x16x4f64(a[2 * i], b[i][0], acc, 0, 0, 0);
+            acc = __builtin_amdgcn_mfma_f64_16x16x4f64(a[2 * i + 1], b[i][1], acc, 0, 0, 0);
+        }
+    };
+    auto load = [&](int c, double (&a)[16], v2d (&b)[8]) __attribute__((always_inline)) {
+        const double SO_GLB* const vp = V + (size_t)c * 128;
+        const double SO_GLB* const rp = row + (size_t)c * 8;
+#pragma unroll
+        for (int i = 0; i < 8; ++i) {
+            a[2 * i] = vp[i * 128];
+            a[2 * i + 1] = vp[i * 128 + 64];
+            b[i] = *(const v2d_a8 SO_GLB*)(rp + 8 * i);
+        }
+    };
+    double aA[16], aB[16];
+    v2d bA[8], bB[8];
+    const int c1f = min(c1, K >> 3);
+    const int nfull = c1f > c0 ? (c1f - c0) >> 3 : 0;
+    if (nfull > 0) {
+        load(c0, aA, bA);
+        for (int n = 0; n < nfull; n += 2) {
+            const int c = c0 + 8 * n;
+            if (n + 1 < nfull) load(c + 8, aB, bB);
+            mm(aA, bA);
+            if (n + 2 < nfull) load(c + 16, aA, bA);
+            if (n + 1 < nfull) mm(aB, bB);
+        }
+    }
+    {
+        const int c = c0 + 8 * nfull;
+#pragma unroll
+        for (int i = 0; i < 8; ++i) {
+            const int cc = c + i;
+            aA[2 * i] = aA[2 * i + 1] = 0.0;
+            bA[i] = v2d{0.0, 0.0};
+            if (cc < c1) {
+                aA[2 * i] = V[(size_t)(2 * cc) * 64];
+                aA[2 * i + 1] = V[(size_t)(2 * cc + 1) * 64];
+                const int f = 8 * cc + 2 * gq;
+                if (f + 1 < K) bA[i] = *(const v2d_a8 SO_GLB*)(row + 8 * cc);
+                else if (f < K) bA[i][0] = row[8 * cc];
+            }
+        }
+        mm(aA, bA);
+    }
+#pragma unroll
+    for (int v = 0; v < 3; ++v) l.ss[(1 + yi) * 192 + v * 64 + lane] = acc[v];
+    flag_st(fl_base + 4 * (kRsosFlagWp + yi), 1);
+}
+
+template <int NY>
+__device__ __attribute__((noinline)) void rsos_wproj_chain(RsosShared* sh_, double* dyn, int64_t G_) {
+    constexpr int NX = 2 * NY + 1;
+    const int lane = threadIdx.x & 63;
+    SO_LDS RsosShared* const sh = (SO_LDS RsosShared*)rsos_lds_ptr(sh_);
+    const int64_t G = rfl64(G_);
+    const SO_LDS RsSos& g = sh->g;
+    const RsosLds l = rsos_carve(dyn, uni(g.cyc) > 0 ? 0 : uni(g.ngroups) * uni(g.ks) * 64, uni(g.rpitch), NX, rsos_nss(NY));
+    const uint32_t fl_base = (uint32_t)(uintptr_t)sh->flags;
+    const int ct = uni(g.ct), fuse = uni(g.fuse);
+    const int gq = lane >> 4, n16 = lane & 15;
+    double s[3] = {0.0, 0.0, 0.0};
+    if (fuse >= 0) {
+        const SO_LDS DCarrier& C0 = sh->ctl.car[0];
+        const DLeaf leaf0 = leaf_uniform(sh_->ctl.leaves[min(kCtlLeaves - 1, max(0, uni(C0.slot_leaf[0])))]);
+        const int64_t ncg = uni(g.nch) / ct;
+        const int64_t r = (G / ncg) * uni(g.rgs) + n16 / ct;
+        const int64_t f0 = (r * rfl64(g.pr) - uni(g.wp)) * rfl64(g.M) + uni(g.wj0);
+        const double2 sc = rsos_sine_at(f0 + leaf0.df + 1, leaf0.v0, leaf0.v1, leaf0.v2, leaf0.flag);
+        const double SO_GLB* const W = (const double SO_GLB*)rfl64((int64_t)(uintptr_t)g.mats) + 14 * 64 + (size_t)((uni(g.wk) + 7) >> 3) * 128;
+#pragma unroll
+        for (int v = 0; v < 3; ++v) {
+            const double t = fma(sc.y, W[gq + 4 * v], sc.x * W[16 + gq + 4 * v]);
+            s[v] = fuse == 2 ? -t : t;
+        }
+    }
+    int spins = 0;
+    for (;;) {
+        const int f = lane < NY ? flag_ld(fl_base + 4 * (kRsosFlagWp + lane)) : 1;
+        if (wave_min(f, NY) >= 1) break;
+        SO_SPIN_PAUSE(spins, 1, 1 << 22);
+    }
+#pragma unroll
+    for (int yi = 0; yi < NY; ++yi)
+#pragma unroll
+        for (int v = 0; v < 3; ++v) s[v] += l.ss[(1 + yi) * 192 + v * 64 + lane];
+#pragma unroll
+    for (int v = 0; v < 3; ++v) l.ss[v * 64 + lane] = s[v];
+}
+
 template <int NY>
 __device__ __attribute__((noinline)) void rsos_helper(RsosShared* sh_, double* dyn) {
     constexpr int NX = 2 * NY + 1;
@@ -966,7 +1101,7 @@
     SO_LDS RsosShared* const sh = (SO_LDS RsosShared*)rsos_lds_ptr(sh_);
     const SO_LDS RsSos& g = sh->g;
     const RsosLds l = rsos_carve(dyn, 0, uni(g.rpitch), NX, rsos_nss(NY));
-    const int NB = (uni(g.wp) + (int)rfl64(g.pr)) * uni(g.ngroups);
+    const int NB = (uni(sh->wpe) + (int)rfl64(g.pr)) * uni(g.ngroups);
     const double SO_GLB* mats = (const double SO_GLB*)rfl64((int64_t)(uintptr_t)g.mats);
     const uint32_t fl_base = (uint32_t)(uintptr_t)sh->flags;
     const int debug = uni(g.debug);
@@ -1015,7 +1150,7 @@
     const SO_LDS RsSos& g = sh->g;
     const int ngroups = uni(g.ngroups), rpitch = uni(g.rpitch), RING = uni(g.ring);
     const RsosLds l = rsos_carve(dyn, CYC > 0 ? 0 : ngroups * KS * 64, rpitch, NX, rsos_nss(NY));
-    const int ct = uni(g.ct), wp = uni(g.wp), debug = uni(g.debug);
+    const int ct = uni(g.ct), wp = uni(sh->wpe), debug = uni(g.debug);
     const int M = (int)rfl64(g.M);
     const int NB = (wp + (int)rfl64(g.pr)) * ngroups;
     constexpr int kw = 4 * KS;
@@ -1440,9 +1575,17 @@
         __syncthreads();
         if (threadIdx.x < kRsosFlags) sh.flags[threadIdx.x] = 0;
         if (threadIdx.x < 192) ss[threadIdx.x] = 0.0;
+        if (threadIdx.x == 0) {
+            const bool pj = NW != 16 && NW != 17 && rsos_wproj_group(sh, G);
+            sh.proj = pj ? 1 : 0;
+            sh.wpe = pj ? 0 : g.wp;
+            if (pj) sh.flags[kRsosFlagSseq] = -1;
+        }
         __syncthreads();
+        const bool proj = sh.proj != 0;
         if (wave == 0) {
             if (!(g.debug & 64)) {
+                if (proj) rsos_wproj_chain<NY>(&sh, lds_raw, G);
                 const int nk = (g.debug & 131072) ? 3 : (2 * g.nsec + 3) / 4;
                 if (nk <= 1) rsos_chain<NY, 1>(&sh, lds_raw, G);
                 else if (nk == 2) rsos_chain<NY, 2>(&sh, lds_raw, G);
@@ -1517,6 +1660,7 @@
             {
             if (NW >= 16 && wave > 12) continue;
             const int yi = NW == 16 ? (wave < 4 ? wave - 1 : wave < 8 ? wave - 2 : wave < 12 ? wave - 3 : 9) : wave - (wave > 4 ? 2 : 1);
+            if (proj) rsos_wproj_y<NY>(&sh, lds_raw, G, yi);
             if constexpr (sizeof(TO) == 4 && CYC > 0) {
                 if (g.f32m) {
                     rsos_ywave<KS, NY, NL, TO, CYC, true, HW>(&sh, lds_raw, G, yi);
diff --git a/signaloperators.jl_amd/csrc/plan.h b/signaloperators.jl_amd/csrc/plan.h
--- a/signaloperators.jl_amd/csrc/plan.h
+++ b/signaloperators.jl_amd/csrc/plan.h
@@ -20,6 +20,8 @@
 int design_resample_rational(int64_t num, int64_t den, std::vector<double>& h, std::string& err);
 int design_resample_arbitrary(double rate, int nphi, std::vector<double>& h, std::string& err);
 
+void rsos_wproj_matrix_sos(const double* sos, int nsec, double gain, const double* tab, const int* jend, int ngroups, int kw, int64_t M, int wp,
+                           std::vector<double>& V, int& j0, int& K);
 int resample_positions(double fs_in, double fs_out, double rate, int nphi, const double* h, int hlen,
                        int64_t n_out, int64_t* j, int32_t* p, double* alpha, int64_t* nfix, int64_t* nbaked);
 
diff --git a/signaloperators.jl_amd/csrc/sigops_internal.h b/signaloperators.jl_amd/csrc/sigops_internal.h
--- a/signaloperators.jl_amd/csrc/sigops_internal.h
+++ b/signaloperators.jl_amd/csrc/sigops_internal.h
@@ -308,7 +308,9 @@
     int32_t debug;
     int32_t cyc;
     int32_t arr2;
-    int32_t pad_;
+    int32_t wproj;
+    int32_t wk;
+    int32_t wj0;
     int64_t out_pitch;
     int64_t store_lo;
     const double* mats;
diff --git a/signaloperators.jl_amd/csrc/stages.cpp b/signaloperators.jl_amd/csrc/stages.cpp
--- a/signaloperators.jl_amd/csrc/stages.cpp
+++ b/signaloperators.jl_amd/csrc/stages.cpp
@@ -1462,9 +1462,12 @@
     }
 }
 
-static void rsos_block_matrices(const SosCoefs& cf, std::vector<double>& mats) {
+static void rsos_block_columns(const SosCoefs& cf, std::vector<double>& Tm, std::vector<double>& Cm, std::vector<double>& Dm, std::vector<double>& Am) {
     const int ns = cf.nsec, D = 2 * ns, B = 16;
-    std::vector<double> Tm(B * B, 0.0), Cm(B * 12, 0.0), Dm(12 * B, 0.0), Am(12 * 12, 0.0);
+    Tm.assign(B * B, 0.0);
+    Cm.assign(B * 12, 0.0);
+    Dm.assign(12 * B, 0.0);
+    Am.assign(12 * 12, 0.0);
     for (int col = 0; col < B + D; ++col) {
         std::vector<double> st(D, 0.0);
         if (col >= B) st[col - B] = 1.0;
@@ -1485,6 +1488,12 @@
             else Am[d * 12 + (col - B)] = st[d];
         }
     }
+}
+
+static void rsos_block_matrices(const SosCoefs& cf, std::vector<double>& mats) {
+    const int B = 16;
+    std::vector<double> Tm, Cm, Dm, Am;
+    rsos_block_columns(cf, Tm, Cm, Dm, Am);
     mats.assign((size_t)14 * 64, 0.0);
     for (int lane = 0; lane < 64; ++lane) {
         const int i = lane & 15, kq = lane >> 4;
@@ -1498,6 +1507,60 @@
             }
         }
     }
+}
+
+static void rsos_wproj_matrix(const SosCoefs& cf, const double* tab, const int* jend, int ngroups, int kw, int64_t M, int wp, std::vector<double>& V,
+                       int& j0, int& K) {
+    std::vector<double> Tm, Cm, Dm, Am;
+    rsos_block_columns(cf, Tm, Cm, Dm, Am);
+    int64_t lo = INT64_MAX, hi = INT64_MIN;
+    for (int p = 0; p < wp; p += std::max(1, wp - 1))
+        for (int gi = 0; gi < ngroups; ++gi) {
+            const int64_t o = (int64_t)p * M + jend[gi] - (kw - 1);
+            lo = std::min(lo, o);
+            hi = std::max(hi, o + kw - 1);
+        }
+    j0 = (int)lo;
+    K = (int)(hi - lo + 1);
+    std::vector<long double> acc((size_t)12 * K, 0.0L), P(12 * 16), Q(12 * 16);
+    for (int i = 0; i < 12 * 16; ++i) P[i] = Dm[i];
+    for (int64_t b = (int64_t)wp * ngroups - 1; b >= 0; --b) {
+        const int gi = (int)(b % ngroups);
+        const int64_t o0 = (b / ngroups) * M + jend[gi] - (kw - 1) - lo;
+        for (int kk = 0; kk < kw; ++kk) {
+            const double* tp = tab + ((size_t)gi * kw + kk) * 16;
+            for (int d = 0; d < 12; ++d) {
+                long double a = 0.0L;
+                for (int t = 0; t < 16; ++t) a += P[d * 16 + t] * (long double)tp[t];
+                acc[(size_t)d * K + o0 + kk] += a;
+            }
+        }
+        if (b == 0) break;
+        for (int d = 0; d < 12; ++d)
+            for (int t = 0; t < 16; ++t) {
+                long double a = 0.0L;
+                for (int e = 0; e < 12; ++e) a += (long double)Am[d * 12 + e] * P[e * 16 + t];
+                Q[d * 16 + t] = a;
+            }
+        P.swap(Q);
+    }
+    V.resize(acc.size());
+    for (size_t i = 0; i < acc.size(); ++i) V[i] = (double)acc[i];
+}
+
+void rsos_wproj_matrix_sos(const double* sos, int nsec, double gain, const double* tab, const int* jend, int ngroups, int kw, int64_t M, int wp,
+                           std::vector<double>& V, int& j0, int& K) {
+    SosCoefs cf{};
+    cf.nsec = nsec;
+    cf.gain = gain;
+    for (int f = 0; f < nsec; ++f) {
+        cf.b0[f] = sos[6 * f + 0];
+        cf.b1[f] = sos[6 * f + 1];
+        cf.b2[f] = sos[6 * f + 2];
+        cf.a1[f] = sos[6 * f + 4];
+        cf.a2[f] = sos[6 * f + 5];
+    }
+    rsos_wproj_matrix(cf, tab, jend, ngroups, kw, M, wp, V, j0, K);
 }
 
 void Plan::fuse_resample_sos() {
@@ -1715,7 +1778,17 @@
             if (ngrp < std::atoll(ev)) continue;
         } else {
             const double unit_cost = ct >= 8 ? 1.0 : ct == 4 ? 1.1 : ct == 2 ? 1.15 : 3.2;
-            const double t_fused = (double)((ngrp + cus - 1) / cus) * (double)((pr + wp) * ngp) * 0.30 * unit_cost * (ks + 14) / 28.0 + 15.0;
+            bool wpj = !std::getenv("SIGOPS_RSOS_NOWPROJ") && !std::getenv("SIGOPS_RSOS_NWAVES") && nodes[S2.node].dtype == SO_F64 && !two_arrays && !was_ga &&
+                       ct >= 8 && wp * Mp + kwp <= 16384;
+            if (wpj && plain_src) wpj = S3.in_array_node >= 0 && nodes[nodes[S3.node].kids[0]].dtype != SO_F32;
+            else if (wpj) {
+                const DCarrier& c0 = S3.carriers[0];
+                const bool sine = c0.nsteps == 1 && (c0.arg[0] & 0x2ff) == 0 && c0.nslots >= 1 && (c0.op[0] == OP_ADD || (c0.op[0] == OP_SUB && !(c0.arg[0] & 0x100))) &&
+                                  c0.slot_kind[0] == OP_FUNC && leaves[c0.slot_leaf[0]].mode == SO_FN_SIN && leaves[c0.slot_leaf[0]].sf == 1;
+                wpj = c0.dtype == SO_F64 && c0.array_node >= 0 && (c0.nsteps == 0 || sine);
+            }
+            const double t_pro = wpj ? 0.013 * (double)(wp * Mp + kwp) : 0.0;
+            const double t_fused = (double)((ngrp + cus - 1) / cus) * ((double)((pr + (wpj ? 0 : wp)) * ngp) * 0.30 * unit_cost * (ks + 14) / 28.0 + t_pro) + 15.0;
             const double t_two = 8.0e-6 * (double)need * nch + 95.0;
             if (std::getenv("SIGOPS_DEBUG_PLAN"))
                 std::fprintf(stderr, "[sigops] k_rsos estimate: fused %.0f us (%lld groups, %lld + %lld periods), two kernels %.0f us\n", t_fused,
@@ -1846,6 +1919,53 @@
         }
         S2.rsos_grid = (int)std::min<int64_t>(ngrp, cus);
         rsos_block_matrices(cf, S2.rsos_mats_host);
+        {
+            const std::vector<double>& tb = own_tab ? S2.rsos_tab_host : S3.tab_host;
+            const std::vector<int>& je = own_tab ? S2.rsos_jend_host : S3.jend_host;
+            const DCarrier& c0 = S3.carriers[0];
+            const bool form = g.fuse == -1 || ((g.fuse == 1 || g.fuse == 2) && g.fuse_sine);
+            S2.rs.wproj = 0;
+            if (!std::getenv("SIGOPS_RSOS_NOWPROJ") && nodes[S2.node].dtype == SO_F64 && !two_arrays && !g.src32 && !g.ring32 && !g.f32m &&
+                !g.gsplit && !g.help && (g.nwaves == 12 || g.nwaves == 8) && ct >= 8 && form && c0.dtype == SO_F64 && c0.array_node >= 0 &&
+                tb.size() == (size_t)ngp * kwp * 16 && (int)je.size() >= ngp && wp * Mp + kwp <= 16384) {
+                std::vector<double> V;
+                int j0 = 0, K = 0;
+                rsos_wproj_matrix(cf, tb.data(), je.data(), ngp, kwp, Mp, (int)wp, V, j0, K);
+                const int K8 = (K + 7) / 8 * 8;
+                std::vector<double>& mt = S2.rsos_mats_host;
+                mt.resize((size_t)14 * 64 + (size_t)K8 / 4 * 64 + 32, 0.0);
+                for (int ksx = 0; ksx < K8 / 4; ++ksx)
+                    for (int lane = 0; lane < 64; ++lane) {
+                        const int i = lane & 15, f = 8 * (ksx >> 1) + 2 * (lane >> 4) + (ksx & 1);
+                        mt[(size_t)14 * 64 + (size_t)ksx * 64 + lane] = i < 12 && f < K ? V[(size_t)i * K + f] : 0.0;
+                    }
+                if (g.fuse >= 0) {
+                    const DLeaf& L0 = leaves[c0.slot_leaf[0]];
+                    const long double wc = L0.flag ? (long double)L0.v0 / (long double)L0.v2 : 1.0L / (long double)L0.v2;
+                    long double vs[12] = {}, vc[12] = {};
+                    for (int f = 0; f < K; ++f) {
+                        long double ph = wc * f;
+                        ph -= floorl(ph);
+                        const long double sn = sinl(2.0L * 3.141592653589793238462643383279502884L * ph);
+                        const long double cs = cosl(2.0L * 3.141592653589793238462643383279502884L * ph);
+                        for (int i = 0; i < 12; ++i) {
+                            vs[i] += (long double)V[(size_t)i * K + f] * sn;
+                            vc[i] += (long double)V[(size_t)i * K + f] * cs;
+                        }
+                    }
+                    for (int i = 0; i < 12; ++i) {
+                        mt[(size_t)14 * 64 + (size_t)K8 / 4 * 64 + i] = (double)vs[i];
+                        mt[(size_t)14 * 64 + (size_t)K8 / 4 * 64 + 16 + i] = (double)vc[i];
+                    }
+                }
+                S2.rs.wproj = 1;
+                S2.rs.wk = K;
+                S2.rs.wj0 = j0;
+                if (std::getenv("SIGOPS_DEBUG_PLAN"))
+                    std::fprintf(stderr, "[sigops] k_rsos: warm-up as one product: %d frames from %d (%d k-steps instead of %lld blocks)\n", K, j0, K8 / 4,
+                                 (long long)(wp * ngp));
+            }
+        }
         S2.rsos_mats_buf = raw_buf(S2.rsos_mats_host.size() * 8);
         if (S2.bad_buf < 0) S2.bad_buf = raw_buf((size_t)nch * 4);
         S3.fused_away = true;
diff --git a/signaloperators.jl_amd/engine.py b/signaloperators.jl_amd/engine.py
--- a/signaloperators.jl_amd/engine.py
+++ b/signaloperators.jl_amd/engine.py
@@ -110,7 +110,12 @@
     def counters(self):
         L = K.lib()
         return {"graph_replays": L.so_plan_counter(self.handle, 0), "graph_captures": L.so_plan_counter(self.handle, 1),
-                "direct_executes": L.so_plan_counter(self.handle, 2), "fused_mfmas_per_block": L.so_plan_counter(self.handle, 3)}
+                "direct_executes": L.so_plan_counter(self.handle, 2), "fused_mfmas_per_block": L.so_plan_counter(self.handle, 3),
+                "wproj": L.so_plan_counter(self.handle, 4)}
+
+    def rsos_geometry(self):
+        L = K.lib()
+        return {k: L.so_plan_counter(self.handle, i) for i, k in enumerate(("pr", "wp", "M", "wproj_frames", "wproj_first"), 5)}
 
     def steps(self):
         out = []
```

Result: faster. 29.75 billion, median of 6 (+1.8%).
